# KirillHit/snn_for_object_detection

Hardware: AMD Instinct MI355X
Metric: event-frames/sec (BxT) SODa-3M GEN1 304x240 fwd+bwd (higher is better)
Workload: dtype f32 (16-bit split products)

## Files before the change

include/snn_hip.h:

```cpp
#ifndef SNN_HIP_H
#define SNN_HIP_H

#include <stddef.h>
#include <stdint.h>

#ifdef __cplusplus
extern "C" {
#endif

#define SNN_ABI_VERSION 20

enum {
    SNN_NEURON_NONE = 0,
    SNN_NEURON_LIF = 1,
    SNN_NEURON_LI = 2,
    SNN_NEURON_LI_TANH = 3,
    SNN_NEURON_SLI = 4,
    SNN_NEURON_SYNAPSE = 5
};

enum { SNN_PREC_FP32 = 0, SNN_PREC_BF16X3 = 1, SNN_PREC_BF16X6 = 3, SNN_PREC_FP16X3 = 4, SNN_PREC_BF16X1 = 5,
       SNN_PREC_BF16S = 6 };

enum { SNN_SCAN_WIDE_ADDRESSING = 1,
       SNN_SCAN_LAST_STEP_ONLY = 2,
       SNN_SCAN_BF16_STORAGE = 4,
       SNN_SCAN_SPIKES_FROM_VDEC = 8,
       SNN_SCAN_SUMS_FROM_STATE = 16,
       SNN_SCAN_STATE_LOOKBACK = 32   };

enum { SNN_POOL_AVG = 0, SNN_POOL_MAX = 1, SNN_POOL_SUM = 2 };

enum { SNN_ACT_RELU = 0, SNN_ACT_SILU = 1, SNN_ACT_TANH = 2 };

enum { SNN_SURR_SUPER = 0, SNN_SURR_TRIANGLE = 1, SNN_SURR_SIGMOID = 2, SNN_SURR_ATAN = 3 };

typedef struct snn_neuron_params {
    float c_mem;
    float c_syn;
    float v_leak;
    float v_th;
    float v_reset;
    float alpha;
    float v_st;
    float tau_sec;
    float tau_dis;
    float dt;
    float sigma;
    int surrogate;
    int reset_detached;
} snn_neuron_params;

int snn_abi_version(void);
const char* snn_last_error(void);

int snn_nchw_to_nhwc(const float* src, float* dst, int64_t N, int C, int H, int W, void* stream);
int snn_nhwc_to_nchw(const float* src, float* dst, int64_t N, int C, int H, int W, void* stream);
int snn_weight_transpose(const float* w, float* wt, int Cout, int KH, int KW, int Cin, void* stream);
int snn_weight_transpose_batched(const float* flat_w, float* flat_wt, const int64_t* table, int n_layers, void* stream);
int snn_weight_presplit(const float* w, void* out, int64_t n, int precision, void* stream);

int snn_conv2d_wgrad_bn_supported(int64_t N, int H, int W, int Cin, int Ho, int Wo, int Cout, int KH, int KW, int stride,
// ... 30 lines not shown
                     const float* addend2, int64_t ld_addend2, int precision, void* stream);
int snn_conv2d_wgrad(const float* x, int64_t ldx, const float* dy, int64_t lddy, float* dw,
                     int64_t N, int H, int W, int Cin, int Ho, int Wo, int Cout,
                     int KH, int KW, int stride, int pad, int accumulate,
                     float* workspace, int splitk, int precision, void* stream);
int snn_conv2d_wgrad_splitk(int64_t N, int H, int W, int Cin, int Ho, int Wo, int Cout, int KH, int KW,
                            int stride, int pad, int precision);
int snn_conv2d_wgrad_kernel(int64_t N, int H, int W, int Cin, int Ho, int Wo, int Cout, int KH, int KW, int stride, int pad,
                            int precision);
int snn_conv2d_gather_plan(int mode, int64_t N, int H, int W, int Cin, int Ho, int Wo, int Cout, int KH, int KW, int stride,
                           int pad, int64_t ld_in, int64_t ld_out, int align_bits, int has_split_image, int has_addend,
                           int has_addend2, int frames_per_step, int precision, int phase, int* out);
int snn_conv2d_wgrad_plan(int64_t N, int H, int W, int Cin, int Ho, int Wo, int Cout, int KH, int KW, int stride, int pad,
                          int64_t ldx, int64_t lddy, int align_bits, int precision, int spikes, int num_cu, int* out);
int snn_conv1x1_spikes_supported(int64_t N, int H, int W, int Cin, int Cout, int64_t ld, int fwd_precision,
                                 int bwd_precision);
int snn_conv1x1_spikes_fwd(const float* vdec, int64_t ld, float v_th, const float* w, float* y, int64_t ldy, int64_t N, int H,
                           int W, int Cin, int Cout, void* stream);
int snn_conv1x1_spikes_wgrad(const float* vdec, int64_t ld, float v_th, const float* dy, int64_t lddy, float* dw, int64_t N,
                             int H, int W, int Cin, int Cout, int accumulate, float* workspace, int splitk, void* stream);

int snn_conv2d_spikes_supported(int64_t N, int H, int W, int Cin, int Ho, int Wo, int Cout, int KH, int KW, int stride,
                                int pad, int64_t ld, int fwd_precision, int bwd_precision);
int snn_conv2d_spikes_fwd(const float* vdec, int64_t ld, float v_th, const float* w, float* y, int64_t ldy, int64_t N, int H,
                          int W, int Cin, int Ho, int Wo, int Cout, int KH, int KW, int stride, int pad, double* bn_partial,
                          int frames_per_step, int* bn_layout, void* stream);
int snn_conv2d_spikes_wgrad(const float* vdec, int64_t ld, float v_th, const float* dy, int64_t lddy, float* dw, int64_t N,
                            int H, int W, int Cin, int Ho, int Wo, int Cout, int KH, int KW, int stride, int pad,
                            int accumulate, float* workspace, int splitk, void* stream);
int snn_conv3x3_halo_spikes(const float* vdec, int64_t ld, float v_th, const void* w_image, float* y, int64_t ldy, int64_t N,
                            int H, int W, int Cin, int Cout, double* bn_partial, int frames_per_step, int* bn_layout,
                            void* stream);

size_t snn_bn_stats_partial_size(int T, int64_t M, int C);
int snn_bn_stats(const float* y, int64_t ldy, int T, int64_t M, int C, double* partial, void* stream);
int snn_bn_stats_finalize(const double* partial, int chunks, int rows_per_chunk, int T, int64_t M, int C,
                          const float* gamma, const float* bias, float eps, float momentum,
                          float* running_mean, float* running_var, int use_running,
                          float* mean, float* invstd, float* alpha, float* beta, void* stream);

int snn_bn_stats_reduce(const double* partial, int chunks, int rows_per_chunk, int T, int64_t M, int C, double* sums,
                        void* stream);
int snn_bn_stats_from_sums(const double* sums, int T, int64_t M_total, int C,
                           const float* gamma, const float* bias, float eps, float momentum,
                           float* running_mean, float* running_var,
                           float* mean, float* invstd, float* alpha, float* beta,
                           double* var_scratch, void* stream);

int snn_affine_neuron_fwd(int neuron, const float* y, int64_t ldy,
                          const float* alpha, const float* beta,
                          const float* v0, const float* i0,
                          float* out, int64_t ldo, const float* addend, int64_t ld_addend,
                          float* vT, float* iT, float* vdec,
                          int T, int64_t M, int C, const snn_neuron_params* p, int flags, void* stream);

size_t snn_affine_neuron_bwd_sums_size(int T, int64_t M, int C);
int snn_affine_neuron_bwd_sums_from_state(int neuron, int T, int64_t M, int C, int64_t ldg, const snn_neuron_params* p,
                                          int flags);
int snn_affine_neuron_bwd_plan(int neuron, int T, int64_t M, int C, int64_t ldg, int64_t ldy, int with_sums,
                               const snn_neuron_params* p, int flags, int64_t* out);
int snn_affine_neuron_bwd(int neuron, const float* g_out, int64_t ldg, const float* state,
                          const float* y, int64_t ldy, const float* g_vT, const float* g_iT,
                          const float* alpha, const float* beta, int apply_scale,
                          float* gx, float* g_v0, float* g_i0, double* sums,
                          int T, int64_t M, int C, const snn_neuron_params* p, int flags, void* stream);

int snn_lif_tau_param(const float* w_mem, const float* w_syn, int n, int C, float* c_mem, float* c_syn, void* stream);
int snn_lif_tau_fwd(int neuron, const float* y, int64_t ldy, const float* alpha, const float* beta,
                    const float* v0, const float* i0, float* out, int64_t ldo,
                    const float* addend, int64_t ld_addend, float* vT, float* iT, float* vdec,
                    int T, int64_t M, int C, const snn_neuron_params* p,
                    const float* c_mem, const float* c_syn, int flags, void* stream);
size_t snn_lif_tau_bwd_partial_size(int T, int64_t M, int C, int with_sums);
int snn_lif_tau_bwd_plan(int neuron, int T, int64_t M, int C, int64_t ldg, int64_t ldy, int with_sums, int with_tau_sums,
                         const snn_neuron_params* p, int flags, int64_t* out);
int snn_lif_tau_bwd(int neuron, const float* g_out, int64_t ldg, const float* state, const float* y, int64_t ldy,
                    const float* g_vT, const float* g_iT, const float* alpha, const float* beta, int apply_scale,
                    float* gx, float* g_v0, float* g_i0, double* sums,
                    int T, int64_t M, int C, const snn_neuron_params* p,
                    const float* c_mem, const float* c_syn, const float* v0, double* tau_partial, int flags, void* stream);
int snn_lif_tau_finalize(const double* tau_partial, int T, int64_t M, int C, int with_sums,
                         const float* c_mem, const float* c_syn, int per_layer,
                         float* d_wmem, float* d_wsyn, int accumulate, void* stream);

int snn_lif_ckpt_interval(void);
int snn_lif_fwd_ckpt(const float* y, int64_t ldy, const float* alpha, const float* beta,
                     const float* v0, const float* i0, float* out, int64_t ldo,
// ... 144 lines not shown
```

snn_for_object_detection_amd/_hip.py:

```python

import ctypes
import os
from ctypes import POINTER, Structure, c_char_p, c_double, c_float, c_int, c_int32, c_int64, c_size_t, c_void_p

_HERE = os.path.dirname(os.path.abspath(__file__))
LIB_PATH = os.environ.get("SNN_HIP_LIB") or os.path.join(_HERE, "libsnn_hip.so")

NEURON_NONE, NEURON_LIF, NEURON_LI, NEURON_LI_TANH, NEURON_SLI, NEURON_SYNAPSE = 0, 1, 2, 3, 4, 5
POOL_AVG, POOL_MAX, POOL_SUM = 0, 1, 2
ACT_RELU, ACT_SILU, ACT_TANH = 0, 1, 2
ABI_VERSION = 20
PREC_FP32, PREC_BF16X3, PREC_BF16X6, PREC_FP16X3, PREC_BF16X1, PREC_BF16S = 0, 1, 3, 4, 5, 6
SCAN_WIDE_ADDRESSING, SCAN_LAST_STEP_ONLY, SCAN_BF16_STORAGE, SCAN_SPIKES_FROM_VDEC, SCAN_SUMS_FROM_STATE = 1, 2, 4, 8, 16
SCAN_STATE_LOOKBACK = 32
SURR_SUPER, SURR_TRIANGLE, SURR_SIGMOID, SURR_ATAN = 0, 1, 2, 3


class NeuronParams(Structure):
    _fields_ = [("c_mem", c_float), ("c_syn", c_float), ("v_leak", c_float), ("v_th", c_float),
                ("v_reset", c_float), ("alpha", c_float), ("v_st", c_float), ("tau_sec", c_float),
                ("tau_dis", c_float), ("dt", c_float), ("sigma", c_float),
                ("surrogate", c_int), ("reset_detached", c_int)]


_P, _I, _L, _F = c_void_p, c_int, c_int64, c_float

SIGNATURES = {
    "snn_abi_version": (c_int, []),
    "snn_last_error": (c_char_p, []),
    "snn_nchw_to_nhwc": (c_int, [_P, _P, _L, _I, _I, _I, _P]),
    "snn_nhwc_to_nchw": (c_int, [_P, _P, _L, _I, _I, _I, _P]),
    "snn_weight_transpose": (c_int, [_P, _P, _I, _I, _I, _I, _P]),
    "snn_weight_transpose_batched": (c_int, [_P, _P, _P, _I, _P]),
    "snn_detect_decode": (c_int, [_P, _P, _P, _I, _I, _P, _P, _P, _P]),
    "snn_nms_sorted": (c_int, [_P, _P, _P, _I, _F, _P, _P, _P, _P, _P]),
    "snn_detect_decode_batched": (c_int, [_P, _P, _P, _I, _I, _I, _P, _P, _P, _P]),
    "snn_nms_sorted_batched": (c_int, [_P, _P, _P, _I, _I, _I, _F, _P, _P, _P, _P, _P]),
    "snn_detect_assemble": (c_int, [_P, _P, _P, _P, _P, _P, _I, _I, _I, _F, _P, _P]),
    "snn_conv2d_fwd": (c_int, [_P, _L, _P, _P, _P, _L, _L, _I, _I, _I, _I, _I, _I, _I, _I, _I, _I, _P, _L, _P, _I, _P, _I,
                               _P]),
    "snn_weight_presplit": (c_int, [_P, _P, _L, _I, _P]),
    "snn_conv2d_fwd_bn_partial_size": (c_size_t, [_L, _I, _I, _I, _I]),
    "snn_conv2d_wgrad_bn_supported": (c_int, [_L, _I, _I, _I, _I, _I, _I, _I, _I, _I, _I]),
    "snn_conv2d_wgrad_bn": (c_int, [_P, _L, _P, _L, _P, _L, _P, _I, _I, _P, _L, _I, _I, _I, _I, _I, _I, _I, _I, _I, _I, _I,
                                    _P, _I, _P]),
    "snn_conv3x3_s2_dgrad_supported": (c_int, [_L, _I, _I, _I, _I, _I, _I]),
    "snn_conv3x3_s2_dgrad_plan": (c_int, [_L, _I, _I, _I, _I, _I, _I, _P]),
    "snn_conv3x3_halo_plan": (c_int, [_L, _I, _I, _I, _I, _I, _P]),
    "snn_conv2d_wgrad_halo_plan": (c_int, [_L, _I, _I, _I, _I, _I, _I, _I, _I, _P]),
    "snn_conv_first_plan": (c_int, [_L, _I, _I, _I, _I, _I, _I, _I, _I, _I, _I, _P]),
    "snn_conv3x3_s2_dgrad": (c_int, [_P, _L, _P, _P, _L, _L, _I, _I, _I, _I, _I, _I, _P, _L, _P, _L, _I, _P]),
    "snn_conv3x3_halo_supported": (c_int, [_L, _I, _I, _I, _I]),
    "snn_conv3x3_halo_bn_chunks": (c_int64, [_I, _I, _I]),
    "snn_weight_frag_image_bytes": (c_size_t, [_I, _I]),
    "snn_weight_frag_image_batched": (c_int, [_P, _P, _P, _I, _I, _I, _I, _P]),
    "snn_conv3x3_halo": (c_int, [_P, _L, _P, _P, _L, _L, _I, _I, _I, _I, _P, _L, _P, _L, _P, _I, _P, _I, _P]),
    "snn_conv2d_dgrad": (c_int, [_P, _L, _P, _P, _P, _L, _L, _I, _I, _I, _I, _I, _I, _I, _I, _I, _I, _P, _L, _P, _L,
                                 _I, _P]),
    "snn_conv2d_wgrad": (c_int, [_P, _L, _P, _L, _P, _L, _I, _I, _I, _I, _I, _I, _I, _I, _I, _I, _I, _P, _I, _I,
                                 _P]),
    "snn_conv2d_wgrad_splitk": (c_int, [_L, _I, _I, _I, _I, _I, _I, _I, _I, _I, _I, _I]),
    "snn_conv2d_wgrad_kernel": (c_int, [_L, _I, _I, _I, _I, _I, _I, _I, _I, _I, _I, _I]),
    "snn_conv2d_gather_plan": (c_int, [_I, _L, _I, _I, _I, _I, _I, _I, _I, _I, _I, _I, _L, _L, _I, _I, _I, _I, _I, _I, _I, _P]),
    "snn_conv2d_wgrad_plan": (c_int, [_L, _I, _I, _I, _I, _I, _I, _I, _I, _I, _I, _L, _L, _I, _I, _I, _I, _P]),
    "snn_conv1x1_spikes_supported": (c_int, [_L, _I, _I, _I, _I, _L, _I, _I]),
    "snn_conv1x1_spikes_fwd": (c_int, [_P, _L, _F, _P, _P, _L, _L, _I, _I, _I, _I, _P]),
    "snn_conv1x1_spikes_wgrad": (c_int, [_P, _L, _F, _P, _L, _P, _L, _I, _I, _I, _I, _I, _P, _I, _P]),
    "snn_conv2d_spikes_supported": (c_int, [_L, _I, _I, _I, _I, _I, _I, _I, _I, _I, _I, _L, _I, _I]),
    "snn_conv2d_spikes_fwd": (c_int, [_P, _L, _F, _P, _P, _L, _L, _I, _I, _I, _I, _I, _I, _I, _I, _I, _I, _P, _I, _P, _P]),
    "snn_conv2d_spikes_wgrad": (c_int, [_P, _L, _F, _P, _L, _P, _L, _I, _I, _I, _I, _I, _I, _I, _I, _I, _I, _I, _P, _I, _P]),
    "snn_conv3x3_halo_spikes": (c_int, [_P, _L, _F, _P, _P, _L, _L, _I, _I, _I, _I, _P, _I, _P, _P]),
    "snn_bn_stats_partial_size": (c_size_t, [_I, _L, _I]),
    "snn_bn_stats": (c_int, [_P, _L, _I, _L, _I, _P, _P]),
    "snn_bn_stats_finalize": (c_int, [_P, _I, _I, _I, _L, _I, _P, _P, _F, _F, _P, _P, _I, _P, _P, _P, _P, _P]),
    "snn_bn_stats_reduce": (c_int, [_P, _I, _I, _I, _L, _I, _P, _P]),
    "snn_bn_stats_from_sums": (c_int, [_P, _I, _L, _I, _P, _P, _F, _F, _P, _P, _P, _P, _P, _P, _P, _P]),
    "snn_bn_bwd_reduce": (c_int, [_P, _I, _L, _I, _P, _P]),
    "snn_bn_bwd_coef": (c_int, [_P, _P, _P, _I, _L, _I, _P, _P, _P, _P, _P, _P, _P, _P, _I, _P]),
    "snn_affine_neuron_fwd": (c_int, [_I, _P, _L, _P, _P, _P, _P, _P, _L, _P, _L, _P, _P, _P, _I, _L, _I,
                                      POINTER(NeuronParams), _I, _P]),
    "snn_lif_ckpt_interval": (c_int, []),
    "snn_lif_fwd_ckpt": (c_int, [_P, _L, _P, _P, _P, _P, _P, _L, _P, _L, _P, _P, _P, _I, _L, _I,
                                 POINTER(NeuronParams), _P]),
    "snn_lif_bwd_ckpt": (c_int, [_P, _L, _P, _P, _L, _P, _P, _P, _P, _I, _P, _P, _P, _P, _I, _L, _I,
                                 POINTER(NeuronParams), _P]),
    "snn_affine_neuron_bwd_sums_size": (c_size_t, [_I, _L, _I]),
    "snn_affine_neuron_bwd": (c_int, [_I, _P, _L, _P, _P, _L, _P, _P, _P, _P, _I, _P, _P, _P, _P, _I, _L, _I,
                                      POINTER(NeuronParams), _I, _P]),
    "snn_bn_bwd_finalize": (c_int, [_P, _I, _L, _I, _P, _P, _P, _P, _P, _P, _P, _P, _I, _P]),
    "snn_bn_bwd_finalize_from_state": (c_int, [_P, _I, _L, _I, _P, _P, _P, _P, _P, _P, _L, _P, _P, _P, _P, _P, _I, _P]),
    "snn_bn_bwd_reduce_from_state": (c_int, [_P, _I, _L, _I, _P, _P, _P, _P, _P, _P, _L, _P, _P]),
    "snn_affine_neuron_bwd_sums_from_state": (c_int, [_I, _I, _L, _I, _L, POINTER(NeuronParams), _I]),
    "snn_affine_neuron_bwd_plan": (c_int, [_I, _I, _L, _I, _L, _L, _I, POINTER(NeuronParams), _I, _P]),
    "snn_lif_tau_param": (c_int, [_P, _P, _I, _I, _P, _P, _P]),
    "snn_lif_tau_fwd": (c_int, [_I, _P, _L, _P, _P, _P, _P, _P, _L, _P, _L, _P, _P, _P, _I, _L, _I,
                                POINTER(NeuronParams), _P, _P, _I, _P]),
    "snn_lif_tau_bwd_partial_size": (c_size_t, [_I, _L, _I, _I]),
    "snn_lif_tau_bwd_plan": (c_int, [_I, _I, _L, _I, _L, _L, _I, _I, POINTER(NeuronParams), _I, _P]),
    "snn_lif_tau_bwd": (c_int, [_I, _P, _L, _P, _P, _L, _P, _P, _P, _P, _I, _P, _P, _P, _P, _I, _L, _I,
                                POINTER(NeuronParams), _P, _P, _P, _P, _I, _P]),
    "snn_lif_tau_finalize": (c_int, [_P, _I, _L, _I, _I, _P, _P, _I, _P, _P, _I, _P]),
    "snn_bn_bwd_apply": (c_int, [_P, _P, _L, _P, _P, _P, _P, _L, _I, _L, _I, _I, _P]),
    "snn_bn_bwd_apply_bf16": (c_int, [_P, _P, _L, _P, _P, _P, _P, _L, _I, _L, _I, _I, _P]),
    "snn_bn_stats_bf16": (c_int, [_P, _L, _I, _L, _I, _P, _P]),
    "snn_copy_channels": (c_int, [_P, _L, _P, _L, _L, _I, _P]),
    "snn_add_channels": (c_int, [_P, _L, _P, _L, _L, _I, _P]),
    "snn_add": (c_int, [_P, _L, _P, _L, _P, _L, _L, _I, _P]),
    "snn_roi_workspace_size": (c_size_t, [_I, _I, _I]),
    "snn_roi_assign": (c_int, [_P, _P, _I, _I, _I, _F, _P, _P, _P, _P, _P]),
    "snn_det_loss_workspace_size": (c_size_t, [_L]),
    "snn_det_loss_fwd": (c_int, [_P, _P, _P, _P, _P, _L, _I, _F, _P, _P, _P, _P]),
    "snn_det_loss_bwd": (c_int, [_P, _P, _P, _P, _P, _L, _I, _F, _P, _P, _P, _P, _P]),
    "snn_label_steps": (c_int, [_P, _I, _I, _I, _I, _I, _P, _P]),
# ... 80 lines not shown
```

snn_for_object_detection_amd/csrc/conv_common.h:

```cpp
#pragma once
#include "snn_common.h"

namespace {

constexpr int kThreads = 256;
#define SNN_CONV_MIN_WAVES 3

typedef __bf16 bf16x8 __attribute__((ext_vector_type(8)));
typedef __bf16 bf16x4 __attribute__((ext_vector_type(4)));
typedef __bf16 bf16x2 __attribute__((ext_vector_type(2)));
typedef float f32x2 __attribute__((ext_vector_type(2)));
typedef unsigned u32x4 __attribute__((ext_vector_type(4)));
typedef unsigned u32x2 __attribute__((ext_vector_type(2)));
typedef _Float16 f16x8 __attribute__((ext_vector_type(8)));
typedef _Float16 f16x2 __attribute__((ext_vector_type(2)));
constexpr float kF16WeightScale = 256.0f;
constexpr float kF16ActScale = 16.0f;
constexpr float kF16Unscale = 1.0f / (kF16WeightScale * kF16ActScale);

__device__ __forceinline__ int div_magic(int n, int d, unsigned magic) { return d == 1 ? n : (int)__umulhi((unsigned)n, magic); }

enum : unsigned {
    kAlignIn16 = 1u, kAlignIn8 = 2u, kAlignW16 = 4u, kAlignOut16 = 8u, kAlignOut8 = 16u, kAlignAdd16 = 32u, kAlignAdd8 = 64u,
    kAlignAdd2_16 = 128u, kAlignAdd2_8 = 256u, kAlignSplit16 = 512u, kAlignAll = 1023u
// ... 17 lines not shown
           N * (int64_t)Ho * Wo < 0x7fffffffLL && (int64_t)H * W * ld * 16 < 0x7fffffffLL;
}

}

struct FirstGeom {
    int64_t ldx, ldy;
    int rows;
    int H, W, Ho, Wo, Cout, stride, pad;
    int group_rows, group_blocks;
    double* bn_partial;
    const float* bn_y;
    int64_t bn_ldy;
    const float* bn_coef;
    int bn_tc;
    int bn_fps;
    int rs;
};

struct FirstPlan {
    int ok;
    int rs, LW, cgs, PP;
    int blocks;
    int group_rows, group_blocks;
    int max_rows, last_stage_rows;
    size_t lds;
};
FirstPlan snn_first_layer_plan(int64_t N, int H, int W, int Ho, int Wo, int Cout, int stride, int pad,
                               int frames_per_step, bool wgrad, int num_cu);
bool snn_first_layer_shape(int Cin, int Cout, int KH, int KW);
int snn_first_layer_blocks(int64_t rows, int num_cu);
int snn_launch_first(bool wgrad, bool bnapply, bool sb, int blocks, size_t lds, const float* x, const float* w,
                     const float* dy, float* out, const FirstGeom& fg, void* stream, const char* name);
```

snn_for_object_detection_amd/csrc/conv_gather.hip:

```cpp
#include <stdlib.h>
#include <type_traits>
#include "conv_common.h"

#if defined(SNN_STAMP) || defined(SNN_CLOCK)
__device__ unsigned long long g_stamps[2048 * 8];
__device__ unsigned long long g_stamps2[2048 * 4];
extern "C" int snn_debug_stamps(unsigned long long* out, int n) {
    return (int)hipMemcpyFromSymbol(out, HIP_SYMBOL(g_stamps), sizeof(unsigned long long) * n);
}
extern "C" int snn_debug_stamps2(unsigned long long* out, int n) {
    return (int)hipMemcpyFromSymbol(out, HIP_SYMBOL(g_stamps2), sizeof(unsigned long long) * n);
}
#endif
#ifdef SNN_STAMP
#define STAMP(i) do { unsigned long long t_ = __builtin_readcyclecounter(); st_acc[i] += t_ - st_last; st_last = t_; } while (0)
#else
#define STAMP(i) do {} while (0)
#endif

namespace {

constexpr int BM = 128;
constexpr int BK = 32;
constexpr int LDK = BK + 4;
// ... 24 lines not shown
template <int WM, int WN, int TN>
__device__ __forceinline__ void stat_flush(double (&s)[TN], double (&q)[TN], double* red, double* __restrict__ partial,
                                           int64_t step, int64_t chunk, int64_t chunks, int n0, int OC, int tid) {
    const int lane = tid & 63, wave = tid >> 6;
#pragma unroll
    for (int j = 0; j < TN; ++j) {
        s[j] += __shfl_xor(s[j], 32, 64);
        q[j] += __shfl_xor(q[j], 32, 64);
        if (lane < 32) {
            red[((wave * TN + j) * 32 + lane) * 2 + 0] = s[j];
            red[((wave * TN + j) * 32 + lane) * 2 + 1] = q[j];
        }
    }
    __syncthreads();
    if (tid < WN * TN * 32) {
        const int wn = tid / (TN * 32), jr = tid % (TN * 32);
        double ss = 0.0, qq = 0.0;
#pragma unroll
        for (int wm = 0; wm < WM; ++wm) {
            const double* src = red + (((wm * WN + wn) * TN) * 32 + jr) * 2;
            ss += src[0];
            qq += src[1];
        }
        if (n0 + tid < OC) {
            double* dst = partial + snn_bn_partial_index(step, chunk, n0 + tid, chunks, OC);
            dst[0] = ss;
            dst[1] = qq;
        }
    }
    __syncthreads();
}

template <int BN, int WM, int WN, bool DGRAD, bool VEC, int SPLIT, bool FAST, bool PRESPLIT = false, bool SB = false,
          bool XSP = false>
__global__ __launch_bounds__(kThreads, (FAST && SPLIT) ? (PRESPLIT ? 3 : (SB ? (DGRAD ? 4 : SNN_GATHER_SB_WAVES) : 2)) : SNN_CONV_MIN_WAVES) void k_conv_gather(const float* __restrict__ in, const float* __restrict__ wk,
                                                          float* __restrict__ out, ConvGeom g,
                                                          const float* __restrict__ addend, int64_t ld_add,
                                                          const float* __restrict__ addend2, int64_t ld_add2) {
    constexpr int TM = BM / WM / 32;
    constexpr int TN = BN / WN / 32;
    constexpr int BROWS = BN / 32;
    static_assert(WM * WN == 4, "4 waves");
    static_assert(!SB || (FAST && SPLIT == 5 && !PRESPLIT), "bf16 storage: the pipelined one-product kernel");
    static_assert(!XSP || (FAST && SPLIT == 4 && !DGRAD && !PRESPLIT && !SB), "spikes from potentials: fp16 x 3 forward");
    constexpr int ES = SB ? 2 : 4;
    constexpr int NPIECE = SPLIT == 3 ? 3 : (SPLIT == 5 ? 1 : 2);
    constexpr int A_BYTES = SPLIT ? NPIECE * BM * LDB * 2 : BM * LDK * 4;
    constexpr int B_BYTES = SPLIT ? NPIECE * BN * LDB * 2 : BN * LDK * 4;
    constexpr int STAGE_BYTES = 4 * 32 * (TN * 32 + 4) * 4;
    constexpr int SMEM_BYTES = A_BYTES + B_BYTES > STAGE_BYTES ? A_BYTES + B_BYTES : STAGE_BYTES;
    __shared__ __attribute__((aligned(16))) unsigned char smem[SMEM_BYTES];
    float* As = reinterpret_cast<float*>(smem);
    float* Bs = reinterpret_cast<float*>(smem + A_BYTES);
    __bf16* Ah = reinterpret_cast<__bf16*>(smem);
    __bf16* Al = Ah + BM * LDB;
    __bf16* Am = Al + BM * LDB;
    __bf16* Bh = reinterpret_cast<__bf16*>(smem + A_BYTES);
    __bf16* Bl = Bh + BN * LDB;
    __bf16* Bm = Bl + BN * LDB;

    const int tid = threadIdx.x;
#if defined(SNN_STAMP) || defined(SNN_CLOCK)
    const unsigned long long st_kernel_begin = __builtin_amdgcn_s_memtime();
    const unsigned long long st_real_begin = __builtin_amdgcn_s_memrealtime();
#endif
    const int lane_id = tid & 63, wave = tid >> 6;
    const int wm = wave / WN, wn = wave % WN;
    const int r = lane_id & 31, h = lane_id >> 5;

    const int bid_xcd = blockIdx.x & 7, bid_q = blockIdx.x >> 3;
    const int bid_n = bid_q % g.ntiles;
    const int64_t bid_m = (int64_t)bid_xcd * g.mtiles_per_xcd + bid_q / g.ntiles;
    if (bid_m >= g.mtiles) return;
    const int64_t m0 = bid_m * BM;
    const int n0 = bid_n * BN;

    const int lrr = tid >> 3;
// ... 10 lines not shown
        const unsigned t = mm / ow_;
        const int ox = (int)(mm - t * ow_);
        const unsigned img = t / oh_;
        const int oy = (int)(t - img * oh_);
        a_base[j] = (int)(img * (unsigned)(g.IH * g.IW));
        if (!DGRAD) {
            a_y0[j] = oy * g.stride - g.pad;
            a_x0[j] = ox * g.stride - g.pad;
        } else if (g.stride == 1) {
            a_y0[j] = oy + g.pad;
            a_x0[j] = ox + g.pad;
        } else {
            a_y0[j] = (int)((unsigned)(oy * g.stride + g.ph + g.pad - g.kh0) / (unsigned)g.stride);
            a_x0[j] = (int)((unsigned)(ox * g.stride + g.pw + g.pad - g.kw0) / (unsigned)g.stride);
        }
    }

    auto decode_k = [&](int kk, int& dy, int& dx, int& c, int& wcol) {
        int tap = div_magic(kk, g.IC, g.magic_ic);
        c = kk - tap * g.IC;
        if (!DGRAD) {
            int kh = div_magic(tap, g.KW, g.magic_kw), kw = tap - kh * g.KW;
            dy = kh;
            dx = kw;
            wcol = kk;
        } else {
            int jh = div_magic(tap, g.nkw, g.magic_kw), jw = tap - jh * g.nkw;
            dy = -jh;
            dx = -jw;
            wcol = ((g.kh0 + g.stride * jh) * g.KW + (g.kw0 + g.stride * jw)) * g.IC + c;
        }
    };

    using AReg = typename std::conditional<SB, u32x2, f32x4>::type;
    AReg ra[4];
    f32x4 rb[BROWS];

    __amdgpu_buffer_rsrc_t rs_a, rs_b;
    int a_rel[4];
    unsigned a_mask[4];
    unsigned b_rel[BROWS];
    if (FAST) {
        const int ow_ = DGRAD ? g.OWc : g.OW, oh_ = DGRAD ? g.OHc : g.OH;
        const int64_t img0 = (unsigned)m0 / (unsigned)(oh_ * ow_);
        const int64_t ipix = (int64_t)g.IH * g.IW;
        const int64_t bytes = ((((int64_t)g.nimg - img0) * ipix - 1) * g.ldi + g.IC) * ES;
        rs_a = __builtin_amdgcn_make_buffer_rsrc(const_cast<char*>(reinterpret_cast<const char*>(in) + img0 * ipix * g.ldi * ES), 0,
                                                 bytes > 0xffffffffLL ? (int)0xffffffffu : (int)(unsigned)bytes,
                                                 0x00020000);
        rs_b = __builtin_amdgcn_make_buffer_rsrc(const_cast<float*>(wk), 0, g.OC * g.KtotFull * 4, 0x00020000);
        const int tw_n = DGRAD ? g.nkw : g.KW;
#pragma unroll
        for (int j = 0; j < 4; ++j) {
            const int relpix = (a_base[j] - (int)(img0 * ipix)) + a_y0[j] * g.IW + a_x0[j];
            a_rel[j] = (relpix * (int)g.ldi + kq) * ES;
            const int nth = DGRAD ? g.nkh : g.KH;
            unsigned xm = 0, mask = 0;
#pragma unroll
            for (int tw = 0; tw < 6; ++tw) {
                const int ix = DGRAD ? a_x0[j] - tw : a_x0[j] + tw;
                xm |= (tw < tw_n && (unsigned)ix < (unsigned)g.IW) ? 1u << tw : 0u;
            }
#pragma unroll
            for (int th = 0; th < 6; ++th) {
                const int iy = DGRAD ? a_y0[j] - th : a_y0[j] + th;
                mask |= (th < nth && (unsigned)iy < (unsigned)g.IH) ? xm << (th * tw_n) : 0u;
            }
            a_mask[j] = a_ok[j] ? mask : 0u;
        }
#pragma unroll
        for (int j = 0; j < BROWS; ++j) {
            const int n = n0 + lr + 32 * j;
            b_rel[j] = n < g.OC ? (unsigned)(n * g.KtotFull + kq) * 4u : 0x80000000u;
        }
    }
    const unsigned fast_tw_n = DGRAD ? g.nkw : g.KW;
    const unsigned fast_tw_one = fast_tw_n == 1 ? 1u : 0u;
    auto load_tiles_fast = [&](int k0n, AReg (&ra)[4], f32x4 (&rb)[BROWS], int which = 3) {
        const bool kin = k0n < g.Ktot;
        const int tap = (int)__umulhi((unsigned)k0n, g.magic_ic);
        const int c0 = k0n - tap * g.IC;
        const int th = (int)(__umulhi((unsigned)tap, g.magic_kw) + (unsigned)tap * fast_tw_one);
        const int tw = tap - th * (int)fast_tw_n;
        int toff, wcol0;
        if (!DGRAD) {
            toff = ((th * g.IW + tw) * (int)g.ldi + c0) * ES;
            wcol0 = k0n;
        } else {
            toff = (c0 - (th * g.IW + tw) * (int)g.ldi) * ES;
            wcol0 = ((g.kh0 + g.stride * th) * g.KW + (g.kw0 + g.stride * tw)) * g.IC + c0;
        }
        const int tbit = kin ? tap : 31;
        if (which & 1) {
#pragma unroll
            for (int j = 0; j < 4; ++j) {
                const int voff = ((a_mask[j] >> tbit) & 1u) ? a_rel[j] + toff : -1;
                if constexpr (SB) ra[j] = __builtin_bit_cast(u32x2, __builtin_amdgcn_raw_buffer_load_b64(rs_a, voff, 0, 0));
                else ra[j] = __builtin_bit_cast(f32x4, __builtin_amdgcn_raw_buffer_load_b128(rs_a, voff, 0, 0));
            }
        }
        if (which & 2) {
            const unsigned wb = (unsigned)wcol0 * 4u;
#pragma unroll
            for (int j = 0; j < BROWS; ++j)
                rb[j] = __builtin_bit_cast(f32x4, __builtin_amdgcn_raw_buffer_load_b128(rs_b, (int)(b_rel[j] + wb), 0, 0));
        }
    };

    auto load_tiles = [&](int k0) {
        if (FAST) {
            load_tiles_fast(k0, ra, rb);
            return;
        }
        if constexpr (!SB) {
        const int kk = k0 + kq;
        if (VEC) {
            const bool kin = kk < g.Ktot;
            int dy, dx, c, wcol;
            decode_k(kin ? kk : g.Ktot - 4, dy, dx, c, wcol);
            const f32x4 zero = {0.f, 0.f, 0.f, 0.f};
#pragma unroll
            for (int j = 0; j < 4; ++j) {
                const int iy = a_y0[j] + dy, ix = a_x0[j] + dx;
                const bool ok = kin & a_ok[j] & ((unsigned)iy < (unsigned)g.IH) & ((unsigned)ix < (unsigned)g.IW);
                const int iyc = min(max(iy, 0), g.IH - 1), ixc = min(max(ix, 0), g.IW - 1);
                f32x4 v = *reinterpret_cast<const f32x4*>(in + (int64_t)(a_base[j] + iyc * g.IW + ixc) * g.ldi + c);
                ra[j] = ok ? v : zero;
            }
#pragma unroll
            for (int j = 0; j < BROWS; ++j) {
                const int n = n0 + lr + 32 * j;
                const int nc = min(n, g.OC - 1);
                f32x4 v = *reinterpret_cast<const f32x4*>(wk + (int64_t)nc * g.KtotFull + wcol);
                rb[j] = (kin & (n < g.OC)) ? v : zero;
            }
        } else {
#pragma unroll
            for (int e = 0; e < 4; ++e) {
                const int ke = kk + e;
                const bool kin = ke < g.Ktot;
                int dy, dx, c, wcol;
                decode_k(kin ? ke : 0, dy, dx, c, wcol);
#pragma unroll
                for (int j = 0; j < 4; ++j) {
                    const int iy = a_y0[j] + dy, ix = a_x0[j] + dx;
                    float v = 0.f;
                    if (kin && a_ok[j] && (unsigned)iy < (unsigned)g.IH && (unsigned)ix < (unsigned)g.IW)
// ... 4 lines not shown
                for (int j = 0; j < BROWS; ++j) {
                    int n = n0 + lr + 32 * j;
                    rb[j][e] = (kin && n < g.OC) ? wk[(int64_t)n * g.KtotFull + wcol] : 0.f;
                }
            }
        }
        }
    };
    auto split_store = [&](const f32x4& v, __bf16* hi_img, __bf16* mid_img, __bf16* lo_img, int row) {
        bf16x4 hi, mid, lo;
#pragma unroll
        for (int e = 0; e < 4; e += 2) {
            f32x2 rest = {v[e], v[e + 1]};
            bf16x2 p = __builtin_convertvector(rest, bf16x2);
            unsigned bits = __builtin_bit_cast(unsigned, p);
            hi[e] = p[0]; hi[e + 1] = p[1];
            rest[0] -= __builtin_bit_cast(float, bits << 16);
            rest[1] -= __builtin_bit_cast(float, bits & 0xffff0000u);
            if (SPLIT == 3) {
                p = __builtin_convertvector(rest, bf16x2);
                bits = __builtin_bit_cast(unsigned, p);
                mid[e] = p[0]; mid[e + 1] = p[1];
                rest[0] -= __builtin_bit_cast(float, bits << 16);
                rest[1] -= __builtin_bit_cast(float, bits & 0xffff0000u);
            }
            p = __builtin_convertvector(rest, bf16x2);
            lo[e] = p[0]; lo[e + 1] = p[1];
        }
        *reinterpret_cast<bf16x4*>(&hi_img[row * LDB + kq]) = hi;
        if (SPLIT == 3) *reinterpret_cast<bf16x4*>(&mid_img[row * LDB + kq]) = mid;
        *reinterpret_cast<bf16x4*>(&lo_img[row * LDB + kq]) = lo;
    };
    auto store_tiles = [&]() {
        if constexpr (SB) return;
        else if (SPLIT) {
#pragma unroll
            for (int j = 0; j < 4; ++j) split_store(ra[j], Ah, Am, Al, lr + 32 * j);
#pragma unroll
            for (int j = 0; j < BROWS; ++j) split_store(rb[j], Bh, Bm, Bl, lr + 32 * j);
        } else {
#pragma unroll
            for (int j = 0; j < 4; ++j) *reinterpret_cast<f32x4*>(&As[(lr + 32 * j) * LDK + kq]) = ra[j];
#pragma unroll
            for (int j = 0; j < BROWS; ++j) *reinterpret_cast<f32x4*>(&Bs[(lr + 32 * j) * LDK + kq]) = rb[j];
        }
    };

    f32x16 acc[TM][TN];
#pragma unroll
    for (int i = 0; i < TM; ++i)
#pragma unroll
        for (int j = 0; j < TN; ++j)
#pragma unroll
            for (int e = 0; e < 16; ++e) acc[i][j][e] = 0.f;

    if constexpr (FAST && SPLIT != 0) {
        constexpr int NP = NPIECE;
        constexpr int NPROD = SPLIT == 3 ? 6 : (SPLIT == 5 ? 1 : 3);
        bf16x4 pa[4][NP], pb[BROWS][NP];
        auto convert = [&](const f32x4& v, bf16x4* out, float scale) {
            if constexpr (SPLIT == 5) {
#pragma unroll
                for (int e = 0; e < 4; e += 2) {
                    const bf16x2 p = __builtin_convertvector(f32x2{v[e], v[e + 1]}, bf16x2);
                    out[0][e] = p[0]; out[0][e + 1] = p[1];
                }
                return;
// ... 3 lines not shown
#pragma unroll
                for (int e = 0; e < 4; e += 2) {
                    const float a = v[e] * scale, b = v[e + 1] * scale;
                    const f16x2 ph = __builtin_convertvector(f32x2{a, b}, f16x2);
                    const f16x2 pl = __builtin_convertvector(f32x2{a - (float)ph[0], b - (float)ph[1]}, f16x2);
                    hi[e >> 1] = __builtin_bit_cast(unsigned, ph);
                    lo[e >> 1] = __builtin_bit_cast(unsigned, pl);
                }
                out[0] = __builtin_bit_cast(bf16x4, hi);
                out[1] = __builtin_bit_cast(bf16x4, lo);
                return;
            }
#pragma unroll
            for (int e = 0; e < 4; e += 2) {
                f32x2 rest = {v[e], v[e + 1]};
                bf16x2 p = __builtin_convertvector(rest, bf16x2);
                unsigned bits = __builtin_bit_cast(unsigned, p);
                out[0][e] = p[0]; out[0][e + 1] = p[1];
                rest[0] -= __builtin_bit_cast(float, bits << 16);
                rest[1] -= __builtin_bit_cast(float, bits & 0xffff0000u);
                if (SPLIT == 3) {
                    p = __builtin_convertvector(rest, bf16x2);
                    bits = __builtin_bit_cast(unsigned, p);
                    out[2][e] = p[0]; out[2][e + 1] = p[1];
                    rest[0] -= __builtin_bit_cast(float, bits << 16);
                    rest[1] -= __builtin_bit_cast(float, bits & 0xffff0000u);
                }
                p = __builtin_convertvector(rest, bf16x2);
                out[1][e] = p[0]; out[1][e + 1] = p[1];
            }
        };
        auto convert_a = [&](const AReg& v, bf16x4* out) {
            if constexpr (SB) out[0] = __builtin_bit_cast(bf16x4, v);
            else if constexpr (XSP) {
                u32x2 hi;
#pragma unroll
                for (int e = 0; e < 4; e += 2)
                    hi[e >> 1] = (v[e] > g.x_th ? 0x4C00u : 0u) | (v[e + 1] > g.x_th ? 0x4C000000u : 0u);
                out[0] = __builtin_bit_cast(bf16x4, hi);
            } else convert(v, out, kF16ActScale);
        };
        auto convert_b = [&](const f32x4& v, bf16x4* out) {
            if constexpr (PRESPLIT) {
                static_assert(!PRESPLIT || SPLIT == 2 || SPLIT == 4, "pre-split weights: two-piece modes only");
                out[0] = __builtin_bit_cast(bf16x4, f32x2{v[0], v[1]});
                out[1] = __builtin_bit_cast(bf16x4, f32x2{v[2], v[3]});
            } else {
                convert(v, out, kF16WeightScale);
            }
        };
        auto write_tiles = [&]() {
#pragma unroll
            for (int j = 0; j < 4; ++j) {
                const int o = (lr + 32 * j) * LDB + kq;
                *reinterpret_cast<bf16x4*>(&Ah[o]) = pa[j][0];
                if constexpr (NP >= 2 && !XSP) *reinterpret_cast<bf16x4*>(&Al[o]) = pa[j][1];
                if constexpr (NP >= 3) *reinterpret_cast<bf16x4*>(&Am[o]) = pa[j][2];
            }
#pragma unroll
            for (int j = 0; j < BROWS; ++j) {
                const int o = (lr + 32 * j) * LDB + kq;
                *reinterpret_cast<bf16x4*>(&Bh[o]) = pb[j][0];
                if constexpr (NP >= 2) *reinterpret_cast<bf16x4*>(&Bl[o]) = pb[j][1];
                if constexpr (NP >= 3) *reinterpret_cast<bf16x4*>(&Bm[o]) = pb[j][2];
            }
        };
        auto mfma_group = [&](int ks) {
            bf16x8 ah[TM], am[TM], al[TM], bh[TN], bm[TN], bl[TN];
#pragma unroll
            for (int i = 0; i < TM; ++i) {
                const int off = ((wm * TM + i) * 32 + r) * LDB + ks * 16 + 8 * h;
                ah[i] = *reinterpret_cast<const bf16x8*>(&Ah[off]);
                if constexpr (NP >= 2 && !XSP) al[i] = *reinterpret_cast<const bf16x8*>(&Al[off]);
                if constexpr (NP >= 3) am[i] = *reinterpret_cast<const bf16x8*>(&Am[off]);
            }
#pragma unroll
            for (int j = 0; j < TN; ++j) {
                const int off = ((wn * TN + j) * 32 + r) * LDB + ks * 16 + 8 * h;
                bh[j] = *reinterpret_cast<const bf16x8*>(&Bh[off]);
                if constexpr (NP >= 2) bl[j] = *reinterpret_cast<const bf16x8*>(&Bl[off]);
                if constexpr (NP >= 3) bm[j] = *reinterpret_cast<const bf16x8*>(&Bm[off]);
            }
#pragma unroll
            for (int i = 0; i < TM; ++i)
#pragma unroll
                for (int j = 0; j < TN; ++j) {
                    if constexpr (SPLIT == 5) {
                        acc[i][j] = __builtin_amdgcn_mfma_f32_32x32x16_bf16(ah[i], bh[j], acc[i][j], 0, 0, 0);
                        continue;
                    }
                    if constexpr (SPLIT == 4 && XSP) {
                        const f16x8 xah = __builtin_bit_cast(f16x8, ah[i]);
                        const f16x8 xbh = __builtin_bit_cast(f16x8, bh[j]), xbl = __builtin_bit_cast(f16x8, bl[j]);
                        acc[i][j] = __builtin_amdgcn_mfma_f32_32x32x16_f16(xah, xbl, acc[i][j], 0, 0, 0);
                        acc[i][j] = __builtin_amdgcn_mfma_f32_32x32x16_f16(xah, xbh, acc[i][j], 0, 0, 0);
                        continue;
                    }
                    if constexpr (SPLIT == 4) {
                        const f16x8 xah = __builtin_bit_cast(f16x8, ah[i]), xal = __builtin_bit_cast(f16x8, al[i]);
                        const f16x8 xbh = __builtin_bit_cast(f16x8, bh[j]), xbl = __builtin_bit_cast(f16x8, bl[j]);
                        acc[i][j] = __builtin_amdgcn_mfma_f32_32x32x16_f16(xal, xbh, acc[i][j], 0, 0, 0);
                        acc[i][j] = __builtin_amdgcn_mfma_f32_32x32x16_f16(xah, xbl, acc[i][j], 0, 0, 0);
                        acc[i][j] = __builtin_amdgcn_mfma_f32_32x32x16_f16(xah, xbh, acc[i][j], 0, 0, 0);
                        continue;
                    }
                    acc[i][j] = __builtin_amdgcn_mfma_f32_32x32x16_bf16(al[i], bh[j], acc[i][j], 0, 0, 0);
                    acc[i][j] = __builtin_amdgcn_mfma_f32_32x32x16_bf16(ah[i], bl[j], acc[i][j], 0, 0, 0);
                    if (SPLIT == 3) {
                        acc[i][j] = __builtin_amdgcn_mfma_f32_32x32x16_bf16(am[i], bm[j], acc[i][j], 0, 0, 0);
                        acc[i][j] = __builtin_amdgcn_mfma_f32_32x32x16_bf16(am[i], bh[j], acc[i][j], 0, 0, 0);
                        acc[i][j] = __builtin_amdgcn_mfma_f32_32x32x16_bf16(ah[i], bm[j], acc[i][j], 0, 0, 0);
                    }
                    acc[i][j] = __builtin_amdgcn_mfma_f32_32x32x16_bf16(ah[i], bh[j], acc[i][j], 0, 0, 0);
                }
        };
        constexpr int NM = TM * TN * (XSP ? 2 : NPROD);
        constexpr int NREAD = XSP ? TM + TN * NP : (TM + TN) * NP;
        constexpr int CONV_OPS = SPLIT == 3 ? 24 : (SPLIT == 5 ? 2 : 14);
        constexpr int VPG_A = ((XSP ? 4 * 8 : 4 * CONV_OPS) + NM - 1) / NM;
        constexpr int VPG_B = PRESPLIT ? 1 : (BROWS * CONV_OPS + NM - 1) / NM;
        if (g.Ktot > 0) {
            AReg ra0[4];
            f32x4 rb0[BROWS];
            load_tiles_fast(0, ra0, rb0);
            load_tiles_fast(BK, ra, rb);
#pragma unroll
            for (int j = 0; j < 4; ++j) convert_a(ra0[j], pa[j]);
#pragma unroll
            for (int j = 0; j < BROWS; ++j) convert_b(rb0[j], pb[j]);
            write_tiles();
        }
        __syncthreads();
#ifdef SNN_STAMP
        unsigned long long st_acc[8] = {0, 0, 0, 0, 0, 0, 0, 0};
        unsigned long long st_last = __builtin_readcyclecounter();
        const unsigned long long st_begin = st_last;
#endif
#pragma unroll 1
        for (int k0 = 0; k0 < g.Ktot; k0 += BK) {
            mfma_group(0);
#pragma unroll
            for (int j = 0; j < 4; ++j) convert_a(ra[j], pa[j]);
            __builtin_amdgcn_sched_group_barrier(0x100, NREAD, 0);
#pragma unroll
            for (int m = 0; m < NM; ++m) {
                __builtin_amdgcn_sched_group_barrier(0x008, 1, 0);
                __builtin_amdgcn_sched_group_barrier(0x002, VPG_A, 0);
            }
            __builtin_amdgcn_sched_barrier(0);
            STAMP(0);
            mfma_group(1);
#pragma unroll
            for (int j = 0; j < BROWS; ++j) convert_b(rb[j], pb[j]);
            __builtin_amdgcn_sched_group_barrier(0x100, NREAD, 0);
#pragma unroll
            for (int m = 0; m < NM; ++m) {
                __builtin_amdgcn_sched_group_barrier(0x008, 1, 0);
                __builtin_amdgcn_sched_group_barrier(0x002, VPG_B, 0);
            }
            __builtin_amdgcn_sched_barrier(0);
            STAMP(1);
            load_tiles_fast(k0 + 2 * BK, ra, rb);
            STAMP(2);
            __syncthreads();
            STAMP(3);
            write_tiles();
            STAMP(4);
            __syncthreads();
            STAMP(5);
        }
#ifdef SNN_STAMP
        if (tid == 0 && bid_n == 0 && blockIdx.x < 2048) {
            st_acc[6] = __builtin_readcyclecounter() - st_begin;
            st_acc[7] = st_begin;
            for (int i = 0; i < 8; ++i) g_stamps[blockIdx.x * 8 + i] = st_acc[i];
        }
#endif
    } else {
        if (g.Ktot > 0) {
            load_tiles(0);
            store_tiles();
        }
        __syncthreads();

    #pragma unroll 1
        for (int k0 = 0; k0 < g.Ktot; k0 += BK) {
            load_tiles(k0 + BK);
            __builtin_amdgcn_sched_barrier(0);
            if (SPLIT) {
    #pragma unroll
                for (int ks = 0; ks < BK / 16; ++ks) {
                    bf16x8 ah[TM], am[TM], al[TM], bh[TN], bm[TN], bl[TN];
    #pragma unroll
                    for (int i = 0; i < TM; ++i) {
// ... 137 lines not shown
                const int a = (int)(t - img * (unsigned)g.OHc);
                const int64_t pix = ((int64_t)img * g.OH + (a * g.stride + g.ph)) * g.OW + (b * g.stride + g.pw);
                dst = out_b + (pix * g.ldo + n) * ES;
                a1p = ad1_b + (pix * ld_add + n) * ES;
                a2p = ad2_b + (pix * ld_add2 + n) * ES;
            }
            if (ovec && n + 3 < g.OC) {
                if (addend) v += St::ld4_last(a1p, 0);
                if (addend2) v += St::ld4_last(a2p, 0);
                St::st4(dst, 0, v);
            } else {
#pragma unroll
                for (int q = 0; q < 4; ++q)
                    if (n + q < g.OC) {
                        float o = v[q];
                        if (addend) o += St::ld1(a1p, q);
                        if (addend2) o += St::ld1(a2p, q);
                        St::st1(dst, q, o);
                    }
            }
        }
        __syncthreads();
    }
#if defined(SNN_STAMP) || defined(SNN_CLOCK)
    if (tid == 0 && bid_n == 0 && blockIdx.x < 2048) {
        g_stamps2[blockIdx.x * 4 + 0] = st_kernel_begin;
        g_stamps2[blockIdx.x * 4 + 1] = __builtin_amdgcn_s_memtime();
        g_stamps2[blockIdx.x * 4 + 2] = st_real_begin;
        g_stamps2[blockIdx.x * 4 + 3] = __builtin_amdgcn_s_memrealtime();
    }
#endif
}

enum GatherLoader { kLoadScalar = 0, kLoadVec = 1, kLoadFast = 2, kLoadFastPresplit = 3, kLoadSB = 4, kLoadXSP = 5 };
enum GatherRefusal { kGatherOk = 0, kGatherTooManyPixels, kGatherNotFastSB, kGatherNotFastXSP, kGatherGridTooLarge };
struct GatherPlan {
    int ok, why;
    int loader;
    int bn;
    int out_vec;
    int mtiles, mtiles_per_xcd, ntiles;
    int64_t blocks;
};
static GatherPlan gather_plan(const ConvGeom& g, bool dgrad, int split, bool sb, bool xsp, unsigned align, bool has_split,
                              bool has_add, bool has_add2) {
    GatherPlan p = {};
    const bool vec = (g.IC % 4 == 0) && (g.ldi % 4 == 0) && (align & (sb ? kAlignIn8 : kAlignIn16)) && (align & kAlignW16);
    const int64_t gm = snn_ceil_div(g.Mtot, BM);
    if (!(g.Mtot < 0x7fffffffLL && (int64_t)g.IH * g.IW < 0x7fffffffLL)) {
        p.why = kGatherTooManyPixels;
        return p;
    }
    const int nth = dgrad ? g.nkh : g.KH, ntw = dgrad ? g.nkw : g.KW;
    const int ntaps = nth * ntw;
    static const bool no_fast = snn_tuning_env("SNN_CONV_NO_FAST") != nullptr;
    const bool fast = vec && !no_fast && g.IC % BK == 0 && ntaps >= 1 && ntaps <= 31 && nth <= 6 && ntw <= 6 &&
                      (int64_t)g.IH * g.IW * g.ldi * 16 < 0x7fffffffLL && (int64_t)g.OC * g.KtotFull * 4 < 0x7fffffffLL;
    p.out_vec = (g.ldo % 4 == 0) && (align & (sb ? kAlignOut8 : kAlignOut16)) &&
                (!has_add || (align & (sb ? kAlignAdd8 : kAlignAdd16))) &&
                (!has_add2 || (align & (sb ? kAlignAdd2_8 : kAlignAdd2_16)));
    if (sb && !fast) {
        p.why = kGatherNotFastSB;
        return p;
    }
    if (xsp && !fast) {
        p.why = kGatherNotFastXSP;
        return p;
    }
    const bool presplit = has_split && (split == 2 || split == 4) && (align & kAlignSplit16);
    p.loader = sb ? kLoadSB : xsp ? kLoadXSP : (fast && presplit) ? kLoadFastPresplit : fast ? kLoadFast : vec ? kLoadVec : kLoadScalar;
    p.bn = g.OC <= 32 ? 32 : (g.OC <= 64 ? 64 : 128);
    p.mtiles = (int)gm;
    p.mtiles_per_xcd = (int)snn_ceil_div(gm, 8);
    p.ntiles = (int)snn_ceil_div(g.OC, p.bn);
    p.blocks = (int64_t)p.mtiles_per_xcd * 8 * p.ntiles;
    if (p.blocks > 0x7fffffffLL) {
        p.why = kGatherGridTooLarge;
        return p;
    }
    p.ok = 1;
    return p;
}

static unsigned gather_align_bits(const void* in, const void* wk, const void* wk_split, const void* out, const void* addend,
                                  int64_t ld_add, const void* addend2, int64_t ld_add2) {
    unsigned a = 0;
    if (aligned(16, {in})) a |= kAlignIn16;
    if (aligned(8, {in})) a |= kAlignIn8;
    if (aligned(16, {wk})) a |= kAlignW16;
    if (aligned(16, {out})) a |= kAlignOut16;
    if (aligned(8, {out})) a |= kAlignOut8;
    if (addend && ld_add % 4 == 0 && aligned(16, {addend})) a |= kAlignAdd16;
    if (addend && ld_add % 4 == 0 && aligned(8, {addend})) a |= kAlignAdd8;
    if (addend2 && ld_add2 % 4 == 0 && aligned(16, {addend2})) a |= kAlignAdd2_16;
    if (addend2 && ld_add2 % 4 == 0 && aligned(8, {addend2})) a |= kAlignAdd2_8;
    if (wk_split && aligned(16, {wk_split})) a |= kAlignSplit16;
    return a;
}

constexpr int gather_wm(int bn) { return bn == 32 ? 4 : 2; }
constexpr int gather_wn(int bn) { return bn == 32 ? 1 : 2; }

static int launch_gather(bool dgrad, int split, bool sb, bool xsp, const float* in, const float* wk, const void* wk_split,
                         float* out, const ConvGeom& g, const float* addend, int64_t ld_add, const float* addend2,
                         int64_t ld_add2, hipStream_t st, const char* name) {
    const GatherPlan p = gather_plan(g, dgrad, split, sb, xsp,
                                     gather_align_bits(in, wk, wk_split, out, addend, ld_add, addend2, ld_add2),
                                     wk_split != nullptr, addend != nullptr, addend2 != nullptr);
    SNN_REQUIRE(p.why != kGatherTooManyPixels, "%s: too many pixels", name);
    SNN_REQUIRE(p.why != kGatherNotFastSB, "%s: bf16 storage covers the pipelined implicit GEMM only (channels a multiple of 32, pixel "
                "stride a multiple of 4, 8-byte aligned tensors): %d channels, stride %lld", name, g.IC, (long long)g.ldi);
    SNN_REQUIRE(p.why != kGatherNotFastXSP, "%s: covers the pipelined implicit GEMM only (input channels a multiple of 32, pixel stride a "
                "multiple of 4, 16-byte aligned tensors): %d channels, stride %lld", name, g.IC, (long long)g.ldi);
    SNN_REQUIRE(p.why != kGatherGridTooLarge, "%s: grid too large", name);
    ConvGeom gg = g;
    gg.out_vec = p.out_vec;
    gg.mtiles = p.mtiles;
    gg.mtiles_per_xcd = p.mtiles_per_xcd;
    gg.ntiles = p.ntiles;
    const dim3 grid((unsigned)p.blocks);
    const float* wsrc = p.loader == kLoadFastPresplit ? static_cast<const float*>(wk_split) : wk;
    dispatch(
        [&](auto BN, auto L, auto DGRAD, auto SPLIT) {
            constexpr int l = L(), s = SPLIT();
            constexpr bool vec = l != kLoadScalar, fast = l >= kLoadFast, pre = l == kLoadFastPresplit, sbl = l == kLoadSB,
                           xspl = l == kLoadXSP;
            constexpr int ksplit = fast ? s : (vec ? (s == 4 ? 3 : (s == 5 ? 2 : s)) : 0);
            if constexpr ((DGRAD() ? s != 3 && s != 4 : s != 2) && (!sbl || s == 5) && (!xspl || (!DGRAD() && s == 4)) &&
                          (!pre || s == 2 || s == 4)) {
                hipLaunchKernelGGL((k_conv_gather<BN(), gather_wm(BN()), gather_wn(BN()), DGRAD(), vec, ksplit, fast, pre, sbl, xspl>),
                                   grid, dim3(kThreads), 0, st, in, wsrc, out, gg, addend, ld_add, addend2, ld_add2);
                return true;
            }
            return false;
        },
        OneOf<32, 64, 128>{p.bn}, OneOf<0, 1, 2, 3, 4, 5>{p.loader}, Flag{dgrad}, OneOf<0, 2, 3, 4, 5>{split});
    SNN_CHECK_LAUNCH(name);
    return 0;
}

}

namespace {
template <bool F16>
__global__ void k_weight_presplit(const f32x4* __restrict__ w, u32x4* __restrict__ out, int64_t groups) {
    for (int64_t i = (int64_t)blockIdx.x * blockDim.x + threadIdx.x; i < groups; i += (int64_t)gridDim.x * blockDim.x) {
        const f32x4 v = w[i];
        u32x4 o;
#pragma unroll
        for (int e = 0; e < 4; e += 2) {
            if (F16) {
                const float a = v[e] * kF16WeightScale, b = v[e + 1] * kF16WeightScale;
                const f16x2 ph = __builtin_convertvector(f32x2{a, b}, f16x2);
                const f16x2 pl = __builtin_convertvector(f32x2{a - (float)ph[0], b - (float)ph[1]}, f16x2);
                o[e >> 1] = __builtin_bit_cast(unsigned, ph);
                o[2 + (e >> 1)] = __builtin_bit_cast(unsigned, pl);
            } else {
                f32x2 rest = {v[e], v[e + 1]};
                const bf16x2 ph = __builtin_convertvector(rest, bf16x2);
                const unsigned bits = __builtin_bit_cast(unsigned, ph);
                rest[0] -= __builtin_bit_cast(float, bits << 16);
                rest[1] -= __builtin_bit_cast(float, bits & 0xffff0000u);
                const bf16x2 pl = __builtin_convertvector(rest, bf16x2);
                o[e >> 1] = bits;
                o[2 + (e >> 1)] = __builtin_bit_cast(unsigned, pl);
            }
        }
        out[i] = o;
    }
// ... 227 lines not shown
                                            int bwd_precision) {
    return snn_conv2d_spikes_supported(N, H, W, Cin, H, W, Cout, 1, 1, 1, 0, ld, fwd_precision, bwd_precision);
}

extern "C" int snn_conv2d_spikes_fwd(const float* vdec, int64_t ld, float v_th, const float* w, float* y, int64_t ldy,
                                     int64_t N, int H, int W, int Cin, int Ho, int Wo, int Cout, int KH, int KW, int stride,
                                     int pad, double* bn_partial, int frames_per_step, int* bn_layout, void* stream) {
    SNN_REQUIRE(vdec && w && y, "snn_conv2d_spikes_fwd: null pointer");
    SNN_REQUIRE(v_th >= 0.0f, "snn_conv2d_spikes_fwd: a negative threshold would turn padding into spikes");
    if (check_conv_shape("snn_conv2d_spikes_fwd", N, H, W, Cin, Ho, Wo, Cout, KH, KW, stride, pad)) return 1;
    SNN_REQUIRE(spikes_shape_ok(N, H, W, Cin, Ho, Wo, Cout, KH, KW, stride, pad, ld) && ldy >= Cout,
                "snn_conv2d_spikes_fwd: shape not covered (ask snn_conv2d_spikes_supported)");
    SNN_REQUIRE(!bn_partial || (bn_layout && frames_per_step > 0 && N % frames_per_step == 0),
                "snn_conv2d_spikes_fwd: statistics need bn_layout and a frames_per_step that divides N");
    if (bn_layout) bn_layout[0] = bn_layout[1] = 0;
    ConvGeom g = gather_fwd_geom(N, H, W, Cin, Ho, Wo, Cout, KH, KW, stride, pad, ld, ldy);
    g.x_th = v_th;
    const int64_t step_rows = bn_partial ? (int64_t)frames_per_step * Ho * Wo : 0;
    if (const int chunks = gather_bn_plan(bn_partial != nullptr, step_rows)) {
        g.bn_partial = bn_partial;
        g.bn_rows = step_rows;
        g.bn_chunks = chunks;
        bn_layout[0] = g.bn_chunks;
        bn_layout[1] = BM;
    }
    return launch_gather(false, 4, false, true, vdec, w, nullptr, y, g, nullptr, 0, nullptr, 0, (hipStream_t)stream,
                         "snn_conv2d_spikes_fwd");
}

extern "C" int snn_conv1x1_spikes_fwd(const float* vdec, int64_t ld, float v_th, const float* w, float* y, int64_t ldy,
                                      int64_t N, int H, int W, int Cin, int Cout, void* stream) {
    return snn_conv2d_spikes_fwd(vdec, ld, v_th, w, y, ldy, N, H, W, Cin, H, W, Cout, 1, 1, 1, 0, nullptr, 0, nullptr, stream);
}
```

snn_for_object_detection_amd/csrc/conv_wgrad.hip:

```cpp
#include <stdlib.h>
#include <type_traits>
#include "conv_common.h"

namespace {

constexpr int WB_K = 32;

struct WgradGeom {
    int64_t Mtot;
    int H, W, Cin, Ho, Wo, Cout, KH, KW, stride, pad;
    int64_t ldx, lddy;
    int Ktot;
    int64_t pix_per_split;
    int tiles_m, tiles_n, splitk;
    int nimg;
    float x_th;
};

template <int TM, int TN, int WM, int WN, bool VEC>
__global__ __launch_bounds__(kThreads, SNN_CONV_MIN_WAVES) void k_conv_wgrad(const float* __restrict__ x, const float* __restrict__ dy,
                                                         float* __restrict__ ws, WgradGeom g) {
    static_assert(WM * WN == 4, "4 waves");
    constexpr int BMc = 32 * TM * WM, BNk = 32 * TN * WN;
    constexpr int DG = BMc / 4, XG = BNk / 4;
// ... 141 lines not shown
        for (int ks = 0; ks < WB_K / 2; ++ks) {
            float a[TM], b[TN];
#pragma unroll
            for (int i = 0; i < TM; ++i) a[i] = Ds[(ks * 2 + h) * BMc + (wm * TM + i) * 32 + r];
#pragma unroll
            for (int j = 0; j < TN; ++j) b[j] = Xs[(ks * 2 + h) * BNk + (wn * TN + j) * 32 + r];
#pragma unroll
            for (int i = 0; i < TM; ++i)
#pragma unroll
                for (int j = 0; j < TN; ++j)
                    acc[i][j] = __builtin_amdgcn_mfma_f32_32x32x2f32(a[i], b[j], acc[i][j], 0, 0, 0);
        }
        __syncthreads();
        store_tiles();
        __syncthreads();
        slot ^= 1;
    }

    float* slab = ws + (int64_t)z * g.Cout * (int64_t)g.Ktot;
#pragma unroll
    for (int i = 0; i < TM; ++i)
#pragma unroll
        for (int j = 0; j < TN; ++j) {
            const int kc = kc0 + (wn * TN + j) * 32 + r;
            if (kc >= g.Ktot) continue;
#pragma unroll
            for (int e = 0; e < 16; ++e) {
                const int co = co0 + (wm * TM + i) * 32 + (e & 3) + 8 * (e >> 2) + 4 * h;
                if (co < g.Cout) slab[(int64_t)co * g.Ktot + kc] = acc[i][j][e];
            }
        }
}

template <int TM, int TN, int WM, int WN, int WBK, bool ONE, bool SB = false, bool XSP = false>
__global__ __launch_bounds__(kThreads, 2) void k_conv_wgrad_pipe(const float* __restrict__ x,
                                                                 const float* __restrict__ dy,
                                                                 float* __restrict__ ws, WgradGeom g) {
    static_assert(WM * WN == 4, "4 waves");
    constexpr int BMc = 32 * TM * WM, BNk = 32 * TN * WN;
    constexpr int DG = BMc / 4, XG = BNk / 4;
    static_assert(WBK == 32 || WBK == 64, "stage length");
    static_assert(!SB || ONE, "bf16 storage: one product");
    static_assert(!XSP || (!ONE && !SB), "spikes from potentials: the bf16 x 3 kernel");
    constexpr int ES = SB ? 2 : 4;
    constexpr int LDW = WBK + 8;
    constexpr int NQ = WBK / 4;
    constexpr int GPP = kThreads / NQ;
    constexpr int DQ = (DG + GPP - 1) / GPP, XQ = (XG + GPP - 1) / GPP;
    __shared__ __attribute__((aligned(16))) __bf16 Dh[BMc * LDW];
    __shared__ __attribute__((aligned(16))) __bf16 Dl[ONE ? 8 : BMc * LDW];
    __shared__ __attribute__((aligned(16))) __bf16 Xh[BNk * LDW];
    __shared__ __attribute__((aligned(16))) __bf16 Xl[(ONE || XSP) ? 8 : BNk * LDW];
    __shared__ __attribute__((aligned(16))) int Pinfo[2][WBK][4];

    const int tid = threadIdx.x;
    const int lane_id = tid & 63, wave = tid >> 6;
    const int wm = wave / WN, wn = wave % WN;
    const int r = lane_id & 31, h = lane_id >> 5;

    const int tiles = g.tiles_m * g.tiles_n;
    int L = blockIdx.x, z, tile;
    if (g.splitk % 8 == 0) {
        z = (L % 8) + 8 * (L / (8 * tiles));
        tile = (L / 8) % tiles;
    } else {
        z = L / tiles;
        tile = L % tiles;
    }
    const int co0 = (tile % g.tiles_m) * BMc;
    const int kc0 = (tile / g.tiles_m) * BNk;
    const unsigned p_lo = (unsigned)((int64_t)z * g.pix_per_split);
    unsigned p_hi = p_lo + (unsigned)g.pix_per_split;
    if (p_hi > (unsigned)g.Mtot) p_hi = (unsigned)g.Mtot;
    if (p_lo >= p_hi) p_hi = p_lo;

    const unsigned opix = (unsigned)(g.Ho * g.Wo), ipix = (unsigned)(g.H * g.W);
    const unsigned img_lo = p_lo / opix;
    __amdgpu_buffer_rsrc_t rs_d, rs_x;
    {
        const int64_t dbytes = p_hi > p_lo ? (((int64_t)(p_hi - p_lo) - 1) * g.lddy + g.Cout) * ES : 0;
        rs_d = __builtin_amdgcn_make_buffer_rsrc(
            const_cast<char*>(reinterpret_cast<const char*>(dy) + (int64_t)p_lo * g.lddy * ES), 0, (int)dbytes, 0x00020000);
        const int64_t xbytes = ((((int64_t)g.nimg - img_lo) * ipix - 1) * g.ldx + g.Cin) * ES;
        rs_x = __builtin_amdgcn_make_buffer_rsrc(
            const_cast<char*>(reinterpret_cast<const char*>(x) + (int64_t)img_lo * ipix * g.ldx * ES), 0,
// ... 4 lines not shown
    int d_off[DQ];
    int x_tapoff[XQ];
    int x_kh[XQ], x_kw[XQ], x_cq[XQ], d_cq[DQ];
    bool x_ok[XQ];
#pragma unroll
    for (int q = 0; q < DQ; ++q) {
        d_cq[q] = (grp0 + GPP * q) * 4;
        const bool ok = (grp0 + GPP * q) < DG && (co0 + d_cq[q]) < g.Cout;
        d_off[q] = ok ? ((quad * 4) * (int)g.lddy + co0 + d_cq[q]) * ES : -1;
    }
#pragma unroll
    for (int q = 0; q < XQ; ++q) {
        x_cq[q] = (grp0 + GPP * q) * 4;
        const int kc = kc0 + x_cq[q];
        x_ok[q] = (grp0 + GPP * q) < XG && kc < g.Ktot;
        const int kcc = x_ok[q] ? kc : 0;
        const int tap = kcc / g.Cin, ci = kcc - tap * g.Cin;
        x_kh[q] = tap / g.KW;
        x_kw[q] = tap - x_kh[q] * g.KW;
        x_tapoff[q] = ((x_kh[q] * g.W + x_kw[q]) * (int)g.ldx + ci) * ES;
    }

    int d_img = 0, d_oy = 0, d_ox = 0;
    unsigned d_p = p_lo + tid;
    if (tid < WBK) {
        const unsigned pp = d_p < (unsigned)g.Mtot ? d_p : 0u;
        const unsigned t = pp / (unsigned)g.Wo;
        d_ox = (int)(pp - t * (unsigned)g.Wo);
        const unsigned im = t / (unsigned)g.Ho;
        d_oy = (int)(t - im * (unsigned)g.Ho);
        d_img = (int)(im - img_lo);
    }
    auto decode = [&](int slot) {
        if (tid < WBK) {
            const int y0 = d_oy * g.stride - g.pad, x0 = d_ox * g.stride - g.pad;
            int4 info;
            info.x = ((d_img * (int)ipix + y0 * g.W + x0) * (int)g.ldx) * ES;
            info.y = y0;
            info.z = x0;
            info.w = d_p < p_hi ? 1 : 0;
            *reinterpret_cast<int4*>(&Pinfo[slot][tid][0]) = info;
            d_p += WBK;
            d_ox += WBK;
            while (d_ox >= g.Wo) {
                d_ox -= g.Wo;
                if (++d_oy == g.Ho) {
                    d_oy = 0;
                    ++d_img;
                }
            }
        }
    };

    using OReg = typename std::conditional<SB, u32x2, f32x4>::type;
    OReg rd[DQ][4], rx[XQ][4];
    auto load_tiles = [&](unsigned p0, int slot) {
        const int dstage = (int)(p0 - p_lo) * (int)g.lddy * ES;
        auto fetch = [&](__amdgpu_buffer_rsrc_t rs, int voff) -> OReg {
            if constexpr (SB) return __builtin_bit_cast(u32x2, __builtin_amdgcn_raw_buffer_load_b64(rs, voff, 0, 0));
            else return __builtin_bit_cast(f32x4, __builtin_amdgcn_raw_buffer_load_b128(rs, voff, 0, 0));
        };
#pragma unroll
        for (int e = 0; e < 4; ++e) {
            const int4 info = *reinterpret_cast<const int4*>(&Pinfo[slot][quad * 4 + e][0]);
#pragma unroll
            for (int q = 0; q < DQ; ++q) {
                const int voff = d_off[q] < 0 ? -1 : d_off[q] + e * (int)g.lddy * ES + dstage;
                rd[q][e] = fetch(rs_d, voff);
            }
#pragma unroll
            for (int q = 0; q < XQ; ++q) {
                const int iy = info.y + x_kh[q], ix = info.z + x_kw[q];
                const bool ok = (info.w != 0) & x_ok[q] & ((unsigned)iy < (unsigned)g.H) & ((unsigned)ix < (unsigned)g.W);
                const int voff = ok ? info.x + x_tapoff[q] : -1;
                rx[q][e] = fetch(rs_x, voff);
            }
        }
    };
    bf16x4 pd[DQ][4][2], px[XQ][4][2];
    auto convert_quad = [&](const OReg (&v)[4], bf16x4 (&out)[4][2]) {
        if constexpr (SB) {
#pragma unroll
            for (int c = 0; c < 4; ++c) {
                const unsigned a0 = v[0][c >> 1], a1 = v[1][c >> 1], a2 = v[2][c >> 1], a3 = v[3][c >> 1];
                u32x2 o;
                if (c & 1) o = u32x2{(a0 >> 16) | (a1 & 0xffff0000u), (a2 >> 16) | (a3 & 0xffff0000u)};
                else o = u32x2{(a0 & 0xffffu) | (a1 << 16), (a2 & 0xffffu) | (a3 << 16)};
                out[c][0] = __builtin_bit_cast(bf16x4, o);
            }
        } else {
#pragma unroll
        for (int c = 0; c < 4; ++c)
#pragma unroll
            for (int e = 0; e < 4; e += 2) {
                f32x2 rest = {v[e][c], v[e + 1][c]};
                bf16x2 pp = __builtin_convertvector(rest, bf16x2);
                const unsigned bits = __builtin_bit_cast(unsigned, pp);
                out[c][0][e] = pp[0]; out[c][0][e + 1] = pp[1];
                if constexpr (!ONE) {
                    rest[0] -= __builtin_bit_cast(float, bits << 16);
                    rest[1] -= __builtin_bit_cast(float, bits & 0xffff0000u);
                    pp = __builtin_convertvector(rest, bf16x2);
                    out[c][1][e] = pp[0]; out[c][1][e + 1] = pp[1];
                }
            }
        }
    };
    auto convert_spikes = [&](const OReg (&v)[4], bf16x4 (&out)[4][2]) {
        if constexpr (XSP) {
#pragma unroll
            for (int c = 0; c < 4; ++c) {
                u32x2 o;
#pragma unroll
                for (int e = 0; e < 4; e += 2)
                    o[e >> 1] = (v[e][c] > g.x_th ? 0x3F80u : 0u) | (v[e + 1][c] > g.x_th ? 0x3F800000u : 0u);
                out[c][0] = __builtin_bit_cast(bf16x4, o);
            }
        }
    };
    auto write_tiles = [&]() {
#pragma unroll
        for (int q = 0; q < DQ; ++q)
            if (grp0 + GPP * q < DG) {
#pragma unroll
                for (int c = 0; c < 4; ++c) {
                    *reinterpret_cast<bf16x4*>(&Dh[(d_cq[q] + c) * LDW + quad * 4]) = pd[q][c][0];
                    if constexpr (!ONE) *reinterpret_cast<bf16x4*>(&Dl[(d_cq[q] + c) * LDW + quad * 4]) = pd[q][c][1];
                }
            }
#pragma unroll
        for (int q = 0; q < XQ; ++q)
            if (grp0 + GPP * q < XG) {
#pragma unroll
                for (int c = 0; c < 4; ++c) {
                    *reinterpret_cast<bf16x4*>(&Xh[(x_cq[q] + c) * LDW + quad * 4]) = px[q][c][0];
                    if constexpr (!ONE && !XSP) *reinterpret_cast<bf16x4*>(&Xl[(x_cq[q] + c) * LDW + quad * 4]) = px[q][c][1];
                }
            }
    };

    f32x16 acc[TM][TN];
#pragma unroll
    for (int i = 0; i < TM; ++i)
#pragma unroll
        for (int j = 0; j < TN; ++j)
#pragma unroll
            for (int e = 0; e < 16; ++e) acc[i][j][e] = 0.f;

    auto mfma_group = [&](int ks) {
        bf16x8 ah[TM], al[TM], bh[TN], bl[TN];
#pragma unroll
        for (int i = 0; i < TM; ++i) {
            const int off = ((wm * TM + i) * 32 + r) * LDW + ks * 16 + 8 * h;
            ah[i] = *reinterpret_cast<const bf16x8*>(&Dh[off]);
            if constexpr (!ONE) al[i] = *reinterpret_cast<const bf16x8*>(&Dl[off]);
        }
#pragma unroll
        for (int j = 0; j < TN; ++j) {
            const int off = ((wn * TN + j) * 32 + r) * LDW + ks * 16 + 8 * h;
            bh[j] = *reinterpret_cast<const bf16x8*>(&Xh[off]);
            if constexpr (!ONE && !XSP) bl[j] = *reinterpret_cast<const bf16x8*>(&Xl[off]);
        }
#pragma unroll
        for (int i = 0; i < TM; ++i)
#pragma unroll
            for (int j = 0; j < TN; ++j) {
                if constexpr (!ONE) {
                    acc[i][j] = __builtin_amdgcn_mfma_f32_32x32x16_bf16(al[i], bh[j], acc[i][j], 0, 0, 0);
                    if constexpr (!XSP) acc[i][j] = __builtin_amdgcn_mfma_f32_32x32x16_bf16(ah[i], bl[j], acc[i][j], 0, 0, 0);
                }
                acc[i][j] = __builtin_amdgcn_mfma_f32_32x32x16_bf16(ah[i], bh[j], acc[i][j], 0, 0, 0);
            }
    };
    constexpr int NM = TM * TN * (ONE ? 1 : (XSP ? 2 : 3));
    constexpr int NREAD = XSP ? 2 * TM + TN : (TM + TN) * (ONE ? 1 : 2);
    constexpr int CQ_OPS = SB ? 12 : 56;
    constexpr int VPG_D = (DQ * CQ_OPS + NM - 1) / NM, VPG_X = (XQ * (XSP ? 24 : CQ_OPS) + NM - 1) / NM;

    decode(0);
    __syncthreads();
    load_tiles(p_lo, 0);
    decode(1);
    __syncthreads();
#pragma unroll
    for (int q = 0; q < DQ; ++q) convert_quad(rd[q], pd[q]);
#pragma unroll
    for (int q = 0; q < XQ; ++q) {
        if constexpr (XSP) convert_spikes(rx[q], px[q]);
        else convert_quad(rx[q], px[q]);
    }
    write_tiles();
    load_tiles(p_lo + WBK, 1);
    decode(0);
    __syncthreads();

    int slot = 0;
#pragma unroll 1
    for (unsigned p0 = p_lo; p0 < p_hi; p0 += WBK) {
        mfma_group(0);
#pragma unroll
        for (int q = 0; q < DQ; ++q) convert_quad(rd[q], pd[q]);
        __builtin_amdgcn_sched_group_barrier(0x100, NREAD, 0);
#pragma unroll
        for (int m = 0; m < NM; ++m) {
            __builtin_amdgcn_sched_group_barrier(0x008, 1, 0);
            __builtin_amdgcn_sched_group_barrier(0x002, VPG_D, 0);
        }
        __builtin_amdgcn_sched_barrier(0);
        mfma_group(1);
#pragma unroll
        for (int q = 0; q < XQ; ++q) {
            if constexpr (XSP) convert_spikes(rx[q], px[q]);
            else convert_quad(rx[q], px[q]);
        }
        __builtin_amdgcn_sched_group_barrier(0x100, NREAD, 0);
#pragma unroll
        for (int m = 0; m < NM; ++m) {
            __builtin_amdgcn_sched_group_barrier(0x008, 1, 0);
            __builtin_amdgcn_sched_group_barrier(0x002, VPG_X, 0);
        }
        __builtin_amdgcn_sched_barrier(0);
#pragma unroll
        for (int ks = 2; ks < WBK / 16; ++ks) mfma_group(ks);
        load_tiles(p0 + 2 * WBK, slot);
        __syncthreads();
        write_tiles();
        decode(slot ^ 1);
        __syncthreads();
        slot ^= 1;
    }

    float* slab = ws + (int64_t)z * g.Cout * (int64_t)g.Ktot;
#pragma unroll
    for (int i = 0; i < TM; ++i)
#pragma unroll
        for (int j = 0; j < TN; ++j) {
            const int kcol = kc0 + (wn * TN + j) * 32 + r;
            if (kcol >= g.Ktot) continue;
#pragma unroll
            for (int e = 0; e < 16; ++e) {
                const int co = co0 + (wm * TM + i) * 32 + (e & 3) + 8 * (e >> 2) + 4 * h;
                if (co < g.Cout) slab[(int64_t)co * g.Ktot + kcol] = acc[i][j][e];
            }
        }
}
// ... 243 lines not shown
    FirstPlan p = snn_first_layer_plan(N, H, W, Ho, Wo, Cout, stride, pad, 0, true, num_cu);
    if (!(ldx % 2 == 0 && (align & kAlignIn8) && lddy % 4 == 0 && (align & (dy_bf16 ? kAlignDy8 : kAlignDy16)) &&
          (int64_t)W * ldx < 0x7fffffffLL))
        p.ok = 0;
    return p;
}
static unsigned wgrad_align_bits(const void* x, const void* dy) {
    return (aligned(16, {x}) ? kAlignIn16 : 0u) | (aligned(8, {x}) ? kAlignIn8 : 0u) | (aligned(16, {dy}) ? kAlignDy16 : 0u) |
           (aligned(8, {dy}) ? kAlignDy8 : 0u);
}
static FirstPlan first_layer_wgrad_plan(const float* x, int64_t ldx, const float* dy, int64_t lddy, int64_t N, int H, int W,
                                        int Cin, int Ho, int Wo, int Cout, int KH, int KW, int stride, int pad) {
    return first_layer_wgrad_plan(wgrad_align_bits(x, dy), ldx, lddy, N, H, W, Cin, Ho, Wo, Cout, KH, KW, stride, pad, false, 0);
}

enum WgradKernel { kWgradPipe = 0, kWgradVec = 1, kWgradScalar = 2, kWgradHalo = 3, kWgradFirst = 4 };
enum WgradRefusal { kWgradOk = 0, kWgradHaloSplitk, kWgradNotPipeSB, kWgradNotPipeXSP, kWgradGridTooLarge };
struct WgradPlan {
    int ok, why;
    int kernel;
    WgradTile t;
    int tiles_m, tiles_n, wbk;
    int splitk;
    int64_t pix_per_split;
    int64_t last_pix;
    int empty_splits;
    bool one;
    FirstPlan fp;
    SnnWgradHaloPlan hp;
    ReducePlan r;
};
static WgradPlan wgrad_plan(int64_t N, int H, int W, int Cin, int Ho, int Wo, int Cout, int KH, int KW, int stride, int pad,
                            int64_t ldx, int64_t lddy, unsigned align, int precision, bool xsp, int num_cu, int splitk,
                            bool halo = true) {
    WgradPlan p = {};
    if (num_cu <= 0) num_cu = snn_num_cu();
    const int bwd_split = precision;
    const bool sbf = precision == SNN_PREC_BF16S;
    const int64_t M = N * Ho * (int64_t)Wo;
    const int Ktot = KH * KW * Cin;
    const int64_t n = (int64_t)Cout * Ktot;
    p.splitk = splitk > 0 ? splitk : wgrad_splitk(N, H, W, Cin, Ho, Wo, Cout, KH, KW, stride, pad, precision, num_cu);
    p.r = wgrad_reduce_plan(n, p.splitk, (align & kAlignDw16) != 0, num_cu);
    p.fp = xsp ? FirstPlan{}
               : first_layer_wgrad_plan(align, ldx, lddy, N, H, W, Cin, Ho, Wo, Cout, KH, KW, stride, pad, sbf, num_cu);
    if (p.fp.ok) {
        p.kernel = kWgradFirst;
        p.ok = 1;
        return p;
    }
    if (bwd_split && halo) {
        p.hp = snn_wgrad_halo_plan(N, H, W, Cin, Ho, Wo, Cout, KH, KW, stride, pad, num_cu);
        if (p.hp.ok) {
            p.kernel = kWgradHalo;
            p.ok = p.splitk == p.hp.slabs;
            p.why = p.ok ? kWgradOk : kWgradHaloSplitk;
            return p;
        }
    }
    const bool vec = (Cin % 4 == 0) && (Cout % 4 == 0) && (ldx % 4 == 0) && (lddy % 4 == 0) &&
                     (sbf ? (align & kAlignIn8) && (align & kAlignDy8) : (align & kAlignIn16) && (align & kAlignDy16));
    p.t = wgrad_tile(Cout, Ktot, bwd_split && Cin % 4 == 0 && Cout % 4 == 0, M);
    static const int wbk_small = snn_tuning_env("SNN_WGRAD_WBK") ? atoi(snn_tuning_env("SNN_WGRAD_WBK")) : 64;
    p.wbk = (p.t.id >= 4 && wbk_small == 64) ? 64 : 32;
    p.pix_per_split = snn_ceil_div(snn_ceil_div(M, p.splitk), p.wbk) * p.wbk;
    const int64_t span_pix = p.pix_per_split * (int64_t)stride * stride + 3 * (int64_t)H * W;
    static const bool no_pipe = snn_tuning_env("SNN_WGRAD_NO_PIPE") != nullptr;
    const bool pipe = vec && bwd_split && !no_pipe && M < 0x7fffffffLL && span_pix * ldx * 4 < 0x7fffffffLL &&
                      p.pix_per_split * lddy * 4 < 0x7fffffffLL && (int64_t)H * W * ldx * 4 < 0x7fffffffLL;
    p.one = precision == SNN_PREC_BF16X1 || sbf;
    p.kernel = pipe ? kWgradPipe : (vec ? kWgradVec : kWgradScalar);
    if (sbf && !pipe) {
        p.why = kWgradNotPipeSB;
        return p;
    }
    if (xsp && !(pipe && !p.one)) {
        p.why = kWgradNotPipeXSP;
        return p;
    }
    p.tiles_m = (int)snn_ceil_div(Cout, p.t.bm);
    p.tiles_n = (int)snn_ceil_div(Ktot, p.t.bn);
    if ((int64_t)p.tiles_m * p.tiles_n * p.splitk > 0x7fffffff) {
        p.why = kWgradGridTooLarge;
        return p;
    }
    const int64_t owners = snn_ceil_div(M, p.pix_per_split);
    p.last_pix = M - (owners - 1) * p.pix_per_split;
    p.empty_splits = (int)(p.splitk - owners);
    p.ok = 1;
    return p;
}
}

static int wgrad_common(const float* x, int64_t ldx, const float* dy, int64_t lddy, float* dw, int64_t N,
                        int H, int W, int Cin, int Ho, int Wo, int Cout, int KH, int KW, int stride, int pad,
                        int accumulate, float* workspace, int splitk, int precision, void* stream, bool xsp, float x_th) {
    SNN_REQUIRE(x && dy && dw && workspace, "snn_conv2d_wgrad: null pointer");
    SNN_REQUIRE(precision == SNN_PREC_FP32 || precision == SNN_PREC_BF16X3 || precision == SNN_PREC_BF16X1 ||
                    precision == SNN_PREC_BF16S,
                "snn_conv2d_wgrad: precision must be SNN_PREC_FP32, _BF16X3, _BF16X1 or _BF16S (got %d)", precision);
    const bool sbf = precision == SNN_PREC_BF16S;
    if (check_conv_shape("snn_conv2d_wgrad", N, H, W, Cin, Ho, Wo, Cout, KH, KW, stride, pad)) return 1;
    SNN_REQUIRE(ldx >= Cin && lddy >= Cout, "snn_conv2d_wgrad: pixel stride smaller than channel count");
    SNN_REQUIRE(splitk >= 1 && splitk <= 32768, "snn_conv2d_wgrad: bad splitk %d", splitk);
    SNN_REQUIRE(N * (int64_t)H * W < 0x7fffffffLL, "snn_conv2d_wgrad: more than 2^31 input pixels");
    WgradGeom g;
    g.Mtot = N * Ho * (int64_t)Wo;
    g.H = H; g.W = W; g.Cin = Cin; g.Ho = Ho; g.Wo = Wo; g.Cout = Cout;
    g.KH = KH; g.KW = KW; g.stride = stride; g.pad = pad;
    g.ldx = ldx; g.lddy = lddy;
    g.Ktot = KH * KW * Cin;
    g.x_th = x_th;
    const unsigned align = wgrad_align_bits(x, dy) | (aligned(16, {dw, workspace}) ? kAlignDw16 : 0u);
    WgradPlan p = wgrad_plan(N, H, W, Cin, Ho, Wo, Cout, KH, KW, stride, pad, ldx, lddy, align, precision, xsp, 0, splitk);
    if (p.kernel == kWgradFirst) {
        const FirstPlan& fp = p.fp;
        FirstGeom fg = {ldx, lddy, (int)(N * Ho), H, W, Ho, Wo, Cout, stride, pad, fp.group_rows, splitk, nullptr,
                        nullptr, 0, nullptr, 0, 1, fp.rs};
        if (const int rc = snn_launch_first(true, false, sbf, splitk, fp.lds, x, nullptr, dy, workspace, fg, stream, "snn_conv2d_wgrad"))
            return rc;
        return wgrad_reduce_slabs(workspace, dw, (int64_t)Cout * g.Ktot, splitk, accumulate, (hipStream_t)stream);
    }
    if (p.kernel == kWgradHalo) {
        const SnnWgradHaloPlan& hp = p.hp;
        SNN_REQUIRE(p.why != kWgradHaloSplitk, "snn_conv2d_wgrad: splitk %d, expected %d (snn_conv2d_wgrad_splitk)", splitk,
                    hp.slabs);
        const int rc = snn_wgrad_halo_launch(hp, x, ldx, dy, lddy, workspace, N, H, W, Cin, Ho, Wo, Cout, stride,
                                             xsp ? 2 : ((precision == SNN_PREC_BF16X1 || sbf) ? 1 : 3), sbf,
                                             (hipStream_t)stream, x_th);
        if (rc == 0)
            return wgrad_reduce_slabs(workspace, dw, (int64_t)Cout * g.Ktot, hp.slabs, accumulate, (hipStream_t)stream);
        if (rc > 0) return rc;
        p = wgrad_plan(N, H, W, Cin, Ho, Wo, Cout, KH, KW, stride, pad, ldx, lddy, align, precision, xsp, 0, splitk, false);
    }
    SNN_REQUIRE(p.why != kWgradNotPipeSB, "snn_conv2d_wgrad: bf16 storage covers the event-frame layer and the pipelined kernels only "
                "(channels and strides multiples of 4, 8-byte aligned tensors, < 2 GiB per pixel split)");
    SNN_REQUIRE(p.why != kWgradNotPipeXSP, "snn_conv1x1_spikes_wgrad: covers the pipelined bf16 x 3 kernel only (channels and "
                "strides multiples of 4, 16-byte aligned tensors, < 2 GiB per pixel split)");
    SNN_REQUIRE(p.why != kWgradGridTooLarge, "snn_conv2d_wgrad: grid too large");
    g.pix_per_split = p.pix_per_split;
    g.nimg = (int)N;
    g.tiles_m = p.tiles_m;
    g.tiles_n = p.tiles_n;
    g.splitk = splitk;
    dim3 grid((unsigned)((int64_t)g.tiles_m * g.tiles_n * splitk));
    hipStream_t st = (hipStream_t)stream;
    dispatch(
        [&](auto ID, auto KERNEL, auto WBK, auto ONE, auto SB, auto XSP) {
            constexpr WgradShape t = kWgradShapes[ID()];
            if constexpr (KERNEL() != kWgradPipe) {
                hipLaunchKernelGGL((k_conv_wgrad<t.tm, t.tn, t.wm, t.wn, KERNEL() == kWgradVec>), grid, dim3(kThreads), 0, st, x, dy,
                                   workspace, g);
            } else if constexpr ((!SB() || ONE()) && (!XSP() || (!ONE() && !SB()))) {
                hipLaunchKernelGGL((k_conv_wgrad_pipe<t.tm, t.tn, t.wm, t.wn, WBK(), ONE(), SB(), XSP()>), grid, dim3(kThreads), 0,
                                   st, x, dy, workspace, g);
            }
            return true;
        },
        OneOf<0, 1, 2, 3, 4, 5>{p.t.id}, OneOf<0, 1, 2>{p.kernel}, OneOf<32, 64>{p.wbk}, Flag{p.one}, Flag{sbf}, Flag{xsp});
    SNN_CHECK_LAUNCH("snn_conv2d_wgrad");
    return wgrad_reduce_slabs(workspace, dw, (int64_t)Cout * g.Ktot, splitk, accumulate, st);
}

extern "C" int snn_conv2d_wgrad_splitk(int64_t N, int H, int W, int Cin, int Ho, int Wo, int Cout, int KH, int KW,
                                       int stride, int pad, int precision) {
    if (N <= 0 || Ho <= 0 || Wo <= 0 || Cin <= 0 || Cout <= 0 || KH <= 0 || KW <= 0) return 1;
    return wgrad_plan(N, H, W, Cin, Ho, Wo, Cout, KH, KW, stride, pad, Cin, Cout, kAlignAll, precision, false, 0, 0).splitk;
}

extern "C" int snn_conv2d_wgrad_kernel(int64_t N, int H, int W, int Cin, int Ho, int Wo, int Cout, int KH, int KW, int stride,
                                       int pad, int precision) {
    if (N <= 0 || Ho <= 0 || Wo <= 0 || Cin <= 0 || Cout <= 0 || KH <= 0 || KW <= 0) return 0;
    if (snn_first_layer_shape(Cin, Cout, KH, KW)) return 2;
    const int k = wgrad_plan(N, H, W, Cin, Ho, Wo, Cout, KH, KW, stride, pad, Cin, Cout, kAlignAll, precision, false, 0, 0).kernel;
    return k == kWgradHalo ? 1 : (k == kWgradFirst ? 2 : 0);
}

extern "C" int snn_conv2d_wgrad_bn_supported(int64_t N, int H, int W, int Cin, int Ho, int Wo, int Cout, int KH, int KW,
                                             int stride, int pad) {
    if (Cin != 2 || KH != 3 || KW != 3) return 0;
    return snn_first_layer_plan(N, H, W, Ho, Wo, Cout, stride, pad, 0, true, 0).ok;
}

extern "C" int snn_conv2d_wgrad_bn(const float* x, int64_t ldx, const float* gx, int64_t ldgx, const float* y, int64_t ldy,
                                   const float* coef, int T, int frames_per_step, float* dw, int64_t N, int H, int W,
                                   int Cin, int Ho, int Wo, int Cout, int KH, int KW, int stride, int pad, int accumulate,
                                   float* workspace, int splitk, void* stream) {
    SNN_REQUIRE(x && gx && y && coef && dw && workspace, "snn_conv2d_wgrad_bn: null pointer");
    if (check_conv_shape("snn_conv2d_wgrad_bn", N, H, W, Cin, Ho, Wo, Cout, KH, KW, stride, pad)) return 1;
    SNN_REQUIRE(frames_per_step > 0 && T > 0 && (int64_t)T * frames_per_step == N,
                "snn_conv2d_wgrad_bn: %lld frames are not %d timesteps of %d", (long long)N, T, frames_per_step);
    SNN_REQUIRE(ldx >= Cin && ldgx >= Cout && ldy >= Cout, "snn_conv2d_wgrad_bn: pixel stride smaller than channel count");
// ... 24 lines not shown
    if (check_conv_shape("snn_conv2d_wgrad_plan", N, H, W, Cin, Ho, Wo, Cout, KH, KW, stride, pad)) return 1;
    if (!(precision == SNN_PREC_FP32 || precision == SNN_PREC_BF16X3 || precision == SNN_PREC_BF16X1 ||
          precision == SNN_PREC_BF16S) || ldx < Cin || lddy < Cout || !(N * (int64_t)H * W < 0x7fffffffLL))
        return 1;
    if (spikes && (precision != SNN_PREC_BF16X3 || !spikes_shape_ok(N, H, W, Cin, Ho, Wo, Cout, KH, KW, stride, pad, ldx)))
        return 1;
    const WgradPlan p = wgrad_plan(N, H, W, Cin, Ho, Wo, Cout, KH, KW, stride, pad, ldx, lddy, (unsigned)align_bits, precision,
                                   spikes != 0, num_cu, 0);
    if (!p.ok) return 1;
    const bool gemm = p.kernel <= kWgradScalar;
    const int v[18] = {1, p.kernel, gemm ? p.t.id : 0, gemm ? p.t.bm : 0, gemm ? p.t.bn : 0, p.tiles_m, p.tiles_n, gemm ? p.wbk : 0,
                       p.splitk, (int)p.pix_per_split, (int)p.last_pix, p.empty_splits, p.r.kind, p.r.kg, p.r.groups, p.r.per,
                       (int)p.r.blocks, gemm ? (int)((int64_t)p.tiles_m * p.tiles_n * p.splitk) : 0};
    for (int i = 0; i < 18; ++i) out[i] = v[i];
    return 0;
}

extern "C" int snn_conv2d_spikes_wgrad(const float* vdec, int64_t ld, float v_th, const float* dy, int64_t lddy, float* dw,
                                       int64_t N, int H, int W, int Cin, int Ho, int Wo, int Cout, int KH, int KW, int stride,
                                       int pad, int accumulate, float* workspace, int splitk, void* stream) {
    SNN_REQUIRE(v_th >= 0.0f, "snn_conv2d_spikes_wgrad: a negative threshold would turn padding into spikes");
    SNN_REQUIRE(spikes_shape_ok(N, H, W, Cin, Ho, Wo, Cout, KH, KW, stride, pad, ld),
                "snn_conv2d_spikes_wgrad: shape not covered (ask snn_conv2d_spikes_supported)");
    return wgrad_common(vdec, ld, dy, lddy, dw, N, H, W, Cin, Ho, Wo, Cout, KH, KW, stride, pad, accumulate, workspace, splitk,
                        SNN_PREC_BF16X3, stream, true, v_th);
}

extern "C" int snn_conv1x1_spikes_wgrad(const float* vdec, int64_t ld, float v_th, const float* dy, int64_t lddy, float* dw,
                                        int64_t N, int H, int W, int Cin, int Cout, int accumulate, float* workspace,
                                        int splitk, void* stream) {
    return snn_conv2d_spikes_wgrad(vdec, ld, v_th, dy, lddy, dw, N, H, W, Cin, H, W, Cout, 1, 1, 1, 0, accumulate, workspace,
                                   splitk, stream);
}
```

snn_for_object_detection_amd/csrc/scan_fwd.hip:

```cpp
#include "scan_common.h"

namespace {

#ifndef SNN_SCAN_PREFETCH
#define SNN_SCAN_PREFETCH 2
#endif
template <int NEURON, int VEC, int SAVE, bool SB = false, bool PC = false>
__global__ __launch_bounds__(kThreads) void k_affine_neuron_fwd(
    const float* __restrict__ y, int64_t ldy, const float* __restrict__ alpha, const float* __restrict__ beta,
    const float* __restrict__ v0, const float* __restrict__ i0, float* __restrict__ out, int64_t ldo,
    const float* __restrict__ addend, int64_t ld_add, float* __restrict__ vT, float* __restrict__ iT,
    float* __restrict__ vdec, int T, int64_t M, int C, snn_neuron_params p, int last_only,
    const float* __restrict__ cmem_pc = nullptr, const float* __restrict__ csyn_pc = nullptr) {
    typedef typename Vec<VEC>::type V;
    static_assert(!SB || SAVE != 2, "the checkpointed scan keeps fp32 checkpoints: not combined with bf16 storage");
    static_assert(!PC || (NEURON == SNN_NEURON_LIF && !SB && SAVE != 2), "per-channel time constants: LIF on fp32 tensors");
    const int cv = C / VEC;
    const int64_t total = M * cv;
    for (int64_t col = (int64_t)blockIdx.x * kThreads + threadIdx.x; col < total;
         col += (int64_t)gridDim.x * kThreads) {
        const int64_t m = col / cv;
        const int c = (int)(col % cv) * VEC;
        V v, i;
        [[maybe_unused]] V cmv, csv;
        if constexpr (PC) {
            cmv = Vec<VEC>::load(cmem_pc + c);
            csv = Vec<VEC>::load(csyn_pc + c);
        }
        if (NEURON != SNN_NEURON_NONE) {
            if (v0) v = Vec<VEC>::load(v0 + m * C + c);
            else {
#pragma unroll
                for (int j = 0; j < VEC; ++j) lane<VEC>(v, j) = p.v_leak;
            }
            if (i0) i = Vec<VEC>::load(i0 + m * C + c);
            else {
#pragma unroll
                for (int j = 0; j < VEC; ++j) lane<VEC>(i, j) = 0.0f;
            }
        }
        auto time_loop = [&](auto piped_c, auto add_c, auto noout_c, auto last_c) {
        constexpr bool PIPED = decltype(piped_c)::value;
        constexpr bool LAST = decltype(last_c)::value;
        constexpr bool ADD = decltype(add_c)::value;
        constexpr bool NOOUT = decltype(noout_c)::value;
        constexpr int kPrefetch = PIPED ? SNN_SCAN_PREFETCH : 0;
        struct StepOps { V x, a, b, ad; };
        auto fetch_step = [&](int t) {
            const int tc = t < T ? t : T - 1;
            const int64_t row = (int64_t)tc * M + m;
            StepOps o;
            o.x = VecS<VEC, SB>::load_last(y, row * ldy + c);
            if (PIPED || alpha) {
                o.a = Vec<VEC>::load(alpha + (int64_t)tc * C + c);
                o.b = Vec<VEC>::load(beta + (int64_t)tc * C + c);
            }
            if (PIPED ? ADD : addend != nullptr) o.ad = VecS<VEC, SB>::load_last(addend, row * ld_add + c);
            return o;
        };
        StepOps sq[kPrefetch > 0 ? kPrefetch : 1];
        if constexpr (kPrefetch > 0) {
#pragma unroll
            for (int k = 0; k < kPrefetch; ++k) sq[k] = fetch_step(k);
        }
        [[maybe_unused]] V o_keep;
        for (int t = 0; t < T; ++t) {
            const int64_t row = (int64_t)t * M + m;
            if (SAVE == 2 && NEURON == SNN_NEURON_LIF && (t % kCkpt) == 0) {
                float* ck = vdec + ((int64_t)(t / kCkpt) * 2 * M + m) * C + c;
                Vec<VEC>::store(ck, v);
                Vec<VEC>::store(ck + M * C, i);
            }
            StepOps cur;
            if constexpr (kPrefetch > 0) {
                cur = sq[0];
#pragma unroll
                for (int k = 0; k + 1 < kPrefetch; ++k) sq[k] = sq[k + 1];
                sq[kPrefetch - 1] = fetch_step(t + kPrefetch);
// ... 34 lines not shown
                        c_mem = lane<VEC>(cmv, j);
                        c_syn = lane<VEC>(csv, j);
                    }
                    float dv = c_mem * ((p.v_leak - vj) + i_new);
                    float v_dec = vj + dv;
                    float di = c_syn * i_new;
                    lane<VEC>(i, j) = i_new + di;
                    if (NEURON == SNN_NEURON_LIF) {
                        float u = v_dec - p.v_th;
                        float z = (u > 0.0f) ? 1.0f : 0.0f;
                        lane<VEC>(v, j) = (1.0f - z) * v_dec + z * p.v_reset;
                        lane<VEC>(o, j) = z;
                        lane<VEC>(vd, j) = v_dec;
                    } else {
                        lane<VEC>(v, j) = v_dec;
                        lane<VEC>(o, j) = (NEURON == SNN_NEURON_LI_TANH) ? tanhf(v_dec) : v_dec;
                    }
                }
            }
            if (PIPED ? ADD : addend != nullptr) {
#pragma unroll
                for (int j = 0; j < VEC; ++j) lane<VEC>(o, j) += lane<VEC>(cur.ad, j);
            }
            if constexpr (LAST) {
                o_keep = o;
            } else if constexpr (!NOOUT) {
                if (PIPED || !last_only) VecS<VEC, SB>::store(out, row * ldo + c, o);
                else if (t == T - 1) VecS<VEC, SB>::store(out, m * ldo + c, o);
            }
            if (SAVE == 1 && (NEURON == SNN_NEURON_LIF || NEURON == SNN_NEURON_SLI || NEURON == SNN_NEURON_SYNAPSE)) {
                if constexpr (VEC == 4 && !SB && SNN_SCAN_NT_AUX != 0) __builtin_nontemporal_store(vd, reinterpret_cast<f32x4*>(vdec + row * C + c));
                else VecS<VEC, SB>::store(vdec, row * C + c, vd);
            }
        }
        if constexpr (LAST) VecS<VEC, SB>::store(out, m * ldo + c, o_keep);
        };
        if constexpr (VEC > 1 && SAVE != 2) {
            if (alpha && !last_only) {
                if (addend) time_loop(std::true_type{}, std::true_type{}, std::false_type{}, std::false_type{});
                else if (SAVE == 1 && NEURON == SNN_NEURON_LIF && !SB && out == nullptr)
                    time_loop(std::true_type{}, std::false_type{}, std::true_type{}, std::false_type{});
                else time_loop(std::true_type{}, std::false_type{}, std::false_type{}, std::false_type{});
            } else if (alpha && last_only && !addend) {
                time_loop(std::true_type{}, std::false_type{}, std::false_type{}, std::true_type{});
            } else {
                time_loop(std::false_type{}, std::false_type{}, std::false_type{}, std::false_type{});
            }
        } else {
            time_loop(std::false_type{}, std::false_type{}, std::false_type{}, std::false_type{});
        }
        if (NEURON != SNN_NEURON_NONE) {
            if (vT) Vec<VEC>::store(vT + m * C + c, v);
            if (iT) Vec<VEC>::store(iT + m * C + c, i);
        }
    }
}

struct FwdPlan {
    int vec, save;
    unsigned blocks;
};
static FwdPlan fwd_plan(int neuron, int64_t M, int C, int lanes, bool saves, bool ckpt) {
    FwdPlan fp;
    static const bool no_v8 = snn_tuning_env("SNN_SCAN_NO_VEC8") != nullptr;
    fp.vec = (lanes == 8 && no_v8) ? 4 : lanes;
    const bool step_state = neuron == SNN_NEURON_LIF || rebuilds_x(neuron);
    fp.save = (saves && step_state) ? (ckpt ? 2 : 1) : 0;
    const int64_t total = M * (C / fp.vec);
    const int64_t per_thread = snn_ceil_div(total, (int64_t)snn_max_blocks() * kThreads);
    fp.blocks = (unsigned)snn_ceil_div(total, kThreads * per_thread);
    return fp;
}
constexpr bool fwd_instance(int neuron, int vec, int save, bool sb, bool pc = false) {
    if (pc && (neuron != SNN_NEURON_LIF || sb || save == 2)) return false;
    return (sb ? (vec != 1 && bf16_neuron(neuron) && save != 2) : vec != 8) &&
           (save == 0 || neuron == SNN_NEURON_LIF || (save == 1 && rebuilds_x(neuron)));
}

}

static int neuron_fwd(int neuron, const float* y, int64_t ldy, const float* alpha, const float* beta, const float* v0,
                      const float* i0, float* out, int64_t ldo, const float* addend, int64_t ld_addend, float* vT,
                      float* iT, float* vdec, bool ckpt, int T, int64_t M, int C, const snn_neuron_params* p,
                      int flags, void* stream, const float* cmem_pc = nullptr, const float* csyn_pc = nullptr) {
    const bool pc = cmem_pc != nullptr;
    const char* const fn = pc ? "snn_lif_tau_fwd" : "snn_affine_neuron_fwd";
    SNN_REQUIRE((flags & ~(SNN_SCAN_LAST_STEP_ONLY | SNN_SCAN_BF16_STORAGE | SNN_SCAN_SPIKES_FROM_VDEC)) == 0,
                "%s: unknown flags 0x%x", fn, flags);
    const int last_only = (flags & SNN_SCAN_LAST_STEP_ONLY) != 0;
    const bool sb = (flags & SNN_SCAN_BF16_STORAGE) != 0;
    const bool no_out = (flags & SNN_SCAN_SPIKES_FROM_VDEC) != 0;
    SNN_REQUIRE(y && p && (out || no_out), "%s: null pointer", fn);
    if (no_out) {
        SNN_REQUIRE(neuron == SNN_NEURON_LIF && vdec && !ckpt && !addend && !last_only && !sb && alpha && !out &&
                        multiples(4, {C, ldy}) && aligned(16, {y, vdec}),
                    "%s: SNN_SCAN_SPIKES_FROM_VDEC is for Norm -> LIF with saved potentials, no shortcut, "
                    "all T steps, fp32 tensors, 4-channel groups; out must be NULL", fn);
        ldo = C;
    }
    SNN_REQUIRE(!last_only || (last_step_neuron(neuron) && !addend),
                "%s: SNN_SCAN_LAST_STEP_ONLY is for LIF / LI / LI+Tanh without a shortcut", fn);
    SNN_REQUIRE(!addend || (ld_addend >= C && neuron != SNN_NEURON_LI_TANH),
                "%s: addend needs ld_addend >= C and is not allowed with LI_TANH", fn);
    SNN_REQUIRE(T > 0 && M > 0 && C > 0 && ldy >= C && ldo >= C, "%s: bad shape", fn);
    SNN_REQUIRE((alpha == nullptr) == (beta == nullptr), "%s: alpha/beta must come together", fn);
    SNN_REQUIRE(neuron >= SNN_NEURON_NONE && neuron <= SNN_NEURON_SYNAPSE, "%s: bad neuron %d", fn,
                neuron);
    auto lanes_ok = [&](int n, size_t act_bytes) {
        return multiples(n, {C, ldy, ldo, addend ? ld_addend : 0}) && aligned(act_bytes, {y, out, vdec, addend}) &&
               aligned(16, {alpha, beta, v0, i0, vT, iT, cmem_pc, csyn_pc});
    };
    SNN_REQUIRE(!sb || (lanes_ok(4, 8) && !ckpt && bf16_neuron(neuron)), "%s: %s, without checkpointing", fn, kBf16Covers);
    const int lanes = sb ? (lanes_ok(8, 16) ? 8 : 4) : (lanes_ok(4, 16) ? 4 : 1);
    const FwdPlan fp = fwd_plan(neuron, M, C, lanes, vdec != nullptr, ckpt);
    const bool launched = dispatch(
        [&](auto NEURON, auto VEC, auto SAVE, auto SB, auto PC) {
            if constexpr (fwd_instance(NEURON(), VEC(), SAVE(), SB(), PC())) {
                hipLaunchKernelGGL((k_affine_neuron_fwd<NEURON(), VEC(), SAVE(), SB(), PC()>), dim3(fp.blocks), dim3(kThreads), 0,
                                   (hipStream_t)stream, y, ldy, alpha, beta, v0, i0, out, ldo, addend, ld_addend, vT, iT,
                                   vdec, T, M, C, *p, last_only, cmem_pc, csyn_pc);
                return true;
            } else {
                return false;
            }
        },
        AnyNeuron{neuron}, OneOf<1, 4, 8>{fp.vec}, OneOf<0, 1, 2>{fp.save}, Flag{sb}, Flag{pc});
    SNN_REQUIRE(launched, "%s: no kernel instance (neuron %d, vec %d, save %d)", fn, neuron, fp.vec, fp.save);
    SNN_CHECK_LAUNCH(fn);
    return 0;
}

extern "C" int snn_affine_neuron_fwd(int neuron, const float* y, int64_t ldy, const float* alpha, const float* beta,
                                     const float* v0, const float* i0, float* out, int64_t ldo, const float* addend,
                                     int64_t ld_addend, float* vT, float* iT, float* vdec, int T, int64_t M, int C,
                                     const snn_neuron_params* p, int flags, void* stream) {
    return neuron_fwd(neuron, y, ldy, alpha, beta, v0, i0, out, ldo, addend, ld_addend, vT, iT, vdec, false, T, M, C, p,
                      flags, stream);
}

extern "C" int snn_lif_ckpt_interval(void) { return kCkpt; }

extern "C" int snn_lif_fwd_ckpt(const float* y, int64_t ldy, const float* alpha, const float* beta, const float* v0,
                                const float* i0, float* out, int64_t ldo, const float* addend, int64_t ld_addend,
                                float* vT, float* iT, float* ckpt, int T, int64_t M, int C, const snn_neuron_params* p,
                                void* stream) {
    SNN_REQUIRE(ckpt, "snn_lif_fwd_ckpt: null checkpoint buffer");
    return neuron_fwd(SNN_NEURON_LIF, y, ldy, alpha, beta, v0, i0, out, ldo, addend, ld_addend, vT, iT, ckpt, true, T, M,
                      C, p, 0, stream);
}

extern "C" int snn_lif_tau_fwd(int neuron, const float* y, int64_t ldy, const float* alpha, const float* beta,
                               const float* v0, const float* i0, float* out, int64_t ldo, const float* addend,
                               int64_t ld_addend, float* vT, float* iT, float* vdec, int T, int64_t M, int C,
                               const snn_neuron_params* p, const float* c_mem, const float* c_syn, int flags, void* stream) {
    SNN_REQUIRE(neuron == SNN_NEURON_LIF && !(flags & SNN_SCAN_BF16_STORAGE), "snn_lif_tau_fwd: %s (neuron %d, flags 0x%x)",
                kTauCovers, neuron, flags);
    SNN_REQUIRE(c_mem && c_syn, "snn_lif_tau_fwd: null time constants");
    return neuron_fwd(neuron, y, ldy, alpha, beta, v0, i0, out, ldo, addend, ld_addend, vT, iT, vdec, false, T, M, C, p,
                      flags & ~SNN_SCAN_WIDE_ADDRESSING, stream, c_mem, c_syn);
}
```

snn_for_object_detection_amd/functional.py:

```python

import collections
import ctypes
import os
from typing import List, NamedTuple, Optional, Sequence, Tuple

import torch
from torch.autograd import Function

from . import _hip
from ._hip import NeuronParams

_F32 = torch.float32
DEFAULT_DT = 0.001


SURROGATES = {"super": _hip.SURR_SUPER, "triangle": _hip.SURR_TRIANGLE, "sigmoid": _hip.SURR_SIGMOID,
              "atan": _hip.SURR_ATAN}


def _surrogate_code(surrogate: str) -> int:
    if surrogate not in SURROGATES:
        raise ValueError(f"unknown surrogate {surrogate!r}: one of {sorted(SURROGATES)}")
    return SURROGATES[surrogate]

# ... 453 lines not shown

    def __init__(self, buf: torch.Tensor):
        self.buf = buf
        self.written = False

    def claim(self) -> int:
        acc = 1 if self.written else 0
        self.written = True
        return acc


_NBT_BATCH = None


def begin_counter_batch() -> None:
    global _NBT_BATCH
    _NBT_BATCH = []


def flush_counter_batch() -> None:
    global _NBT_BATCH
    pending, _NBT_BATCH = _NBT_BATCH, None
    if pending:
        by_inc = {}
        for t, inc in pending:
            by_inc.setdefault(inc, []).append(t)
        for inc, tensors in by_inc.items():
            torch._foreach_add_(tensors, inc)


FUSE_OUTER_ADDEND = not os.environ.get("SNN_NO_OUTER_ADDEND")
USE_SIBLING_FUSION = not os.environ.get("SNN_NO_SIBLING_FUSION")
USE_SPIKES_FROM_VDEC = not os.environ.get("SNN_NO_SPIKES_FROM_VDEC")


class GradAccumulator:

    __slots__ = ("deposits", "result", "fused", "outer", "exclusive", "grad_in_slot")

    def __init__(self):
        self.deposits = {}
        self.result = None
        self.fused = {}
        self.outer = None
        self.exclusive = set()
        self.grad_in_slot = False

    def deposit(self, key, g: torch.Tensor, exclusive: bool = False) -> None:
        if self.result is None and g is not None:
            self.deposits[key] = g
            if exclusive:
                self.exclusive.add(key)

    def set_result(self, dx: torch.Tensor) -> None:
        self.result = dx


def _acc_of(x):
    return getattr(x, "_snn_acc", None)


def _same_tensor(a: torch.Tensor, b: torch.Tensor) -> bool:
    return (a.data_ptr() == b.data_ptr() and tuple(a.shape) == tuple(b.shape) and a.stride() == b.stride())


def _slot_of(param) -> Optional[GradSlot]:
# ... 317 lines not shown
            else:
                _copy_cl(g, dst)
            off += c
        return out, None


def split_channels(x: torch.Tensor, widths: Sequence[int]) -> List[torch.Tensor]:
    return list(_SplitChannels.apply(x, tuple(int(c) for c in widths)))


def _group_key(w1: torch.Tensor, w2s: Sequence[torch.Tensor]) -> Tuple[int, ...]:
    return (id(w1),) + tuple(id(w) for w in w2s)


def _group_versions(w1: torch.Tensor, w2s: Sequence[torch.Tensor]) -> Tuple[int, ...]:
    return tuple(w._version for w in w2s) + (w1._version,)


def _kept_product(w1: torch.Tensor, w2s: Sequence[torch.Tensor], shape: Tuple[int, int]):
    kept = getattr(w2s[0], "_snn_sibling_weight", None)
    entry = kept.get(_group_key(w1, w2s)) if kept is not None else None
    if entry is None:
        return None
    k1, k2s, versions, wc, wct = entry
    if (k1 is w1 and all(a is b for a, b in zip(k2s, w2s)) and versions == _group_versions(w1, w2s)
            and tuple(wc.shape) == shape):
        return wc, wct
    return None


class _SiblingConv1x1(Function):

    @staticmethod
    def forward(ctx, x, w1, dest, acc, prec, slot1, slots2, x_th, *w2s):
        _require_device(x, "conv2d input", bf16_ok=True)
        fwd_prec, bwd_prec = _conv_precs(prec, x.dtype == _BF16)
        T, B, Cin, H, W = _dims5(x)
        C1 = w1.shape[0] if w1 is not None else Cin
        widths = [int(w.shape[0]) for w in w2s]
        Ct = sum(widths)
        for w in w2s:
            if w.shape[1] != C1 or tuple(w.shape[2:]) != (1, 1):
                raise RuntimeError("sibling 1x1 convolutions: weight shapes do not match the input")
        if w1 is not None and (w1.shape[1] != Cin or tuple(w1.shape[2:]) != (1, 1)):
            raise RuntimeError("sibling 1x1 convolutions: the composed weight does not chain")
        x = _raw_to_cl(x)
        w1m = None if w1 is None else w1.detach().reshape(C1, Cin).contiguous()
        w2ms = [w.detach().reshape(c, C1).contiguous() for w, c in zip(w2s, widths)]
        need_t = ctx.needs_input_grad[0]
        kept = _kept_product(w1, w2s, (Ct, Cin)) if w1 is not None else None
        if kept is not None:
            wc, wct = kept
        else:
            if w1 is not None and all(getattr(w, "_snn_wt", None) is not None for w in (w1, *w2s)):
                if getattr(w2s[0], "_snn_sibling_group", None) is None:
                    w2s[0]._snn_sibling_group = {}
                w2s[0]._snn_sibling_group[_group_key(w1, w2s)] = (w1, tuple(w2s))
            wc = torch.empty((Ct, Cin), device=x.device, dtype=_F32)
            wct = torch.empty((Cin, Ct), device=x.device, dtype=_F32) if need_t else None
            row = 0
            for w2m, c in zip(w2ms, widths):
                if w1m is not None:
                    _small_gemm(w2m, False, w1m, False, wc[row:row + c], 0, ct=wct, ct_col=row)
                else:
                    wc[row:row + c].copy_(w2m)
                row += c
            if w1m is None and need_t:
                wct.copy_(wc.t())
        y = _out_tensor(dest, T, B, Ct, H, W, x)
        x, x_th = _spikes_fwd_operand(x, x_th, lambda: _spikes_fwd_ok(
            _hip.query("snn_conv1x1_spikes_supported", T * B, H, W, Cin, Ct, cl_stride(x), fwd_prec, bwd_prec), False,
            x.data_ptr(), wc.data_ptr()))
        if x_th is not None:
            _hip.call("snn_conv1x1_spikes_fwd", x.data_ptr(), cl_stride(x), x_th, wc.data_ptr(), y.data_ptr(), cl_stride(y),
                      T * B, H, W, Cin, Ct, _stream())
        else:
            _hip.call("snn_conv2d_fwd", x.data_ptr(), cl_stride(x), wc.data_ptr(), None, y.data_ptr(), cl_stride(y), T * B,
                      H, W, Cin, H, W, Ct, 1, 1, 1, 0, None, 0, None, 0, None, fwd_prec, _stream())
        ctx.prec = bwd_prec
        ctx.x_th = x_th
        ctx.save_for_backward(x, w1m, *w2ms)
        ctx.wct = wct
        ctx.geom = (T, B, Cin, H, W, Ct, 1, 1, H, W, 1, 0)
        ctx.widths, ctx.c1 = widths, C1
        ctx.slot1, ctx.slots2 = slot1, slots2
        ctx.acc = acc
        return y

    @staticmethod
    def backward(ctx, gy):
        x, w1m, *w2ms = ctx.saved_tensors
        T, B, Cin, H, W, Ct = ctx.geom[:6]
        C1, widths = ctx.c1, ctx.widths
        composed = w1m is not None
        gy = _raw_to_cl(gy)
        ldg, ldx = cl_stride(gy), cl_stride(x)
        dx = dw1 = None
        dw2s = [None] * len(widths)
        if ctx.needs_input_grad[0]:
            dx = _dgrad_accumulate(ctx.acc, gy, ldg, ctx.wct, x, ctx.geom, _stream(), ctx.prec)
        if any(ctx.needs_input_grad[8:]) or (composed and ctx.needs_input_grad[1]):
            slot1, slots2 = ctx.slot1, ctx.slots2
            slotted = all(s_ is not None for s_ in slots2) and (slot1 is not None or not composed)
            splitk = _hip.query("snn_conv2d_wgrad_splitk", T * B, H, W, Cin, H, W, Ct, 1, 1, 1, 0, ctx.prec)
            xw, ldxw, x_th = _spikes_wgrad_operand(x, ldx, ctx.x_th, gy, ldg)
            with _WgradLaunch(x.device, slotted, splitk, Ct, Cin, hold=(x, xw, gy), with_g=True) as (stream, ws, G):
                if x_th is not None:
                    _hip.call("snn_conv1x1_spikes_wgrad", xw.data_ptr(), ldxw, x_th, gy.data_ptr(), ldg, G.data_ptr(),
                              T * B, H, W, Cin, Ct, 0, ws.data_ptr(), splitk, stream)
                else:
                    _hip.call("snn_conv2d_wgrad", xw.data_ptr(), ldxw, gy.data_ptr(), ldg, G.data_ptr(), T * B, H, W,
                              Cin, H, W, Ct, 1, 1, 1, 0, 0, ws.data_ptr(), splitk, ctx.prec, stream)
                g1 = None
                if composed:
                    g1 = slot1.buf.view(C1, Cin) if slotted else torch.empty((C1, Cin), device=x.device, dtype=_F32)
                    acc1 = slot1.claim() if slotted else 0
                row = 0
                for b, (w2m, c) in enumerate(zip(w2ms, widths)):
                    Gb = G[row:row + c]
                    row += c
                    if slotted:
                        g2, acc2 = slots2[b].buf.view(c, C1), slots2[b].claim()
                    else:
                        g2, acc2 = torch.empty((c, C1), device=x.device, dtype=_F32), 0
                    if composed:
                        _small_gemm(Gb, False, w1m, True, g2, acc2)
                        _small_gemm(w2m, True, Gb, False, g1, acc1)
                        acc1 = 1
                    elif acc2:
                        g2.add_(Gb)
                    else:
                        g2.copy_(Gb)
                    if not slotted:
                        dw2s[b] = g2.view(c, C1, 1, 1)
                if composed and not slotted:
                    dw1 = g1.view(C1, Cin, 1, 1)
        return (dx, dw1, None, None, None, None, None, None, *dw2s)


def sibling_conv1x1(x: torch.Tensor, w1: Optional[torch.Tensor], w2s: Sequence[torch.Tensor], dest: Optional[Dest] = None,
                    forward_precision: Optional[str] = None, backward_precision: Optional[str] = None) -> torch.Tensor:
    return _SiblingConv1x1.apply(x, w1, dest, _acc_of(x), _prec_codes(forward_precision, backward_precision),
                                 _slot_of(w1), tuple(_slot_of(w) for w in w2s), getattr(x, "_snn_spike_threshold", None),
                                 *w2s)


def composed_conv1x1(x: torch.Tensor, w1: torch.Tensor, w2: torch.Tensor, dest: Optional[Dest] = None,
                     forward_precision: Optional[str] = None, backward_precision: Optional[str] = None) -> torch.Tensor:
    if x.dtype == _BF16 and (w1.shape[1] % 32 or w2.shape[0] % 32):
        y = to_bfloat16(composed_conv1x1(to_float32(x), w1, w2, None, forward_precision, backward_precision))
        return place(y, dest) if dest is not None else y
    seq, single = as_sequence(x)
    y = _SiblingConv1x1.apply(seq, w1, dest, _acc_of(seq), _prec_codes(forward_precision, backward_precision),
                              _slot_of(w1), (_slot_of(w2),), None, w2)
    return y[0] if single else y


class BnPartial(NamedTuple):
    partial: torch.Tensor
    chunks: int
    rows_per_chunk: int
    data_ptr: int
    dims: Tuple[int, int, int]


def conv2d(x: torch.Tensor, weight: torch.Tensor, stride: int = 1, padding: int = 0, dest: Optional[Dest] = None,
           forward_precision: Optional[str] = None, backward_precision: Optional[str] = None,
           bn_stats: bool = False) -> torch.Tensor:
    if x.dtype == _BF16 and (weight.shape[1] % 32 or weight.shape[0] % 32):
        y = to_bfloat16(conv2d(to_float32(x), weight, stride, padding, None, forward_precision, backward_precision, False))
        return place(y, dest) if dest is not None else y
    x_th = getattr(x, "_snn_spike_threshold", None)
    seq, single = as_sequence(x)
    bn_out = [] if bn_stats else None
    y = _Conv2d.apply(seq, weight, int(stride), int(padding), _slot_of(weight), dest, _acc_of(seq),
                      _prec_codes(forward_precision, backward_precision), bn_out, x_th)
    y = y[0] if single else y
    if bn_out:
        y._snn_bn_partial = bn_out[0]
    if bn_stats and not single and _slot_of(weight) is not None and _wgrad_bn_ok(seq, weight, int(stride), int(padding)):
        y._snn_defer_apply = True
    return y


class NeuronState(NamedTuple):
    v: torch.Tensor
    i: torch.Tensor
# ... 64 lines not shown
                  mean.data_ptr(), invstd.data_ptr(), gx.data_ptr(), y.data_ptr(), ldy, raw_local.data_ptr(), st)
    else:
        _hip.call("snn_bn_bwd_reduce", sums.data_ptr(), T, M, C, raw_local.data_ptr(), st)
    raw = raw_local.clone()
    dist.all_reduce(raw, op=dist.ReduceOp.SUM, group=sync_group[0])
    param_sums = torch.empty((T, C, 2), device=y.device, dtype=torch.float64)
    _hip.call("snn_bn_bwd_coef", raw.data_ptr(), raw_local.data_ptr(), param_sums.data_ptr(), T, M * world,
              C, _ptr(gamma), mean.data_ptr(), invstd.data_ptr(), coef[0].data_ptr(), coef[1].data_ptr(),
              coef[2].data_ptr(), dg_ptr, db_ptr, acc_flag, st)


def _ptr_at(t: Optional[torch.Tensor], offset: int) -> Optional[int]:
    return None if t is None else t.data_ptr() + offset


class _NeuronCfg(NamedTuple):
    neuron: int
    has_bn: bool
    training: bool
    eps: float
    momentum: float
    running_mean: Optional[torch.Tensor]
    running_var: Optional[torch.Tensor]
    params: NeuronParams
    g_slot: Optional[GradSlot]
    b_slot: Optional[GradSlot]
    dest: Optional[Dest]
    sync_group: object
    bn_hint: object
    last_only: bool
    defer_apply: bool
    spikes_out: Optional[list]
    tau_slots: Tuple[Optional[GradSlot], Optional[GradSlot]]


def _bf16_scan_covers(neuron: int, channels: int) -> bool:
    return neuron in (_hip.NEURON_NONE, _hip.NEURON_LIF, _hip.NEURON_LI, _hip.NEURON_LI_TANH) and channels % 4 == 0


def _takes_checkpointed_pair(neuron: int, nbytes: int, params: NeuronParams, last_only: bool, sb: bool, tau: bool) -> bool:
    return (neuron == _hip.NEURON_LIF and LIF_CHECKPOINT_BYTES is not None and not last_only and not sb
            and nbytes >= LIF_CHECKPOINT_BYTES and default_gradient_rule(params) and not tau)


def _grad_pair(slots, needed, n: int, dev):
    if not any(needed):
        return None, None, 0, None, None
    if all(s_ is not None or not need for s_, need in zip(slots, needed)):
        acc = 1 if (slots[0] or slots[1]).written else 0
        for s_ in slots:
            if s_ is not None:
                s_.claim()
        pa, pb = (s_.buf.data_ptr() if (s_ is not None and need) else None for s_, need in zip(slots, needed))
        return pa, pb, acc, None, None
    fa, fb = (torch.empty((n,), device=dev, dtype=_F32) if need else None for need in needed)
    return _ptr(fa), _ptr(fb), 0, fa, fb


class _AffineNeuron(Function):

    @staticmethod
    def forward(ctx, y, gamma, bias, v0, i0, addend, cfg, w_mem=None, w_syn=None):
        neuron, has_bn, params, dest, sync_group, last_only = (cfg.neuron, cfg.has_bn, cfg.params, cfg.dest, cfg.sync_group,
                                                               cfg.last_only)
        _require_device(y, "norm/neuron input", bf16_ok=True)
        sb = y.dtype == _BF16
# ... 63 lines not shown
        if neuron in _SAVES_STEP and need_grad:
            ckpt = ckpt_pair
            if ckpt:
                k = _hip.query("snn_lif_ckpt_interval")
                vdec = torch.empty(((T + k - 1) // k, 2, B, H, W, C), device=dev, dtype=_F32)
            else:
                vdec = torch.empty((T, B, H, W, C), device=dev, dtype=y.dtype)
        if v0 is not None:
            v0 = _expand_state(v0, (B, C, H, W), dev)
        if i0 is not None:
            i0 = _expand_state(i0, (B, C, H, W), dev)
        ctx.addend_acc = None
        ad_ptr, ld_ad = None, 0
        if addend is not None:
            if neuron == _hip.NEURON_LI_TANH:
                raise RuntimeError("a fused shortcut is not supported after LI+Tanh (its backward reads the output)")
            ctx.addend_acc = _acc_of(addend)
            addend = _raw_to_cl(addend)
            if tuple(addend.shape) != (T, B, C, H, W):
                raise RuntimeError("Residual merge: branch outputs differ in shape")
            if addend.dtype != y.dtype:
                raise RuntimeError("Residual merge: shortcut and branch are stored in different types (fp32 / bf16)")
            ad_ptr, ld_ad = addend.data_ptr(), cl_stride(addend)
        if ckpt:
            _hip.call("snn_lif_fwd_ckpt", y.data_ptr(), ldy, _ptr(alpha), _ptr(beta), _ptr(v0), _ptr(i0),
                      out.data_ptr(), cl_stride(out), ad_ptr, ld_ad, _ptr(vT), _ptr(iT), vdec.data_ptr(), T, M, C,
                      params, st)
        else:
            head = (neuron, y.data_ptr(), ldy, _ptr(alpha), _ptr(beta), _ptr(v0), _ptr(i0),
                    _ptr(out), C if out is None else cl_stride(out), ad_ptr, ld_ad, _ptr(vT) if has_state else None,
                    _ptr(iT) if has_state else None, _ptr(vdec), T, M, C, params)
            fwd_flags = ((_hip.SCAN_LAST_STEP_ONLY if last_only else 0) | sb_flag
                         | (_hip.SCAN_SPIKES_FROM_VDEC if no_out else 0))
            if tau:
                _hip.call("snn_lif_tau_fwd", *head, c_mem.data_ptr(), c_syn.data_ptr(), fwd_flags, st)
            else:
                _hip.call("snn_affine_neuron_fwd", *head, fwd_flags, st)
            if no_out:
                out = _alias(vdec, vdec.storage_offset(), T, B, C, H, W, C)
                spikes_out.append(float(params.v_th))
        ctx.ckpt = ckpt
        ctx.sb = sb
        ctx.defer_apply = cfg.defer_apply
        ctx.last_only = last_only
        ctx.cfg = (neuron, has_bn, use_running, NeuronParams.from_buffer_copy(params), (T, B, C, H, W))
        ctx.slots = (cfg.g_slot, cfg.b_slot)
        ctx.tau = tau
        ctx.tau_slots = cfg.tau_slots
        ctx.tau_n = w_mem.numel() if tau else 0
        ctx.sync_group = sync_group if (has_bn and not use_running) else None
        ctx.has_v0 = v0 is not None
        ctx.has_i0 = i0 is not None
        if neuron == _hip.NEURON_LI_TANH and need_grad and not is_channels_last(out):
            raise RuntimeError("LI+Tanh output placed in a concat slice is not supported for training")
        state = vdec if neuron in _SAVES_STEP else (out if neuron == _hip.NEURON_LI_TANH else None)
        ctx.save_for_backward(y, gamma, mean, invstd, alpha, beta, state, bias if has_bn else None, c_mem, c_syn,
                              v0 if (tau and need_grad) else None)
        if not has_state:
            ctx.mark_non_differentiable(vT, iT)
        if sb and last_only:
            out = _raw_convert(out, _F32)
        return out, vT, iT

    @staticmethod
    def backward(ctx, g_out, g_vT, g_iT):
        y, gamma, mean, invstd, alpha, beta, state, bn_bias, c_mem, c_syn, v0_saved = ctx.saved_tensors
        neuron, has_bn, use_running, params, (T, B, C, H, W) = ctx.cfg
        M = B * H * W
        st = _stream()
        dev = y.device
        has_state = neuron != _hip.NEURON_NONE
        g_addend = None
        if g_out is not None and ctx.needs_input_grad[5]:
# ... 127 lines not shown

def affine_neuron_bwd_plan(neuron: int, T: int, M: int, C: int, ldg: int, ldy: int, with_sums: bool, flags: int = 0,
                           params: Optional[NeuronParams] = None) -> BwdPlan:
    out = (ctypes.c_int64 * 10)()
    _hip.call("snn_affine_neuron_bwd_plan", neuron, T, M, C, ldg, ldy, int(bool(with_sums)), params or neuron_params(),
              flags, ctypes.addressof(out))
    return BwdPlan(*out)


class TauBwdPlan(NamedTuple):
    scan: BwdPlan
    ordered: int
    lds_bytes: int


def lif_tau_bwd_plan(T: int, M: int, C: int, ldg: int, ldy: int, with_sums: bool, with_tau_sums: bool = True, flags: int = 0,
                     params: Optional[NeuronParams] = None, neuron: int = _hip.NEURON_LIF) -> TauBwdPlan:
    out = (ctypes.c_int64 * 12)()
    _hip.call("snn_lif_tau_bwd_plan", neuron, T, M, C, ldg, ldy, int(bool(with_sums)), int(bool(with_tau_sums)),
              params or neuron_params(), flags, ctypes.addressof(out))
    return TauBwdPlan(BwdPlan(*out[:10]), int(out[10]), int(out[11]))


def _expand_state(s: torch.Tensor, shape, dev) -> torch.Tensor:
    s = s.detach()
    if s.dim() == 0 or tuple(s.shape) != tuple(shape):
        s = s.to(device=dev, dtype=_F32).expand(shape)
    return _raw_dense_cl(s)


def affine_neuron(y: torch.Tensor, neuron: int, state: Optional[NeuronState] = None, bn=None,
                  params: Optional[NeuronParams] = None, dest: Optional[Dest] = None,
                  addend: Optional[torch.Tensor] = None, last_only: bool = False, spikes_ok: bool = False,
                  tau: Optional[Tuple[torch.Tensor, torch.Tensor]] = None):
    if y.dtype == _BF16 and not _bf16_scan_covers(neuron, y.shape[-3]):
        if tau is not None:
            _tau_refusal(neuron, True)
        out, new_state = affine_neuron(to_float32(y), neuron, state, bn, params, None,
                                       None if addend is None else to_float32(addend), last_only, False)
        out = out if (last_only and y.dim() == 5) else to_bfloat16(out)
        return (place(out, dest) if dest is not None else out), new_state
    bn_hint = getattr(y, "_snn_bn_partial", None)
    defer_apply = bool(getattr(y, "_snn_defer_apply", False))
    seq, single = as_sequence(y)
    if addend is not None:
        acc = _acc_of(addend)
        addend, _ = as_sequence(addend)
        if acc is not None:
            addend._snn_acc = acc
    params = params or neuron_params()
    has_bn = bn is not None
    gamma = bias = rm = rv = None
    training, eps, momentum = False, 1e-5, 0.1
    if has_bn:
        gamma, bias = bn.weight, bn.bias
        training = bn.training or (bn.running_mean is None and bn.running_var is None)
        rm, rv = bn.running_mean, bn.running_var
        eps = bn.eps
        if bn.momentum is None:
            raise RuntimeError("cumulative-average BatchNorm (momentum=None) is not supported")
        momentum = bn.momentum
        if training and seq.shape[1] * seq.shape[3] * seq.shape[4] <= 1:
            raise ValueError("Expected more than 1 value per channel when training, got input size "
                             f"{torch.Size((seq.shape[1], seq.shape[2], seq.shape[3], seq.shape[4]))}")
        if training and bn.num_batches_tracked is not None:
            if _NBT_BATCH is not None:
                _NBT_BATCH.append((bn.num_batches_tracked, int(seq.shape[0])))
            else:
                bn.num_batches_tracked.add_(seq.shape[0])
    v0 = i0 = None
    if state is not None:
        if neuron == _hip.NEURON_SYNAPSE:
            (v0,) = state
        else:
            v0, i0 = state
    sync_group = getattr(bn, "_snn_sync_group", None) if has_bn else None
    spikes_out = [] if (spikes_ok and not single and dest is None and addend is None) else None
    w_mem, w_syn = tau if tau is not None else (None, None)
    cfg = _NeuronCfg(neuron=neuron, has_bn=has_bn, training=training, eps=float(eps), momentum=float(momentum),
                     running_mean=rm, running_var=rv, params=params, g_slot=_slot_of(gamma), b_slot=_slot_of(bias), dest=dest,
                     sync_group=sync_group, bn_hint=bn_hint, last_only=bool(last_only) and not single,
                     defer_apply=defer_apply, spikes_out=spikes_out, tau_slots=(_slot_of(w_mem), _slot_of(w_syn)))
    out, vT, iT = _AffineNeuron.apply(seq, gamma, bias, v0, i0, addend, cfg, w_mem, w_syn)
    if spikes_out:
        out._snn_spike_threshold = spikes_out[0]
    if neuron == _hip.NEURON_NONE:
        new_state = None
    elif neuron == _hip.NEURON_SYNAPSE:
        new_state = SynapseState(vT)
    else:
        new_state = NeuronState(vT, iT)
    if last_only and not single:
        return out, new_state
    return (out[0] if single else out), new_state


def _copy_cl(src: torch.Tensor, dst: torch.Tensor) -> None:
    if src.dtype != dst.dtype:
        raise RuntimeError("merge: operands are stored in different types (fp32 / bf16 storage mixed)")
    T, B, C, H, W = _dims5(src)
    _hip.call("snn_copy_channels_bf16" if src.dtype == _BF16 else "snn_copy_channels", src.data_ptr(), cl_stride(src),
              dst.data_ptr(), cl_stride(dst), T * B * H * W, C, _stream())


def _add_cl(a: torch.Tensor, b: torch.Tensor, dst: torch.Tensor) -> None:
    if not (a.dtype == b.dtype == dst.dtype):
        raise RuntimeError("merge: operands are stored in different types (fp32 / bf16 storage mixed)")
    T, B, C, H, W = _dims5(a)
    _hip.call("snn_add_bf16" if a.dtype == _BF16 else "snn_add", a.data_ptr(), cl_stride(a), b.data_ptr(), cl_stride(b),
              dst.data_ptr(), cl_stride(dst), T * B * H * W, C, _stream())


class _Concat(Function):

    @staticmethod
    def forward(ctx, dest, *xs):
        xs = [_raw_to_cl(x) for x in xs]
        T, B, _, H, W = _dims5(xs[0])
# ... 651 lines not shown
```

snn_for_object_detection_amd/generator.py:

```python

import inspect
import os
from typing import Any, List, Optional, Tuple, Union

import torch
from torch import nn

from . import _hip
from . import functional as HF
from .anchors import AnchorGenerator
from .layer_gen import *
from .layer_gen import (ConvLSTM, Dense, HipBatchNorm2d, HipConv2d, HipReLU, HipSiLU, HipTanh, LayerGen,
                        LICell, LIFCell, Residual, Return, SLICell, StateStorage, Storage, SumPool2d, SynapseCell)

ListGen = List[Union[LayerGen, "ListGen"]]
ListState = List[Union[torch.Tensor, None, "ListState"]]


def _is_module_stateful(m: nn.Module) -> bool:
    return "state" in inspect.signature(m.forward).parameters


def _neuron_cell(layer: nn.Module) -> Optional[nn.Module]:
    cell = layer.module if isinstance(layer, StateStorage) else layer
# ... 200 lines not shown
                pending = siblings[b]
            for k, (kind, idx, span) in enumerate(plan):
                if siblings is not None and k == 0:
                    continue
                last = k == len(plan) - 1
                step_dest = branch_dest if last else None
                step_promise, pending = pending, None
                if zero_copy and not last:
                    nkind, nidx, _ = plan[k + 1]
                    nxt = branch[nidx]
                    if nkind == "layer" and isinstance(nxt, BlockGen) and nxt._pass_offset is not None:
                        parent = branch_dest if (k + 1 == len(plan) - 1) else None
                        pending = HF.ConcatPromise(nxt.out_channels, parent=parent)
                        step_dest = HF.Dest(pending, nxt._pass_offset, nxt.in_channels)
                layer = branch[idx]
                if kind == "norm_neuron":
                    holder = branch[idx + 1]
                    cell = _neuron_cell(holder)
                    neuron = cell.kind
                    if span == 3:
                        neuron = _hip.NEURON_LI_TANH
                    old = branch_state[idx + 1]
                    direct = step_dest if neuron != _hip.NEURON_LI_TANH else None
                    shortcut = None
                    if fuse_here and last:
                        direct, shortcut = dest, inputs[self._fused_shortcut[1]]
                    only_last = (last_only and last and zero_copy and len(self.net) == 1 and direct is None
                                 and shortcut is None
                                 and neuron in (_hip.NEURON_LIF, _hip.NEURON_LI, _hip.NEURON_LI_TANH)
                                 and not (getattr(cell, "tau", None) is not None and torch.is_grad_enabled()
                                          and any(w.requires_grad for w in cell.tau))
                                 and not (isinstance(holder, StateStorage) and not self.training))
                    nxt_l = branch[plan[k + 1][1]] if (not last and plan[k + 1][0] == "layer") else None
                    spikes_ok = (zero_copy and not last and self.training and neuron == _hip.NEURON_LIF
                                 and direct is None and shortcut is None and not isinstance(holder, StateStorage)
                                 and HF.USE_SPIKES_FROM_VDEC
                                 and ((plan[k + 1][0] == "conv_block" and branch[plan[k + 1][1] + 1]._siblings is not None
                                       and HF.USE_SIBLING_FUSION)
                                      or (isinstance(nxt_l, HipConv2d) and nxt_l.in_channels % 32 == 0
                                          and nxt_l.out_channels % 4 == 0 and nxt_l.kernel_size[0] <= 5
                                          and nxt_l.forward_precision is None and nxt_l.backward_precision is None)))
                    Y, new = HF.affine_neuron(Y, neuron, old, bn=layer, params=cell.params, dest=direct,
                                              addend=shortcut, last_only=only_last, spikes_ok=spikes_ok,
                                              tau=getattr(cell, "tau", None))
                    if isinstance(holder, StateStorage):
                        holder.record(old, Y, new)
                    branch_state[idx + 1] = new
                elif kind == "conv_block":
                    blk = branch[idx + 1]
                    Y, branch_state[idx + 1] = blk(Y, branch_state[idx + 1], dest=step_dest, promise=step_promise,
                                                   pre_conv=layer)
                elif isinstance(layer, BlockGen):
                    Y, branch_state[idx] = layer(Y, branch_state[idx], dest=step_dest, promise=step_promise,
                                                 last_only=last_only and last and len(self.net) == 1)
                elif isinstance(layer, HipConv2d) and pre_conv is not None and k == 0:
                    Y = HF.composed_conv1x1(Y, pre_conv.weight, layer.weight, dest=step_dest,
                                            forward_precision=pre_conv.forward_precision or layer.forward_precision,
                                            backward_precision=(pre_conv.backward_precision
                                                                or layer.backward_precision))
                elif isinstance(layer, HipConv2d):
                    feeds_bn = False
                    if not last and plan[k + 1][0] == "norm_neuron" and Y.is_cuda:
                        bn = branch[plan[k + 1][1]]
                        feeds_bn = bn.training or (bn.running_mean is None and bn.running_var is None)
                    Y = layer(Y, dest=step_dest, bn_stats=feeds_bn)
                elif isinstance(layer, (LIFCell, LICell, SLICell, SynapseCell)):
                    Y, branch_state[idx] = layer(Y, branch_state[idx], dest=step_dest)
                elif flags[idx]:
                    Y, branch_state[idx] = layer(Y, branch_state[idx])
                else:
                    Y = layer(Y)
                if step_dest is not None:
                    Y = HF.place(Y, step_dest)
            if branch_dest is not None and not plan:
                Y = HF.place(Y, branch_dest)
            out.append(Y)
            out_state.append(branch_state)
# ... 186 lines not shown
```

snn_for_object_detection_amd/profiler.py:

```python

from collections import defaultdict
from typing import Dict

import torch


WGRAD_LABELS = ("k_conv_wgrad_pipe", "k_conv_wgrad_halo", "k_conv_first<wgrad>")


def _wgrad_label(n, h, w, cin, ho, wo, cout, kh, kw, stride, pad, prec) -> str:
    from . import _hip
    return WGRAD_LABELS[int(_hip.query("snn_conv2d_wgrad_kernel", n, h, w, cin, ho, wo, cout, kh, kw, stride, pad, prec))]


def _conv_label(name: str, a) -> str:
    if name == "snn_conv2d_wgrad":
        return _wgrad_label(a[5], a[6], a[7], a[8], a[9], a[10], a[11], a[12], a[13], a[14], a[15], a[19])
    dgrad = name == "snn_conv2d_dgrad"
    cin, cout = a[8], a[11]
    oc, ic = (cin, cout) if dgrad else (cout, cin)
    if not dgrad and cin == 2 and a[12] == 3 and a[13] == 3 and cout % 4 == 0 and (cout // 4) & (cout // 4 - 1) == 0 \
            and cout <= 256 and a[16] is None:
        return "k_conv_first<2, 3, false>"
    if oc <= 32:
# ... 4 lines not shown
        tile = "128, 2, 2"
    return f"k_conv_gather<{tile}, {'true' if dgrad else 'false'}, {'true' if ic % 4 == 0 else 'false'}>"


PREC_BF16S, SCAN_BF16_STORAGE = 6, 4


def work_of(name: str, a):
    if name in ("snn_conv2d_fwd", "snn_conv2d_dgrad"):
        a = tuple(a[:3]) + tuple(a[4:])
        n, h, w, cin, ho, wo, cout, kh, kw = a[5], a[6], a[7], a[8], a[9], a[10], a[11], a[12], a[13]
        sb = a[21 if name == "snn_conv2d_fwd" else 20] == PREC_BF16S
        es = 2.0 if sb else 4.0
        es_in = 4.0 if (cin == 2 and name == "snn_conv2d_fwd") else es
        flops = 2.0 * n * ho * wo * cout * kh * kw * cin
        byts = es_in * n * h * w * cin + es * n * ho * wo * cout + 4.0 * cout * kh * kw * cin
        return _conv_label(name, a) + (", bf16s" if sb else ""), flops, byts
    if name == "snn_conv2d_wgrad":
        n, h, w, cin, ho, wo, cout, kh, kw = a[5], a[6], a[7], a[8], a[9], a[10], a[11], a[12], a[13]
        sb = a[19] == PREC_BF16S
        es = 2.0 if sb else 4.0
        flops = 2.0 * n * ho * wo * cout * kh * kw * cin
        byts = (4.0 if cin == 2 else es) * n * h * w * cin + es * n * ho * wo * cout + 4.0 * cout * kh * kw * cin
        return _conv_label(name, a) + (", bf16s" if sb else ""), flops, byts
    if name in ("snn_conv1x1_spikes_fwd", "snn_conv1x1_spikes_wgrad"):
        fwd = name.endswith("_fwd")
        n, h, w, cin, cout = (a[6], a[7], a[8], a[9], a[10])
        flops = 2.0 * n * h * w * cout * cin
        byts = 4.0 * (n * h * w * cin + n * h * w * cout + cout * cin)
        if not fwd:
            return WGRAD_LABELS[0], flops, byts
        tile = "32, 4, 1" if cout <= 32 else ("64, 2, 2" if cout <= 64 else "128, 2, 2")
        return f"k_conv_gather<{tile}, false, true>", flops, byts
    if name in ("snn_conv2d_spikes_fwd", "snn_conv2d_spikes_wgrad"):
        fwd = name.endswith("_fwd")
        n, h, w, cin, ho, wo, cout, kh, kw, stride, pad = a[6:17]
        flops = 2.0 * n * ho * wo * cout * kh * kw * cin
        byts = 4.0 * (n * h * w * cin + n * ho * wo * cout + cout * kh * kw * cin)
        if not fwd:
            return _wgrad_label(n, h, w, cin, ho, wo, cout, kh, kw, stride, pad, 1) + ", spikes", flops, byts
        tile = "32, 4, 1" if cout <= 32 else ("64, 2, 2" if cout <= 64 else "128, 2, 2")
        return f"k_conv_gather<{tile}, false, true>", flops, byts
    if name == "snn_conv3x3_halo_spikes":
        n, h, w, cin, cout = a[6], a[7], a[8], a[9], a[10]
        flops = 2.0 * n * h * w * cout * 9 * cin
        byts = 4.0 * (n * h * w * cin + n * h * w * cout) + 4.0 * cout * 9 * cin
        return f"k_conv_halo3<{128 if cout % 128 == 0 else (64 if cout % 64 == 0 else 32)}, fwd, spikes>", flops, byts
    if name == "snn_conv3x3_halo":
        n, h, w, cin, cout, prec = a[5], a[6], a[7], a[8], a[9], a[17]
        es = 2.0 if prec == PREC_BF16S else 4.0
        flops = 2.0 * n * h * w * cout * 9 * cin
        byts = es * (n * h * w * cin + n * h * w * cout) + 4.0 * cout * 9 * cin
        kind = "fwd" if prec == 4 else ("dgrad" if prec == 1 else "bf16s")
        return f"k_conv_halo3<{128 if cout % 128 == 0 else (64 if cout % 64 == 0 else 32)}, {kind}>", flops, byts
    if name == "snn_conv3x3_s2_dgrad":
        n, h, w, cin, ho, wo, cout = a[5], a[6], a[7], a[8], a[9], a[10], a[11]
        sb = a[16] == PREC_BF16S
        flops = 2.0 * n * ho * wo * cout * 9 * cin
        byts = (2.0 if sb else 4.0) * (n * h * w * cin + n * ho * wo * cout) + 4.0 * cout * 9 * cin
        return "k_conv_s2dgrad3<dgrad>" + (", bf16s" if sb else ""), flops, byts
    if name == "snn_conv2d_wgrad_bn":
        n, h, w, cin, ho, wo, cout, kh, kw = a[10], a[11], a[12], a[13], a[14], a[15], a[16], a[17], a[18]
        flops = 2.0 * n * ho * wo * cout * kh * kw * cin
        byts = 4.0 * (n * h * w * cin + 2 * n * ho * wo * cout + cout * kh * kw * cin)
        return WGRAD_LABELS[2], flops, byts
    if name == "snn_affine_neuron_fwd":
        neuron, T, M, C = a[0], a[14], a[15], a[16]
        last_only = bool(a[18] & 2)
        elems = float(T) * M * C
        wrote_out = 0 if a[7] is None else (1.0 / T if last_only else 1)
        tensors = 1 + wrote_out + (1 if a[13] is not None else 0) + (1 if a[9] is not None else 0)
        sb = bool(a[18] & SCAN_BF16_STORAGE)
        return f"k_affine_neuron_fwd<{neuron}>" + (", bf16s" if sb else ""), 12.0 * elems, (2.0 if sb else 4.0) * elems * tensors
    if name == "snn_affine_neuron_bwd":
        neuron, T, M, C = a[0], a[15], a[16], a[17]
        last_only = bool(a[19] & 2)
        elems = float(T) * M * C
        one = 1.0 / T if last_only else 1
        saved = 0 if a[3] is None else (one if neuron == 3 else 1)
        from_state = bool(a[19] & 16)
        tensors = one + 1 + saved + (1 if (a[14] is not None and not from_state) else 0)
        sb = bool(a[19] & SCAN_BF16_STORAGE)
        return f"k_affine_neuron_bwd<{neuron}>" + (", bf16s" if sb else ""), 16.0 * elems, (2.0 if sb else 4.0) * elems * tensors
    if name == "snn_lif_fwd_ckpt":
        T, M, C = a[13], a[14], a[15]
        elems = float(T) * M * C
        return "k_affine_neuron_fwd<1,ckpt>", 12.0 * elems, 4.0 * elems * (2.5 + (1 if a[8] is not None else 0))
    if name == "snn_lif_bwd_ckpt":
        T, M, C = a[14], a[15], a[16]
        elems = float(T) * M * C
        return "k_lif_bwd_ckpt", 28.0 * elems, 4.0 * elems * 3.5
    if name == "snn_convlstm_seq_fwd":
        T, M, Cin, Ch = a[9], a[10], a[11], a[12]
        px = float(T) * M
        saved = 5 * Ch if a[7] is not None else 0
        return "k_lstm_seq_fwd", 2.0 * px * 4 * Ch * (Cin + Ch), 4.0 * (px * (Cin + Ch + saved) + 4 * Ch * (Cin + Ch))
    if name == "snn_convlstm_seq_bwd":
        T, M, Cin, Ch = a[12], a[13], a[14], a[15]
        px = float(T) * M
        moved = 5 * Ch + 4 * Ch + (Ch if a[4] is not None else 0) + (Cin if a[8] is not None else 0)
        return "k_lstm_seq_bwd", 2.0 * px * 4 * Ch * (Cin + Ch), 4.0 * (px * moved + 4 * Ch * (Cin + Ch))
    if name in ("snn_bn_stats", "snn_bn_stats_bf16"):
        T, M, C = a[2], a[3], a[4]
        sb = name.endswith("_bf16")
        return "k_bn_stats" + (", bf16s" if sb else ""), 3.0 * T * M * C, (2.0 if sb else 4.0) * T * M * C
    if name in ("snn_bn_bwd_apply", "snn_bn_bwd_apply_bf16"):
        T, M, C = a[8], a[9], a[10]
        sb = name.endswith("_bf16")
        return "k_bn_bwd_apply" + (", bf16s" if sb else ""), 4.0 * T * M * C, (6.0 if sb else 12.0) * T * M * C
    if name in ("snn_copy_channels", "snn_add_channels"):
        M, C = a[4], a[5]
        return "k_channels", 0.0, (8.0 if name == "snn_copy_channels" else 12.0) * M * C
    if name == "snn_add":
        return "k_add", float(a[6]) * a[7], 12.0 * a[6] * a[7]
    if name in ("snn_nchw_to_nhwc", "snn_nhwc_to_nchw"):
        n = float(a[2]) * a[3] * a[4] * a[5]
        return "k_layout", 0.0, 8.0 * n
    if name == "snn_adamax_step":
        return "k_adamax", 8.0 * a[4], 28.0 * a[4]
    if name == "snn_adamax_step_ctl":
        return "k_adamax_ctl", 12.0 * a[4], 28.0 * a[4]
    if name == "snn_grad_norm":
        return "k_grad_norm", 2.0 * a[1], 4.0 * a[1]
    return name, 0.0, 0.0


class KernelProfiler:

    def __init__(self):
        self.records = []
        self.neuron_steps = 0.0

    def before(self, name, args):
        label, flops, byts = work_of(name, args)
        if name in ("snn_affine_neuron_fwd", "snn_lif_fwd_ckpt"):
            self.neuron_steps += flops / 12.0
        start = torch.cuda.Event(enable_timing=True)
        end = torch.cuda.Event(enable_timing=True)
        start.record()
        return (label, flops, byts, start, end)

    def after(self, token):
        token[4].record()
        self.records.append(token)

    def summary(self) -> Dict[str, dict]:
        torch.cuda.synchronize()
        agg = defaultdict(lambda: {"calls": 0, "ms": 0.0, "flops": 0.0, "bytes": 0.0})
        for label, flops, byts, start, end in self.records:
            row = agg[label]
            row["calls"] += 1
            row["ms"] += start.elapsed_time(end)
            row["flops"] += flops
            row["bytes"] += byts
        for row in agg.values():
            sec = max(row["ms"], 1e-9) * 1e-3
            row["avg_us"] = 1e3 * row["ms"] / row["calls"]
            row["tflops"] = row["flops"] / sec / 1e12
            row["gbs"] = row["bytes"] / sec / 1e9
        return dict(agg)
```

Before: 7225.

## Emit packed spike bit masks from LIF forward for sibling 1x1 convs

The LIF forward scan can now also write a packed one-bit-per-channel spike mask. Sibling 1x1 convolutions consume that mask directly, expanding the bits to fp16 operands in registers instead of loading fp32 potentials and thresholding them. The aim is to cut the activation bytes the 1x1 GEMM forward and wgrad read by a large factor. The cost is an extra mask write in the scan plus new kernel variants. SCAN_SPIKE_MASK reuses the value 32 already taken by SCAN_STATE_LOOKBACK, so the two flags could collide.

```diff
diff --git a/include/snn_hip.h b/include/snn_hip.h
--- a/include/snn_hip.h
+++ b/include/snn_hip.h
@@ -27,7 +27,8 @@
        SNN_SCAN_BF16_STORAGE = 4,
        SNN_SCAN_SPIKES_FROM_VDEC = 8,
        SNN_SCAN_SUMS_FROM_STATE = 16,
-       SNN_SCAN_STATE_LOOKBACK = 32   };
+       SNN_SCAN_STATE_LOOKBACK = 32,
+       SNN_SCAN_SPIKE_MASK = 32       };
 
 enum { SNN_POOL_AVG = 0, SNN_POOL_MAX = 1, SNN_POOL_SUM = 2 };
 
@@ -124,6 +125,14 @@
                             int H, int W, int Cin, int Cout, double* bn_partial, int frames_per_step, int* bn_layout,
                             void* stream);
 
+int snn_conv1x1_mask_supported(int64_t N, int H, int W, int Cin, int Cout, const uint32_t* mask, int64_t ld_mask,
+                               const float* w, const float* y, int64_t ldy, const float* dy, int64_t lddy, const float* dw,
+                               int fwd_precision, int bwd_precision);
+int snn_conv1x1_mask_fwd(const uint32_t* mask, int64_t ld_mask, const float* w, float* y, int64_t ldy, int64_t N, int H, int W,
+                         int Cin, int Cout, void* stream);
+int snn_conv1x1_mask_wgrad(const uint32_t* mask, int64_t ld_mask, const float* dy, int64_t lddy, float* dw, int64_t N, int H,
+                           int W, int Cin, int Cout, int accumulate, float* workspace, int splitk, void* stream);
+
 size_t snn_bn_stats_partial_size(int T, int64_t M, int C);
 int snn_bn_stats(const float* y, int64_t ldy, int T, int64_t M, int C, double* partial, void* stream);
 int snn_bn_stats_finalize(const double* partial, int chunks, int rows_per_chunk, int T, int64_t M, int C,
@@ -145,6 +154,10 @@
                           float* out, int64_t ldo, const float* addend, int64_t ld_addend,
                           float* vT, float* iT, float* vdec,
                           int T, int64_t M, int C, const snn_neuron_params* p, int flags, void* stream);
+int snn_affine_neuron_fwd_mask(int neuron, const float* y, int64_t ldy, const float* alpha, const float* beta,
+                               const float* v0, const float* i0, float* out, int64_t ldo, const float* addend,
+                               int64_t ld_addend, float* vT, float* iT, float* vdec, int T, int64_t M, int C,
+                               const snn_neuron_params* p, int flags, void* stream, uint32_t* mask, int64_t ld_mask);
 
 size_t snn_affine_neuron_bwd_sums_size(int T, int64_t M, int C);
 int snn_affine_neuron_bwd_sums_from_state(int neuron, int T, int64_t M, int C, int64_t ldg, const snn_neuron_params* p,
diff --git a/snn_for_object_detection_amd/_hip.py b/snn_for_object_detection_amd/_hip.py
--- a/snn_for_object_detection_amd/_hip.py
+++ b/snn_for_object_detection_amd/_hip.py
@@ -13,6 +13,7 @@
 PREC_FP32, PREC_BF16X3, PREC_BF16X6, PREC_FP16X3, PREC_BF16X1, PREC_BF16S = 0, 1, 3, 4, 5, 6
 SCAN_WIDE_ADDRESSING, SCAN_LAST_STEP_ONLY, SCAN_BF16_STORAGE, SCAN_SPIKES_FROM_VDEC, SCAN_SUMS_FROM_STATE = 1, 2, 4, 8, 16
 SCAN_STATE_LOOKBACK = 32
+SCAN_SPIKE_MASK = 32
 SURR_SUPER, SURR_TRIANGLE, SURR_SIGMOID, SURR_ATAN = 0, 1, 2, 3
 
 
@@ -66,6 +67,9 @@
     "snn_conv1x1_spikes_supported": (c_int, [_L, _I, _I, _I, _I, _L, _I, _I]),
     "snn_conv1x1_spikes_fwd": (c_int, [_P, _L, _F, _P, _P, _L, _L, _I, _I, _I, _I, _P]),
     "snn_conv1x1_spikes_wgrad": (c_int, [_P, _L, _F, _P, _L, _P, _L, _I, _I, _I, _I, _I, _P, _I, _P]),
+    "snn_conv1x1_mask_supported": (c_int, [_L, _I, _I, _I, _I, _P, _L, _P, _P, _L, _P, _L, _P, _I, _I]),
+    "snn_conv1x1_mask_fwd": (c_int, [_P, _L, _P, _P, _L, _L, _I, _I, _I, _I, _P]),
+    "snn_conv1x1_mask_wgrad": (c_int, [_P, _L, _P, _L, _P, _L, _I, _I, _I, _I, _I, _P, _I, _P]),
     "snn_conv2d_spikes_supported": (c_int, [_L, _I, _I, _I, _I, _I, _I, _I, _I, _I, _I, _L, _I, _I]),
     "snn_conv2d_spikes_fwd": (c_int, [_P, _L, _F, _P, _P, _L, _L, _I, _I, _I, _I, _I, _I, _I, _I, _I, _I, _P, _I, _P, _P]),
     "snn_conv2d_spikes_wgrad": (c_int, [_P, _L, _F, _P, _L, _P, _L, _I, _I, _I, _I, _I, _I, _I, _I, _I, _I, _I, _P, _I, _P]),
@@ -79,6 +83,8 @@
     "snn_bn_bwd_coef": (c_int, [_P, _P, _P, _I, _L, _I, _P, _P, _P, _P, _P, _P, _P, _P, _I, _P]),
     "snn_affine_neuron_fwd": (c_int, [_I, _P, _L, _P, _P, _P, _P, _P, _L, _P, _L, _P, _P, _P, _I, _L, _I,
                                       POINTER(NeuronParams), _I, _P]),
+    "snn_affine_neuron_fwd_mask": (c_int, [_I, _P, _L, _P, _P, _P, _P, _P, _L, _P, _L, _P, _P, _P, _I, _L, _I,
+                                           POINTER(NeuronParams), _I, _P, _P, _L]),
     "snn_lif_ckpt_interval": (c_int, []),
     "snn_lif_fwd_ckpt": (c_int, [_P, _L, _P, _P, _P, _P, _P, _L, _P, _L, _P, _P, _P, _I, _L, _I,
                                  POINTER(NeuronParams), _P]),
diff --git a/snn_for_object_detection_amd/csrc/conv_common.h b/snn_for_object_detection_amd/csrc/conv_common.h
--- a/snn_for_object_detection_amd/csrc/conv_common.h
+++ b/snn_for_object_detection_amd/csrc/conv_common.h
@@ -73,3 +73,6 @@
 int snn_first_layer_blocks(int64_t rows, int num_cu);
 int snn_launch_first(bool wgrad, bool bnapply, bool sb, int blocks, size_t lds, const float* x, const float* w,
                      const float* dy, float* out, const FirstGeom& fg, void* stream, const char* name);
+
+bool snn_wgrad_mask_ok(int64_t N, int H, int W, int Cin, int Cout, const uint32_t* mask, int64_t ld_mask, const float* dy,
+                       int64_t lddy, const float* dw);
diff --git a/snn_for_object_detection_amd/csrc/conv_gather.hip b/snn_for_object_detection_amd/csrc/conv_gather.hip
--- a/snn_for_object_detection_amd/csrc/conv_gather.hip
+++ b/snn_for_object_detection_amd/csrc/conv_gather.hip
@@ -80,7 +80,7 @@
 }
 
 template <int BN, int WM, int WN, bool DGRAD, bool VEC, int SPLIT, bool FAST, bool PRESPLIT = false, bool SB = false,
-          bool XSP = false>
+          bool XSP = false, bool XM = false>
 __global__ __launch_bounds__(kThreads, (FAST && SPLIT) ? (PRESPLIT ? 3 : (SB ? (DGRAD ? 4 : SNN_GATHER_SB_WAVES) : 2)) : SNN_CONV_MIN_WAVES) void k_conv_gather(const float* __restrict__ in, const float* __restrict__ wk,
                                                           float* __restrict__ out, ConvGeom g,
                                                           const float* __restrict__ addend, int64_t ld_add,
@@ -91,6 +91,7 @@
     static_assert(WM * WN == 4, "4 waves");
     static_assert(!SB || (FAST && SPLIT == 5 && !PRESPLIT), "bf16 storage: the pipelined one-product kernel");
     static_assert(!XSP || (FAST && SPLIT == 4 && !DGRAD && !PRESPLIT && !SB), "spikes from potentials: fp16 x 3 forward");
+    static_assert(!XM || XSP, "spike bit mask: an instance of the spikes-from-potentials kernel");
     constexpr int ES = SB ? 2 : 4;
     constexpr int NPIECE = SPLIT == 3 ? 3 : (SPLIT == 5 ? 1 : 2);
     constexpr int A_BYTES = SPLIT ? NPIECE * BM * LDB * 2 : BM * LDK * 4;
@@ -167,7 +168,7 @@
         }
     };
 
-    using AReg = typename std::conditional<SB, u32x2, f32x4>::type;
+    using AReg = typename std::conditional<SB, u32x2, typename std::conditional<XM, unsigned, f32x4>::type>::type;
     AReg ra[4];
     f32x4 rb[BROWS];
 
@@ -175,7 +176,21 @@
     int a_rel[4];
     unsigned a_mask[4];
     unsigned b_rel[BROWS];
-    if (FAST) {
+    [[maybe_unused]] int xm_rel[TM];
+    if constexpr (XM) {
+        rs_a = __builtin_amdgcn_make_buffer_rsrc(const_cast<float*>(in), 0, (int)(g.Mtot * g.ldi * 4), 0x00020000);
+        rs_b = __builtin_amdgcn_make_buffer_rsrc(const_cast<float*>(wk), 0, g.OC * g.KtotFull * 4, 0x00020000);
+#pragma unroll
+        for (int i = 0; i < TM; ++i) {
+            const int64_t m = m0 + (wm * TM + i) * 32 + r;
+            xm_rel[i] = m < g.Mtot ? (int)(m * g.ldi * 4) : -1;
+        }
+#pragma unroll
+        for (int j = 0; j < BROWS; ++j) {
+            const int n = n0 + lr + 32 * j;
+            b_rel[j] = n < g.OC ? (unsigned)(n * g.KtotFull + kq) * 4u : 0x80000000u;
+        }
+    } else if (FAST) {
         const int ow_ = DGRAD ? g.OWc : g.OW, oh_ = DGRAD ? g.OHc : g.OH;
         const int64_t img0 = (unsigned)m0 / (unsigned)(oh_ * ow_);
         const int64_t ipix = (int64_t)g.IH * g.IW;
@@ -226,7 +241,13 @@
             wcol0 = ((g.kh0 + g.stride * th) * g.KW + (g.kw0 + g.stride * tw)) * g.IC + c0;
         }
         const int tbit = kin ? tap : 31;
-        if (which & 1) {
+        if constexpr (XM) {
+            if (which & 1) {
+#pragma unroll
+                for (int i = 0; i < TM; ++i)
+                    ra[i] = (unsigned)__builtin_amdgcn_raw_buffer_load_b32(rs_a, (kin && xm_rel[i] >= 0) ? xm_rel[i] + (k0n >> 5) * 4 : -1, 0, 0);
+            }
+        } else if (which & 1) {
 #pragma unroll
             for (int j = 0; j < 4; ++j) {
                 const int voff = ((a_mask[j] >> tbit) & 1u) ? a_rel[j] + toff : -1;
@@ -247,7 +268,7 @@
             load_tiles_fast(k0, ra, rb);
             return;
         }
-        if constexpr (!SB) {
+        if constexpr (!SB && !XM) {
         const int kk = k0 + kq;
         if (VEC) {
             const bool kin = kk < g.Ktot;
@@ -318,7 +339,7 @@
         *reinterpret_cast<bf16x4*>(&lo_img[row * LDB + kq]) = lo;
     };
     auto store_tiles = [&]() {
-        if constexpr (SB) return;
+        if constexpr (SB || XM) return;
         else if (SPLIT) {
 #pragma unroll
             for (int j = 0; j < 4; ++j) split_store(ra[j], Ah, Am, Al, lr + 32 * j);
@@ -388,6 +409,7 @@
         };
         auto convert_a = [&](const AReg& v, bf16x4* out) {
             if constexpr (SB) out[0] = __builtin_bit_cast(bf16x4, v);
+            else if constexpr (XM) return;
             else if constexpr (XSP) {
                 u32x2 hi;
 #pragma unroll
@@ -405,9 +427,20 @@
                 convert(v, out, kF16WeightScale);
             }
         };
+        [[maybe_unused]] unsigned xm_cur[TM];
+        auto xm_expand = [&](unsigned word, int sel) {
+            const unsigned b = (word >> (8 * sel)) & 0xffu;
+            u32x4 d;
+#pragma unroll
+            for (int q = 0; q < 4; ++q) {
+                const unsigned v = (b >> (2 * q)) & 3u;
+                d[q] = ((v | (v << 15)) & 0x00010001u) * 0x4C00u;
+            }
+            return __builtin_bit_cast(bf16x8, d);
+        };
         auto write_tiles = [&]() {
 #pragma unroll
-            for (int j = 0; j < 4; ++j) {
+            for (int j = 0; j < (XM ? 0 : 4); ++j) {
                 const int o = (lr + 32 * j) * LDB + kq;
                 *reinterpret_cast<bf16x4*>(&Ah[o]) = pa[j][0];
                 if constexpr (NP >= 2 && !XSP) *reinterpret_cast<bf16x4*>(&Al[o]) = pa[j][1];
@@ -426,6 +459,10 @@
 #pragma unroll
             for (int i = 0; i < TM; ++i) {
                 const int off = ((wm * TM + i) * 32 + r) * LDB + ks * 16 + 8 * h;
+                if constexpr (XM) {
+                    ah[i] = xm_expand(xm_cur[i], 2 * ks + h);
+                    continue;
+                }
                 ah[i] = *reinterpret_cast<const bf16x8*>(&Ah[off]);
                 if constexpr (NP >= 2 && !XSP) al[i] = *reinterpret_cast<const bf16x8*>(&Al[off]);
                 if constexpr (NP >= 3) am[i] = *reinterpret_cast<const bf16x8*>(&Am[off]);
@@ -471,15 +508,19 @@
                 }
         };
         constexpr int NM = TM * TN * (XSP ? 2 : NPROD);
-        constexpr int NREAD = XSP ? TM + TN * NP : (TM + TN) * NP;
+        constexpr int NREAD = XM ? TN * NP : (XSP ? TM + TN * NP : (TM + TN) * NP);
         constexpr int CONV_OPS = SPLIT == 3 ? 24 : (SPLIT == 5 ? 2 : 14);
-        constexpr int VPG_A = ((XSP ? 4 * 8 : 4 * CONV_OPS) + NM - 1) / NM;
+        constexpr int VPG_A = ((XM ? TM * 18 : (XSP ? 4 * 8 : 4 * CONV_OPS)) + NM - 1) / NM;
         constexpr int VPG_B = PRESPLIT ? 1 : (BROWS * CONV_OPS + NM - 1) / NM;
         if (g.Ktot > 0) {
             AReg ra0[4];
             f32x4 rb0[BROWS];
             load_tiles_fast(0, ra0, rb0);
             load_tiles_fast(BK, ra, rb);
+            if constexpr (XM) {
+#pragma unroll
+                for (int i = 0; i < TM; ++i) xm_cur[i] = ra0[i];
+            }
 #pragma unroll
             for (int j = 0; j < 4; ++j) convert_a(ra0[j], pa[j]);
 #pragma unroll
@@ -516,6 +557,10 @@
             }
             __builtin_amdgcn_sched_barrier(0);
             STAMP(1);
+            if constexpr (XM) {
+#pragma unroll
+                for (int i = 0; i < TM; ++i) xm_cur[i] = ra[i];
+            }
             load_tiles_fast(k0 + 2 * BK, ra, rb);
             STAMP(2);
             __syncthreads();
@@ -719,7 +764,7 @@
 #endif
 }
 
-enum GatherLoader { kLoadScalar = 0, kLoadVec = 1, kLoadFast = 2, kLoadFastPresplit = 3, kLoadSB = 4, kLoadXSP = 5 };
+enum GatherLoader { kLoadScalar = 0, kLoadVec = 1, kLoadFast = 2, kLoadFastPresplit = 3, kLoadSB = 4, kLoadXSP = 5, kLoadXM = 6 };
 enum GatherRefusal { kGatherOk = 0, kGatherTooManyPixels, kGatherNotFastSB, kGatherNotFastXSP, kGatherGridTooLarge };
 struct GatherPlan {
     int ok, why;
@@ -730,9 +775,9 @@
     int64_t blocks;
 };
 static GatherPlan gather_plan(const ConvGeom& g, bool dgrad, int split, bool sb, bool xsp, unsigned align, bool has_split,
-                              bool has_add, bool has_add2) {
+                              bool has_add, bool has_add2, bool xm = false) {
     GatherPlan p = {};
-    const bool vec = (g.IC % 4 == 0) && (g.ldi % 4 == 0) && (align & (sb ? kAlignIn8 : kAlignIn16)) && (align & kAlignW16);
+    const bool vec = (g.IC % 4 == 0) && (xm || g.ldi % 4 == 0) && (align & (sb ? kAlignIn8 : kAlignIn16)) && (align & kAlignW16);
     const int64_t gm = snn_ceil_div(g.Mtot, BM);
     if (!(g.Mtot < 0x7fffffffLL && (int64_t)g.IH * g.IW < 0x7fffffffLL)) {
         p.why = kGatherTooManyPixels;
@@ -742,7 +787,8 @@
     const int ntaps = nth * ntw;
     static const bool no_fast = snn_tuning_env("SNN_CONV_NO_FAST") != nullptr;
     const bool fast = vec && !no_fast && g.IC % BK == 0 && ntaps >= 1 && ntaps <= 31 && nth <= 6 && ntw <= 6 &&
-                      (int64_t)g.IH * g.IW * g.ldi * 16 < 0x7fffffffLL && (int64_t)g.OC * g.KtotFull * 4 < 0x7fffffffLL;
+                      (int64_t)g.IH * g.IW * g.ldi * 16 < 0x7fffffffLL && (int64_t)g.OC * g.KtotFull * 4 < 0x7fffffffLL &&
+                      (!xm || (ntaps == 1 && g.stride == 1 && g.pad == 0 && g.ldi * 32 >= g.IC && g.Mtot * g.ldi * 4 < 0x7fffffffLL));
     p.out_vec = (g.ldo % 4 == 0) && (align & (sb ? kAlignOut8 : kAlignOut16)) &&
                 (!has_add || (align & (sb ? kAlignAdd8 : kAlignAdd16))) &&
                 (!has_add2 || (align & (sb ? kAlignAdd2_8 : kAlignAdd2_16)));
@@ -755,7 +801,7 @@
         return p;
     }
     const bool presplit = has_split && (split == 2 || split == 4) && (align & kAlignSplit16);
-    p.loader = sb ? kLoadSB : xsp ? kLoadXSP : (fast && presplit) ? kLoadFastPresplit : fast ? kLoadFast : vec ? kLoadVec : kLoadScalar;
+    p.loader = sb ? kLoadSB : xm ? kLoadXM : xsp ? kLoadXSP : (fast && presplit) ? kLoadFastPresplit : fast ? kLoadFast : vec ? kLoadVec : kLoadScalar;
     p.bn = g.OC <= 32 ? 32 : (g.OC <= 64 ? 64 : 128);
     p.mtiles = (int)gm;
     p.mtiles_per_xcd = (int)snn_ceil_div(gm, 8);
@@ -790,10 +836,11 @@
 
 static int launch_gather(bool dgrad, int split, bool sb, bool xsp, const float* in, const float* wk, const void* wk_split,
                          float* out, const ConvGeom& g, const float* addend, int64_t ld_add, const float* addend2,
-                         int64_t ld_add2, hipStream_t st, const char* name) {
-    const GatherPlan p = gather_plan(g, dgrad, split, sb, xsp,
-                                     gather_align_bits(in, wk, wk_split, out, addend, ld_add, addend2, ld_add2),
-                                     wk_split != nullptr, addend != nullptr, addend2 != nullptr);
+                         int64_t ld_add2, hipStream_t st, const char* name, bool xm = false) {
+    unsigned align = gather_align_bits(in, wk, wk_split, out, addend, ld_add, addend2, ld_add2);
+    if (xm) align = (align & ~(kAlignIn16 | kAlignIn8)) | (aligned(4, {in}) ? kAlignIn16 : 0u);
+    const GatherPlan p = gather_plan(g, dgrad, split, sb, xsp, align, wk_split != nullptr, addend != nullptr,
+                                     addend2 != nullptr, xm);
     SNN_REQUIRE(p.why != kGatherTooManyPixels, "%s: too many pixels", name);
     SNN_REQUIRE(p.why != kGatherNotFastSB, "%s: bf16 storage covers the pipelined implicit GEMM only (channels a multiple of 32, pixel "
                 "stride a multiple of 4, 8-byte aligned tensors): %d channels, stride %lld", name, g.IC, (long long)g.ldi);
@@ -811,17 +858,17 @@
         [&](auto BN, auto L, auto DGRAD, auto SPLIT) {
             constexpr int l = L(), s = SPLIT();
             constexpr bool vec = l != kLoadScalar, fast = l >= kLoadFast, pre = l == kLoadFastPresplit, sbl = l == kLoadSB,
-                           xspl = l == kLoadXSP;
+                           xml = l == kLoadXM, xspl = l == kLoadXSP || xml;
             constexpr int ksplit = fast ? s : (vec ? (s == 4 ? 3 : (s == 5 ? 2 : s)) : 0);
             if constexpr ((DGRAD() ? s != 3 && s != 4 : s != 2) && (!sbl || s == 5) && (!xspl || (!DGRAD() && s == 4)) &&
                           (!pre || s == 2 || s == 4)) {
-                hipLaunchKernelGGL((k_conv_gather<BN(), gather_wm(BN()), gather_wn(BN()), DGRAD(), vec, ksplit, fast, pre, sbl, xspl>),
+                hipLaunchKernelGGL((k_conv_gather<BN(), gather_wm(BN()), gather_wn(BN()), DGRAD(), vec, ksplit, fast, pre, sbl, xspl, xml>),
                                    grid, dim3(kThreads), 0, st, in, wsrc, out, gg, addend, ld_add, addend2, ld_add2);
                 return true;
             }
             return false;
         },
-        OneOf<32, 64, 128>{p.bn}, OneOf<0, 1, 2, 3, 4, 5>{p.loader}, Flag{dgrad}, OneOf<0, 2, 3, 4, 5>{split});
+        OneOf<32, 64, 128>{p.bn}, OneOf<0, 1, 2, 3, 4, 5, 6>{p.loader}, Flag{dgrad}, OneOf<0, 2, 3, 4, 5>{split});
     SNN_CHECK_LAUNCH(name);
     return 0;
 }
@@ -1115,3 +1162,40 @@
                                       int64_t N, int H, int W, int Cin, int Cout, void* stream) {
     return snn_conv2d_spikes_fwd(vdec, ld, v_th, w, y, ldy, N, H, W, Cin, H, W, Cout, 1, 1, 1, 0, nullptr, 0, nullptr, stream);
 }
+
+namespace {
+static bool mask_fwd_ok(int64_t N, int H, int W, int Cin, int Cout, const uint32_t* mask, int64_t ld_mask, const float* w,
+                        const float* y, int64_t ldy) {
+    if (!(N > 0 && H > 0 && W > 0 && Cin > 0 && Cout > 0 && Cin % 32 == 0 && ld_mask >= Cin / 32 && ldy >= Cout &&
+          N * (int64_t)H * W < 0x7fffffffLL && (int64_t)Cin * Cin < 0xffffffffLL && mask && w && y))
+        return false;
+    const ConvGeom g = gather_fwd_geom(N, H, W, Cin, H, W, Cout, 1, 1, 1, 0, ld_mask, ldy);
+    unsigned align = gather_align_bits(mask, w, nullptr, y, nullptr, 0, nullptr, 0) & ~(kAlignIn16 | kAlignIn8);
+    if (aligned(4, {mask})) align |= kAlignIn16;
+    const GatherPlan p = gather_plan(g, false, 4, false, true, align, false, false, false, true);
+    return p.ok && p.loader == kLoadXM;
+}
+}
+
+extern "C" int snn_conv1x1_mask_supported(int64_t N, int H, int W, int Cin, int Cout, const uint32_t* mask, int64_t ld_mask,
+                                          const float* w, const float* y, int64_t ldy, const float* dy, int64_t lddy,
+                                          const float* dw, int fwd_precision, int bwd_precision) {
+    if (fwd_precision != SNN_PREC_FP16X3 || bwd_precision != SNN_PREC_BF16X3 || !mask) return 0;
+    if (!(N > 0 && H > 0 && W > 0 && Cin > 0 && Cout > 0 && Cin % 32 == 0 && ld_mask >= Cin / 32 && aligned(4, {mask}) &&
+          N * (int64_t)H * W * ld_mask * 4 < 0x7fffffffLL))
+        return 0;
+    if ((w || y) && !mask_fwd_ok(N, H, W, Cin, Cout, mask, ld_mask, w, y, ldy)) return 0;
+    if ((dy || dw) && !snn_wgrad_mask_ok(N, H, W, Cin, Cout, mask, ld_mask, dy, lddy, dw)) return 0;
+    return 1;
+}
+
+extern "C" int snn_conv1x1_mask_fwd(const uint32_t* mask, int64_t ld_mask, const float* w, float* y, int64_t ldy, int64_t N,
+                                    int H, int W, int Cin, int Cout, void* stream) {
+    SNN_REQUIRE(mask && w && y, "snn_conv1x1_mask_fwd: null pointer");
+    if (check_conv_shape("snn_conv1x1_mask_fwd", N, H, W, Cin, H, W, Cout, 1, 1, 1, 0)) return 1;
+    SNN_REQUIRE(mask_fwd_ok(N, H, W, Cin, Cout, mask, ld_mask, w, y, ldy),
+                "snn_conv1x1_mask_fwd: call not covered (ask snn_conv1x1_mask_supported)");
+    const ConvGeom g = gather_fwd_geom(N, H, W, Cin, H, W, Cout, 1, 1, 1, 0, ld_mask, ldy);
+    return launch_gather(false, 4, false, true, reinterpret_cast<const float*>(mask), w, nullptr, y, g, nullptr, 0, nullptr, 0,
+                         (hipStream_t)stream, "snn_conv1x1_mask_fwd", true);
+}
diff --git a/snn_for_object_detection_amd/csrc/conv_wgrad.hip b/snn_for_object_detection_amd/csrc/conv_wgrad.hip
--- a/snn_for_object_detection_amd/csrc/conv_wgrad.hip
+++ b/snn_for_object_detection_amd/csrc/conv_wgrad.hip
@@ -197,7 +197,7 @@
         }
 }
 
-template <int TM, int TN, int WM, int WN, int WBK, bool ONE, bool SB = false, bool XSP = false>
+template <int TM, int TN, int WM, int WN, int WBK, bool ONE, bool SB = false, bool XSP = false, bool XM = false>
 __global__ __launch_bounds__(kThreads, 2) void k_conv_wgrad_pipe(const float* __restrict__ x,
                                                                  const float* __restrict__ dy,
                                                                  float* __restrict__ ws, WgradGeom g) {
@@ -207,6 +207,8 @@
     static_assert(WBK == 32 || WBK == 64, "stage length");
     static_assert(!SB || ONE, "bf16 storage: one product");
     static_assert(!XSP || (!ONE && !SB), "spikes from potentials: the bf16 x 3 kernel");
+    static_assert(!XM || XSP, "spike bit mask: an instance of the spikes-from-potentials kernel");
+    constexpr int XW = ((BNk / 32) * WBK + kThreads - 1) / kThreads;
     constexpr int ES = SB ? 2 : 4;
     constexpr int LDW = WBK + 8;
     constexpr int NQ = WBK / 4;
@@ -214,8 +216,9 @@
     constexpr int DQ = (DG + GPP - 1) / GPP, XQ = (XG + GPP - 1) / GPP;
     __shared__ __attribute__((aligned(16))) __bf16 Dh[BMc * LDW];
     __shared__ __attribute__((aligned(16))) __bf16 Dl[ONE ? 8 : BMc * LDW];
-    __shared__ __attribute__((aligned(16))) __bf16 Xh[BNk * LDW];
+    __shared__ __attribute__((aligned(16))) __bf16 Xh[XM ? 8 : BNk * LDW];
     __shared__ __attribute__((aligned(16))) __bf16 Xl[(ONE || XSP) ? 8 : BNk * LDW];
+    __shared__ __attribute__((aligned(16))) unsigned Xw[XM ? XW * kThreads : 4];
     __shared__ __attribute__((aligned(16))) int Pinfo[2][WBK][4];
 
     const int tid = threadIdx.x;
@@ -286,6 +289,7 @@
         d_img = (int)(im - img_lo);
     }
     auto decode = [&](int slot) {
+        if constexpr (XM) return;
         if (tid < WBK) {
             const int y0 = d_oy * g.stride - g.pad, x0 = d_ox * g.stride - g.pad;
             int4 info;
@@ -308,22 +312,38 @@
 
     using OReg = typename std::conditional<SB, u32x2, f32x4>::type;
     OReg rd[DQ][4], rx[XQ][4];
+    [[maybe_unused]] unsigned rxw[XW] = {}, pxw[XW] = {};
+    [[maybe_unused]] const int xm_pl = tid % WBK;
+    [[maybe_unused]] const int xm_word = kc0 / 32 + tid / WBK;
+    [[maybe_unused]] bool xm_ok[XW];
+#pragma unroll
+    for (int k = 0; k < XW; ++k)
+        xm_ok[k] = tid / WBK + k * (kThreads / WBK) < BNk / 32 && (xm_word + k * (kThreads / WBK)) * 32 < g.Cin;
+    if constexpr (XM)
+        rs_x = __builtin_amdgcn_make_buffer_rsrc(const_cast<float*>(x), 0, (int)(g.Mtot * g.ldx * 4), 0x00020000);
     auto load_tiles = [&](unsigned p0, int slot) {
         const int dstage = (int)(p0 - p_lo) * (int)g.lddy * ES;
         auto fetch = [&](__amdgpu_buffer_rsrc_t rs, int voff) -> OReg {
             if constexpr (SB) return __builtin_bit_cast(u32x2, __builtin_amdgcn_raw_buffer_load_b64(rs, voff, 0, 0));
             else return __builtin_bit_cast(f32x4, __builtin_amdgcn_raw_buffer_load_b128(rs, voff, 0, 0));
         };
+        if constexpr (XM) {
+            const unsigned p = p0 + (unsigned)xm_pl;
+#pragma unroll
+            for (int k = 0; k < XW; ++k)
+                rxw[k] = (unsigned)__builtin_amdgcn_raw_buffer_load_b32(
+                    rs_x, (xm_ok[k] && p < p_hi) ? (int)((p * (unsigned)g.ldx + (unsigned)(xm_word + k * (kThreads / WBK))) * 4u) : -1, 0, 0);
+        }
 #pragma unroll
         for (int e = 0; e < 4; ++e) {
-            const int4 info = *reinterpret_cast<const int4*>(&Pinfo[slot][quad * 4 + e][0]);
+            const int4 info = XM ? int4{0, 0, 0, 0} : *reinterpret_cast<const int4*>(&Pinfo[slot][quad * 4 + e][0]);
 #pragma unroll
             for (int q = 0; q < DQ; ++q) {
                 const int voff = d_off[q] < 0 ? -1 : d_off[q] + e * (int)g.lddy * ES + dstage;
                 rd[q][e] = fetch(rs_d, voff);
             }
 #pragma unroll
-            for (int q = 0; q < XQ; ++q) {
+            for (int q = 0; q < (XM ? 0 : XQ); ++q) {
                 const int iy = info.y + x_kh[q], ix = info.z + x_kw[q];
                 const bool ok = (info.w != 0) & x_ok[q] & ((unsigned)iy < (unsigned)g.H) & ((unsigned)ix < (unsigned)g.W);
                 const int voff = ok ? info.x + x_tapoff[q] : -1;
@@ -382,8 +402,12 @@
                     if constexpr (!ONE) *reinterpret_cast<bf16x4*>(&Dl[(d_cq[q] + c) * LDW + quad * 4]) = pd[q][c][1];
                 }
             }
-#pragma unroll
-        for (int q = 0; q < XQ; ++q)
+        if constexpr (XM) {
+#pragma unroll
+            for (int k = 0; k < XW; ++k) Xw[tid + kThreads * k] = pxw[k];
+        }
+#pragma unroll
+        for (int q = 0; q < (XM ? 0 : XQ); ++q)
             if (grp0 + GPP * q < XG) {
 #pragma unroll
                 for (int c = 0; c < 4; ++c) {
@@ -411,6 +435,17 @@
         }
 #pragma unroll
         for (int j = 0; j < TN; ++j) {
+            if constexpr (XM) {
+                const u32x4 w0 = *reinterpret_cast<const u32x4*>(&Xw[(wn * TN + j) * WBK + ks * 16 + 8 * h]);
+                const u32x4 w1 = *reinterpret_cast<const u32x4*>(&Xw[(wn * TN + j) * WBK + ks * 16 + 8 * h + 4]);
+                u32x4 d;
+                d[0] = (((w0[0] >> r) & 1u) | (((w0[1] >> r) & 1u) << 16)) * 0x3F80u;
+                d[1] = (((w0[2] >> r) & 1u) | (((w0[3] >> r) & 1u) << 16)) * 0x3F80u;
+                d[2] = (((w1[0] >> r) & 1u) | (((w1[1] >> r) & 1u) << 16)) * 0x3F80u;
+                d[3] = (((w1[2] >> r) & 1u) | (((w1[3] >> r) & 1u) << 16)) * 0x3F80u;
+                bh[j] = __builtin_bit_cast(bf16x8, d);
+                continue;
+            }
             const int off = ((wn * TN + j) * 32 + r) * LDW + ks * 16 + 8 * h;
             bh[j] = *reinterpret_cast<const bf16x8*>(&Xh[off]);
             if constexpr (!ONE && !XSP) bl[j] = *reinterpret_cast<const bf16x8*>(&Xl[off]);
@@ -427,9 +462,9 @@
             }
     };
     constexpr int NM = TM * TN * (ONE ? 1 : (XSP ? 2 : 3));
-    constexpr int NREAD = XSP ? 2 * TM + TN : (TM + TN) * (ONE ? 1 : 2);
+    constexpr int NREAD = XM ? 2 * TM + 2 * TN : (XSP ? 2 * TM + TN : (TM + TN) * (ONE ? 1 : 2));
     constexpr int CQ_OPS = SB ? 12 : 56;
-    constexpr int VPG_D = (DQ * CQ_OPS + NM - 1) / NM, VPG_X = (XQ * (XSP ? 24 : CQ_OPS) + NM - 1) / NM;
+    constexpr int VPG_D = (DQ * CQ_OPS + NM - 1) / NM, VPG_X = XM ? (TN * 20 + NM - 1) / NM : (XQ * (XSP ? 24 : CQ_OPS) + NM - 1) / NM;
 
     decode(0);
     __syncthreads();
@@ -439,8 +474,11 @@
 #pragma unroll
     for (int q = 0; q < DQ; ++q) convert_quad(rd[q], pd[q]);
 #pragma unroll
+    for (int k = 0; k < XW; ++k) pxw[k] = rxw[k];
+#pragma unroll
     for (int q = 0; q < XQ; ++q) {
-        if constexpr (XSP) convert_spikes(rx[q], px[q]);
+        if constexpr (XM) continue;
+        else if constexpr (XSP) convert_spikes(rx[q], px[q]);
         else convert_quad(rx[q], px[q]);
     }
     write_tiles();
@@ -463,8 +501,11 @@
         __builtin_amdgcn_sched_barrier(0);
         mfma_group(1);
 #pragma unroll
+        for (int k = 0; k < XW; ++k) pxw[k] = rxw[k];
+#pragma unroll
         for (int q = 0; q < XQ; ++q) {
-            if constexpr (XSP) convert_spikes(rx[q], px[q]);
+            if constexpr (XM) continue;
+            else if constexpr (XSP) convert_spikes(rx[q], px[q]);
             else convert_quad(rx[q], px[q]);
         }
         __builtin_amdgcn_sched_group_barrier(0x100, NREAD, 0);
@@ -774,7 +815,7 @@
 };
 static WgradPlan wgrad_plan(int64_t N, int H, int W, int Cin, int Ho, int Wo, int Cout, int KH, int KW, int stride, int pad,
                             int64_t ldx, int64_t lddy, unsigned align, int precision, bool xsp, int num_cu, int splitk,
-                            bool halo = true) {
+                            bool halo = true, bool xm = false) {
     WgradPlan p = {};
     if (num_cu <= 0) num_cu = snn_num_cu();
     const int bwd_split = precision;
@@ -800,7 +841,7 @@
             return p;
         }
     }
-    const bool vec = (Cin % 4 == 0) && (Cout % 4 == 0) && (ldx % 4 == 0) && (lddy % 4 == 0) &&
+    const bool vec = (Cin % 4 == 0) && (Cout % 4 == 0) && (xm || ldx % 4 == 0) && (lddy % 4 == 0) &&
                      (sbf ? (align & kAlignIn8) && (align & kAlignDy8) : (align & kAlignIn16) && (align & kAlignDy16));
     p.t = wgrad_tile(Cout, Ktot, bwd_split && Cin % 4 == 0 && Cout % 4 == 0, M);
     static const int wbk_small = snn_tuning_env("SNN_WGRAD_WBK") ? atoi(snn_tuning_env("SNN_WGRAD_WBK")) : 64;
@@ -809,7 +850,8 @@
     const int64_t span_pix = p.pix_per_split * (int64_t)stride * stride + 3 * (int64_t)H * W;
     static const bool no_pipe = snn_tuning_env("SNN_WGRAD_NO_PIPE") != nullptr;
     const bool pipe = vec && bwd_split && !no_pipe && M < 0x7fffffffLL && span_pix * ldx * 4 < 0x7fffffffLL &&
-                      p.pix_per_split * lddy * 4 < 0x7fffffffLL && (int64_t)H * W * ldx * 4 < 0x7fffffffLL;
+                      p.pix_per_split * lddy * 4 < 0x7fffffffLL && (int64_t)H * W * ldx * 4 < 0x7fffffffLL &&
+                      (!xm || (Cin % 32 == 0 && ldx * 32 >= Cin && M * ldx * 4 < 0x7fffffffLL));
     p.one = precision == SNN_PREC_BF16X1 || sbf;
     p.kernel = pipe ? kWgradPipe : (vec ? kWgradVec : kWgradScalar);
     if (sbf && !pipe) {
@@ -836,14 +878,15 @@
 
 static int wgrad_common(const float* x, int64_t ldx, const float* dy, int64_t lddy, float* dw, int64_t N,
                         int H, int W, int Cin, int Ho, int Wo, int Cout, int KH, int KW, int stride, int pad,
-                        int accumulate, float* workspace, int splitk, int precision, void* stream, bool xsp, float x_th) {
+                        int accumulate, float* workspace, int splitk, int precision, void* stream, bool xsp, float x_th,
+                        bool xm = false) {
     SNN_REQUIRE(x && dy && dw && workspace, "snn_conv2d_wgrad: null pointer");
     SNN_REQUIRE(precision == SNN_PREC_FP32 || precision == SNN_PREC_BF16X3 || precision == SNN_PREC_BF16X1 ||
                     precision == SNN_PREC_BF16S,
                 "snn_conv2d_wgrad: precision must be SNN_PREC_FP32, _BF16X3, _BF16X1 or _BF16S (got %d)", precision);
     const bool sbf = precision == SNN_PREC_BF16S;
     if (check_conv_shape("snn_conv2d_wgrad", N, H, W, Cin, Ho, Wo, Cout, KH, KW, stride, pad)) return 1;
-    SNN_REQUIRE(ldx >= Cin && lddy >= Cout, "snn_conv2d_wgrad: pixel stride smaller than channel count");
+    SNN_REQUIRE((xm || ldx >= Cin) && lddy >= Cout, "snn_conv2d_wgrad: pixel stride smaller than channel count");
     SNN_REQUIRE(splitk >= 1 && splitk <= 32768, "snn_conv2d_wgrad: bad splitk %d", splitk);
     SNN_REQUIRE(N * (int64_t)H * W < 0x7fffffffLL, "snn_conv2d_wgrad: more than 2^31 input pixels");
     WgradGeom g;
@@ -853,8 +896,9 @@
     g.ldx = ldx; g.lddy = lddy;
     g.Ktot = KH * KW * Cin;
     g.x_th = x_th;
-    const unsigned align = wgrad_align_bits(x, dy) | (aligned(16, {dw, workspace}) ? kAlignDw16 : 0u);
-    WgradPlan p = wgrad_plan(N, H, W, Cin, Ho, Wo, Cout, KH, KW, stride, pad, ldx, lddy, align, precision, xsp, 0, splitk);
+    unsigned align = wgrad_align_bits(x, dy) | (aligned(16, {dw, workspace}) ? kAlignDw16 : 0u);
+    if (xm) align = (align & ~(kAlignIn16 | kAlignIn8)) | (aligned(4, {x}) ? kAlignIn16 : 0u);
+    WgradPlan p = wgrad_plan(N, H, W, Cin, Ho, Wo, Cout, KH, KW, stride, pad, ldx, lddy, align, precision, xsp, 0, splitk, !xm, xm);
     if (p.kernel == kWgradFirst) {
         const FirstPlan& fp = p.fp;
         FirstGeom fg = {ldx, lddy, (int)(N * Ho), H, W, Ho, Wo, Cout, stride, pad, fp.group_rows, splitk, nullptr,
@@ -888,18 +932,18 @@
     dim3 grid((unsigned)((int64_t)g.tiles_m * g.tiles_n * splitk));
     hipStream_t st = (hipStream_t)stream;
     dispatch(
-        [&](auto ID, auto KERNEL, auto WBK, auto ONE, auto SB, auto XSP) {
+        [&](auto ID, auto KERNEL, auto WBK, auto ONE, auto SB, auto XSP, auto XM) {
             constexpr WgradShape t = kWgradShapes[ID()];
             if constexpr (KERNEL() != kWgradPipe) {
                 hipLaunchKernelGGL((k_conv_wgrad<t.tm, t.tn, t.wm, t.wn, KERNEL() == kWgradVec>), grid, dim3(kThreads), 0, st, x, dy,
                                    workspace, g);
-            } else if constexpr ((!SB() || ONE()) && (!XSP() || (!ONE() && !SB()))) {
-                hipLaunchKernelGGL((k_conv_wgrad_pipe<t.tm, t.tn, t.wm, t.wn, WBK(), ONE(), SB(), XSP()>), grid, dim3(kThreads), 0,
+            } else if constexpr ((!SB() || ONE()) && (!XSP() || (!ONE() && !SB())) && (!XM() || XSP())) {
+                hipLaunchKernelGGL((k_conv_wgrad_pipe<t.tm, t.tn, t.wm, t.wn, WBK(), ONE(), SB(), XSP(), XM()>), grid, dim3(kThreads), 0,
                                    st, x, dy, workspace, g);
             }
             return true;
         },
-        OneOf<0, 1, 2, 3, 4, 5>{p.t.id}, OneOf<0, 1, 2>{p.kernel}, OneOf<32, 64>{p.wbk}, Flag{p.one}, Flag{sbf}, Flag{xsp});
+        OneOf<0, 1, 2, 3, 4, 5>{p.t.id}, OneOf<0, 1, 2>{p.kernel}, OneOf<32, 64>{p.wbk}, Flag{p.one}, Flag{sbf}, Flag{xsp}, Flag{xm});
     SNN_CHECK_LAUNCH("snn_conv2d_wgrad");
     return wgrad_reduce_slabs(workspace, dw, (int64_t)Cout * g.Ktot, splitk, accumulate, st);
 }
@@ -990,3 +1034,27 @@
     return snn_conv2d_spikes_wgrad(vdec, ld, v_th, dy, lddy, dw, N, H, W, Cin, H, W, Cout, 1, 1, 1, 0, accumulate, workspace,
                                    splitk, stream);
 }
+
+bool snn_wgrad_mask_ok(int64_t N, int H, int W, int Cin, int Cout, const uint32_t* mask, int64_t ld_mask, const float* dy,
+                       int64_t lddy, const float* dw) {
+    if (!(N > 0 && H > 0 && W > 0 && Cin > 0 && Cout > 0 && mask && dy && dw && Cin % 32 == 0 && Cout % 4 == 0 &&
+          ld_mask >= Cin / 32 && lddy >= Cout && lddy % 4 == 0 && aligned(4, {mask, dw}) && aligned(16, {dy}) &&
+          (int64_t)Cin * Cout < (1LL << 26)))
+        return false;
+    const int64_t M = N * H * (int64_t)W;
+    if (!(M < 0x7fffffffLL - 64 && (M + 64 + 3 * (int64_t)H * W) * ld_mask * 4 < 0x7fffffffLL && (M + 64) * lddy * 4 < 0x7fffffffLL))
+        return false;
+    const unsigned align = kAlignIn16 | kAlignDy16 | kAlignDy8 | (aligned(16, {dw}) ? kAlignDw16 : 0u);
+    const WgradPlan p = wgrad_plan(N, H, W, Cin, H, W, Cout, 1, 1, 1, 0, ld_mask, lddy, align, SNN_PREC_BF16X3, true, 0, 0, false, true);
+    return p.ok && p.kernel == kWgradPipe;
+}
+
+extern "C" int snn_conv1x1_mask_wgrad(const uint32_t* mask, int64_t ld_mask, const float* dy, int64_t lddy, float* dw, int64_t N,
+                                      int H, int W, int Cin, int Cout, int accumulate, float* workspace, int splitk,
+                                      void* stream) {
+    SNN_REQUIRE(mask && dy && dw && workspace, "snn_conv1x1_mask_wgrad: null pointer");
+    SNN_REQUIRE(snn_wgrad_mask_ok(N, H, W, Cin, Cout, mask, ld_mask, dy, lddy, dw),
+                "snn_conv1x1_mask_wgrad: call not covered (ask snn_conv1x1_mask_supported)");
+    return wgrad_common(reinterpret_cast<const float*>(mask), ld_mask, dy, lddy, dw, N, H, W, Cin, H, W, Cout, 1, 1, 1, 0,
+                        accumulate, workspace, splitk, SNN_PREC_BF16X3, stream, true, 0.0f, true);
+}
diff --git a/snn_for_object_detection_amd/csrc/scan_fwd.hip b/snn_for_object_detection_amd/csrc/scan_fwd.hip
--- a/snn_for_object_detection_amd/csrc/scan_fwd.hip
+++ b/snn_for_object_detection_amd/csrc/scan_fwd.hip
@@ -11,7 +11,8 @@
     const float* __restrict__ v0, const float* __restrict__ i0, float* __restrict__ out, int64_t ldo,
     const float* __restrict__ addend, int64_t ld_add, float* __restrict__ vT, float* __restrict__ iT,
     float* __restrict__ vdec, int T, int64_t M, int C, snn_neuron_params p, int last_only,
-    const float* __restrict__ cmem_pc = nullptr, const float* __restrict__ csyn_pc = nullptr) {
+    const float* __restrict__ cmem_pc = nullptr, const float* __restrict__ csyn_pc = nullptr,
+    uint32_t* __restrict__ mask = nullptr, int64_t ld_mask = 0) {
     typedef typename Vec<VEC>::type V;
     static_assert(!SB || SAVE != 2, "the checkpointed scan keeps fp32 checkpoints: not combined with bf16 storage");
     static_assert(!PC || (NEURON == SNN_NEURON_LIF && !SB && SAVE != 2), "per-channel time constants: LIF on fp32 tensors");
@@ -39,11 +40,12 @@
                 for (int j = 0; j < VEC; ++j) lane<VEC>(i, j) = 0.0f;
             }
         }
-        auto time_loop = [&](auto piped_c, auto add_c, auto noout_c, auto last_c) {
+        auto time_loop = [&](auto piped_c, auto add_c, auto noout_c, auto last_c, auto mask_c) {
         constexpr bool PIPED = decltype(piped_c)::value;
         constexpr bool LAST = decltype(last_c)::value;
         constexpr bool ADD = decltype(add_c)::value;
         constexpr bool NOOUT = decltype(noout_c)::value;
+        constexpr bool MASK = decltype(mask_c)::value;
         constexpr int kPrefetch = PIPED ? SNN_SCAN_PREFETCH : 0;
         struct StepOps { V x, a, b, ad; };
         auto fetch_step = [&](int t) {
@@ -144,22 +146,35 @@
                 if constexpr (VEC == 4 && !SB && SNN_SCAN_NT_AUX != 0) __builtin_nontemporal_store(vd, reinterpret_cast<f32x4*>(vdec + row * C + c));
                 else VecS<VEC, SB>::store(vdec, row * C + c, vd);
             }
+            if constexpr (MASK && VEC == 4) {
+                unsigned wd = 0;
+#pragma unroll
+                for (int j = 0; j < VEC; ++j) wd |= (lane<VEC>(vd, j) > p.v_th ? 1u : 0u) << j;
+                wd <<= (c & 31);
+                wd |= (unsigned)__builtin_amdgcn_update_dpp(0, (int)wd, 0xB1, 0xf, 0xf, true);
+                wd |= (unsigned)__builtin_amdgcn_update_dpp(0, (int)wd, 0x4E, 0xf, 0xf, true);
+                wd |= (unsigned)__builtin_amdgcn_update_dpp(0, (int)wd, 0x141, 0xf, 0xf, true);
+                mask[row * ld_mask + (c >> 5)] = wd;
+            }
         }
         if constexpr (LAST) VecS<VEC, SB>::store(out, m * ldo + c, o_keep);
         };
         if constexpr (VEC > 1 && SAVE != 2) {
             if (alpha && !last_only) {
-                if (addend) time_loop(std::true_type{}, std::true_type{}, std::false_type{}, std::false_type{});
-                else if (SAVE == 1 && NEURON == SNN_NEURON_LIF && !SB && out == nullptr)
-                    time_loop(std::true_type{}, std::false_type{}, std::true_type{}, std::false_type{});
-                else time_loop(std::true_type{}, std::false_type{}, std::false_type{}, std::false_type{});
+                constexpr std::true_type yes{};
+                constexpr std::false_type no{};
+                if (addend) time_loop(yes, yes, no, no, no);
+                else if (SAVE == 1 && NEURON == SNN_NEURON_LIF && !SB && !PC && VEC == 4 && out == nullptr && mask != nullptr)
+                    time_loop(yes, no, yes, no, yes);
+                else if (SAVE == 1 && NEURON == SNN_NEURON_LIF && !SB && out == nullptr) time_loop(yes, no, yes, no, no);
+                else time_loop(yes, no, no, no, no);
             } else if (alpha && last_only && !addend) {
-                time_loop(std::true_type{}, std::false_type{}, std::false_type{}, std::true_type{});
+                time_loop(std::true_type{}, std::false_type{}, std::false_type{}, std::true_type{}, std::false_type{});
             } else {
-                time_loop(std::false_type{}, std::false_type{}, std::false_type{}, std::false_type{});
+                time_loop(std::false_type{}, std::false_type{}, std::false_type{}, std::false_type{}, std::false_type{});
             }
         } else {
-            time_loop(std::false_type{}, std::false_type{}, std::false_type{}, std::false_type{});
+            time_loop(std::false_type{}, std::false_type{}, std::false_type{}, std::false_type{}, std::false_type{});
         }
         if (NEURON != SNN_NEURON_NONE) {
             if (vT) Vec<VEC>::store(vT + m * C + c, v);
@@ -194,11 +209,15 @@
 static int neuron_fwd(int neuron, const float* y, int64_t ldy, const float* alpha, const float* beta, const float* v0,
                       const float* i0, float* out, int64_t ldo, const float* addend, int64_t ld_addend, float* vT,
                       float* iT, float* vdec, bool ckpt, int T, int64_t M, int C, const snn_neuron_params* p,
-                      int flags, void* stream, const float* cmem_pc = nullptr, const float* csyn_pc = nullptr) {
+                      int flags, void* stream, const float* cmem_pc = nullptr, const float* csyn_pc = nullptr,
+                      uint32_t* mask = nullptr, int64_t ld_mask = 0) {
     const bool pc = cmem_pc != nullptr;
-    const char* const fn = pc ? "snn_lif_tau_fwd" : "snn_affine_neuron_fwd";
-    SNN_REQUIRE((flags & ~(SNN_SCAN_LAST_STEP_ONLY | SNN_SCAN_BF16_STORAGE | SNN_SCAN_SPIKES_FROM_VDEC)) == 0,
+    const char* const fn = pc ? "snn_lif_tau_fwd" : (mask ? "snn_affine_neuron_fwd_mask" : "snn_affine_neuron_fwd");
+    SNN_REQUIRE((flags & ~(SNN_SCAN_LAST_STEP_ONLY | SNN_SCAN_BF16_STORAGE | SNN_SCAN_SPIKES_FROM_VDEC | SNN_SCAN_SPIKE_MASK)) == 0,
                 "%s: unknown flags 0x%x", fn, flags);
+    const bool with_mask = (flags & SNN_SCAN_SPIKE_MASK) != 0;
+    SNN_REQUIRE(with_mask == (mask != nullptr) && (!with_mask || !pc),
+                "%s: SNN_SCAN_SPIKE_MASK comes with a mask buffer, through snn_affine_neuron_fwd_mask only", fn);
     const int last_only = (flags & SNN_SCAN_LAST_STEP_ONLY) != 0;
     const bool sb = (flags & SNN_SCAN_BF16_STORAGE) != 0;
     const bool no_out = (flags & SNN_SCAN_SPIKES_FROM_VDEC) != 0;
@@ -224,13 +243,16 @@
     };
     SNN_REQUIRE(!sb || (lanes_ok(4, 8) && !ckpt && bf16_neuron(neuron)), "%s: %s, without checkpointing", fn, kBf16Covers);
     const int lanes = sb ? (lanes_ok(8, 16) ? 8 : 4) : (lanes_ok(4, 16) ? 4 : 1);
+    SNN_REQUIRE(!with_mask || (no_out && C % 32 == 0 && ld_mask >= C / 32 && aligned(4, {mask}) && lanes == 4),
+                "%s: SNN_SCAN_SPIKE_MASK needs SNN_SCAN_SPIKES_FROM_VDEC, C a multiple of 32, ld_mask >= C / 32 and 16-byte "
+                "aligned operands", fn);
     const FwdPlan fp = fwd_plan(neuron, M, C, lanes, vdec != nullptr, ckpt);
     const bool launched = dispatch(
         [&](auto NEURON, auto VEC, auto SAVE, auto SB, auto PC) {
             if constexpr (fwd_instance(NEURON(), VEC(), SAVE(), SB(), PC())) {
                 hipLaunchKernelGGL((k_affine_neuron_fwd<NEURON(), VEC(), SAVE(), SB(), PC()>), dim3(fp.blocks), dim3(kThreads), 0,
                                    (hipStream_t)stream, y, ldy, alpha, beta, v0, i0, out, ldo, addend, ld_addend, vT, iT,
-                                   vdec, T, M, C, *p, last_only, cmem_pc, csyn_pc);
+                                   vdec, T, M, C, *p, last_only, cmem_pc, csyn_pc, mask, ld_mask);
                 return true;
             } else {
                 return false;
@@ -248,6 +270,17 @@
                                      const snn_neuron_params* p, int flags, void* stream) {
     return neuron_fwd(neuron, y, ldy, alpha, beta, v0, i0, out, ldo, addend, ld_addend, vT, iT, vdec, false, T, M, C, p,
                       flags, stream);
+}
+
+extern "C" int snn_affine_neuron_fwd_mask(int neuron, const float* y, int64_t ldy, const float* alpha, const float* beta,
+                                          const float* v0, const float* i0, float* out, int64_t ldo, const float* addend,
+                                          int64_t ld_addend, float* vT, float* iT, float* vdec, int T, int64_t M, int C,
+                                          const snn_neuron_params* p, int flags, void* stream, uint32_t* mask,
+                                          int64_t ld_mask) {
+    SNN_REQUIRE(((flags & SNN_SCAN_SPIKE_MASK) != 0) == (mask != nullptr),
+                "snn_affine_neuron_fwd_mask: SNN_SCAN_SPIKE_MASK and the mask buffer come together");
+    return neuron_fwd(neuron, y, ldy, alpha, beta, v0, i0, out, ldo, addend, ld_addend, vT, iT, vdec, false, T, M, C, p,
+                      flags, stream, nullptr, nullptr, mask, ld_mask);
 }
 
 extern "C" int snn_lif_ckpt_interval(void) { return kCkpt; }
diff --git a/snn_for_object_detection_amd/functional.py b/snn_for_object_detection_amd/functional.py
--- a/snn_for_object_detection_amd/functional.py
+++ b/snn_for_object_detection_amd/functional.py
@@ -509,6 +509,8 @@
 FUSE_OUTER_ADDEND = not os.environ.get("SNN_NO_OUTER_ADDEND")
 USE_SIBLING_FUSION = not os.environ.get("SNN_NO_SIBLING_FUSION")
 USE_SPIKES_FROM_VDEC = not os.environ.get("SNN_NO_SPIKES_FROM_VDEC")
+USE_SPIKE_MASK = not os.environ.get("SNN_NO_SPIKE_MASK")
+SPIKE_MASK_MIN_BYTES = 4 << 20
 
 
 class GradAccumulator:
@@ -892,7 +894,7 @@
 class _SiblingConv1x1(Function):
 
     @staticmethod
-    def forward(ctx, x, w1, dest, acc, prec, slot1, slots2, x_th, *w2s):
+    def forward(ctx, x, w1, dest, acc, prec, slot1, slots2, x_th, x_mask, *w2s):
         _require_device(x, "conv2d input", bf16_ok=True)
         fwd_prec, bwd_prec = _conv_precs(prec, x.dtype == _BF16)
         T, B, Cin, H, W = _dims5(x)
@@ -931,7 +933,14 @@
         x, x_th = _spikes_fwd_operand(x, x_th, lambda: _spikes_fwd_ok(
             _hip.query("snn_conv1x1_spikes_supported", T * B, H, W, Cin, Ct, cl_stride(x), fwd_prec, bwd_prec), False,
             x.data_ptr(), wc.data_ptr()))
-        if x_th is not None:
+        if x_th is None:
+            x_mask = None
+        if x_mask is not None and _hip.query("snn_conv1x1_mask_supported", T * B, H, W, Cin, Ct, x_mask.data_ptr(),
+                                             x_mask.shape[-1], wc.data_ptr(), y.data_ptr(), cl_stride(y), None, 0, None,
+                                             fwd_prec, bwd_prec):
+            _hip.call("snn_conv1x1_mask_fwd", x_mask.data_ptr(), x_mask.shape[-1], wc.data_ptr(), y.data_ptr(), cl_stride(y),
+                      T * B, H, W, Cin, Ct, _stream())
+        elif x_th is not None:
             _hip.call("snn_conv1x1_spikes_fwd", x.data_ptr(), cl_stride(x), x_th, wc.data_ptr(), y.data_ptr(), cl_stride(y),
                       T * B, H, W, Cin, Ct, _stream())
         else:
@@ -939,6 +948,8 @@
                       H, W, Cin, H, W, Ct, 1, 1, 1, 0, None, 0, None, 0, None, fwd_prec, _stream())
         ctx.prec = bwd_prec
         ctx.x_th = x_th
+        ctx.x_mask = x_mask
+        ctx.fwd_prec = fwd_prec
         ctx.save_for_backward(x, w1m, *w2ms)
         ctx.wct = wct
         ctx.geom = (T, B, Cin, H, W, Ct, 1, 1, H, W, 1, 0)
@@ -959,13 +970,19 @@
         dw2s = [None] * len(widths)
         if ctx.needs_input_grad[0]:
             dx = _dgrad_accumulate(ctx.acc, gy, ldg, ctx.wct, x, ctx.geom, _stream(), ctx.prec)
-        if any(ctx.needs_input_grad[8:]) or (composed and ctx.needs_input_grad[1]):
+        if any(ctx.needs_input_grad[9:]) or (composed and ctx.needs_input_grad[1]):
             slot1, slots2 = ctx.slot1, ctx.slots2
             slotted = all(s_ is not None for s_ in slots2) and (slot1 is not None or not composed)
             splitk = _hip.query("snn_conv2d_wgrad_splitk", T * B, H, W, Cin, H, W, Ct, 1, 1, 1, 0, ctx.prec)
             xw, ldxw, x_th = _spikes_wgrad_operand(x, ldx, ctx.x_th, gy, ldg)
-            with _WgradLaunch(x.device, slotted, splitk, Ct, Cin, hold=(x, xw, gy), with_g=True) as (stream, ws, G):
-                if x_th is not None:
+            x_mask = ctx.x_mask
+            with _WgradLaunch(x.device, slotted, splitk, Ct, Cin, hold=(x, xw, gy, x_mask), with_g=True) as (stream, ws, G):
+                if x_mask is not None and _hip.query("snn_conv1x1_mask_supported", T * B, H, W, Cin, Ct, x_mask.data_ptr(),
+                                                     x_mask.shape[-1], None, None, 0, gy.data_ptr(), ldg, G.data_ptr(),
+                                                     ctx.fwd_prec, ctx.prec):
+                    _hip.call("snn_conv1x1_mask_wgrad", x_mask.data_ptr(), x_mask.shape[-1], gy.data_ptr(), ldg, G.data_ptr(),
+                              T * B, H, W, Cin, Ct, 0, ws.data_ptr(), splitk, stream)
+                elif x_th is not None:
                     _hip.call("snn_conv1x1_spikes_wgrad", xw.data_ptr(), ldxw, x_th, gy.data_ptr(), ldg, G.data_ptr(),
                               T * B, H, W, Cin, Ct, 0, ws.data_ptr(), splitk, stream)
                 else:
@@ -995,14 +1012,14 @@
                         dw2s[b] = g2.view(c, C1, 1, 1)
                 if composed and not slotted:
                     dw1 = g1.view(C1, Cin, 1, 1)
-        return (dx, dw1, None, None, None, None, None, None, *dw2s)
+        return (dx, dw1, None, None, None, None, None, None, None, *dw2s)
 
 
 def sibling_conv1x1(x: torch.Tensor, w1: Optional[torch.Tensor], w2s: Sequence[torch.Tensor], dest: Optional[Dest] = None,
                     forward_precision: Optional[str] = None, backward_precision: Optional[str] = None) -> torch.Tensor:
     return _SiblingConv1x1.apply(x, w1, dest, _acc_of(x), _prec_codes(forward_precision, backward_precision),
                                  _slot_of(w1), tuple(_slot_of(w) for w in w2s), getattr(x, "_snn_spike_threshold", None),
-                                 *w2s)
+                                 getattr(x, "_snn_spike_mask", None), *w2s)
 
 
 def composed_conv1x1(x: torch.Tensor, w1: torch.Tensor, w2: torch.Tensor, dest: Optional[Dest] = None,
@@ -1012,7 +1029,7 @@
         return place(y, dest) if dest is not None else y
     seq, single = as_sequence(x)
     y = _SiblingConv1x1.apply(seq, w1, dest, _acc_of(seq), _prec_codes(forward_precision, backward_precision),
-                              _slot_of(w1), (_slot_of(w2),), None, w2)
+                              _slot_of(w1), (_slot_of(w2),), None, None, w2)
     return y[0] if single else y
 
 
@@ -1143,6 +1160,7 @@
     defer_apply: bool
     spikes_out: Optional[list]
     tau_slots: Tuple[Optional[GradSlot], Optional[GradSlot]]
+    spike_mask: bool = False
 
 
 def _bf16_scan_covers(neuron: int, channels: int) -> bool:
@@ -1272,13 +1290,21 @@
                     _ptr(iT) if has_state else None, _ptr(vdec), T, M, C, params)
             fwd_flags = ((_hip.SCAN_LAST_STEP_ONLY if last_only else 0) | sb_flag
                          | (_hip.SCAN_SPIKES_FROM_VDEC if no_out else 0))
+            mask = None
+            if no_out and cfg.spike_mask and USE_SPIKE_MASK and not tau and C % 32 == 0 and T * M * C * 4 >= SPIKE_MASK_MIN_BYTES and all(
+                    t is None or t.data_ptr() % 16 == 0 for t in (y, alpha, beta, v0, i0, vT, iT, vdec)):
+                mask = torch.empty((T, B, H, W, C // 32), device=dev, dtype=torch.int32)
             if tau:
                 _hip.call("snn_lif_tau_fwd", *head, c_mem.data_ptr(), c_syn.data_ptr(), fwd_flags, st)
+            elif mask is not None:
+                _hip.call("snn_affine_neuron_fwd_mask", *head, fwd_flags | _hip.SCAN_SPIKE_MASK, st, mask.data_ptr(), C // 32)
             else:
                 _hip.call("snn_affine_neuron_fwd", *head, fwd_flags, st)
             if no_out:
                 out = _alias(vdec, vdec.storage_offset(), T, B, C, H, W, C)
                 spikes_out.append(float(params.v_th))
+                if mask is not None:
+                    spikes_out.append(mask)
         ctx.ckpt = ckpt
         ctx.sb = sb
         ctx.defer_apply = cfg.defer_apply
@@ -1472,7 +1498,7 @@
 def affine_neuron(y: torch.Tensor, neuron: int, state: Optional[NeuronState] = None, bn=None,
                   params: Optional[NeuronParams] = None, dest: Optional[Dest] = None,
                   addend: Optional[torch.Tensor] = None, last_only: bool = False, spikes_ok: bool = False,
-                  tau: Optional[Tuple[torch.Tensor, torch.Tensor]] = None):
+                  tau: Optional[Tuple[torch.Tensor, torch.Tensor]] = None, spike_mask_ok: bool = False):
     if y.dtype == _BF16 and not _bf16_scan_covers(neuron, y.shape[-3]):
         if tau is not None:
             _tau_refusal(neuron, True)
@@ -1520,10 +1546,13 @@
     cfg = _NeuronCfg(neuron=neuron, has_bn=has_bn, training=training, eps=float(eps), momentum=float(momentum),
                      running_mean=rm, running_var=rv, params=params, g_slot=_slot_of(gamma), b_slot=_slot_of(bias), dest=dest,
                      sync_group=sync_group, bn_hint=bn_hint, last_only=bool(last_only) and not single,
-                     defer_apply=defer_apply, spikes_out=spikes_out, tau_slots=(_slot_of(w_mem), _slot_of(w_syn)))
+                     defer_apply=defer_apply, spikes_out=spikes_out, tau_slots=(_slot_of(w_mem), _slot_of(w_syn)),
+                     spike_mask=bool(spike_mask_ok))
     out, vT, iT = _AffineNeuron.apply(seq, gamma, bias, v0, i0, addend, cfg, w_mem, w_syn)
     if spikes_out:
         out._snn_spike_threshold = spikes_out[0]
+        if len(spikes_out) > 1:
+            out._snn_spike_mask = spikes_out[1]
     if neuron == _hip.NEURON_NONE:
         new_state = None
     elif neuron == _hip.NEURON_SYNAPSE:
diff --git a/snn_for_object_detection_amd/generator.py b/snn_for_object_detection_amd/generator.py
--- a/snn_for_object_detection_amd/generator.py
+++ b/snn_for_object_detection_amd/generator.py
@@ -256,17 +256,18 @@
                                           and any(w.requires_grad for w in cell.tau))
                                  and not (isinstance(holder, StateStorage) and not self.training))
                     nxt_l = branch[plan[k + 1][1]] if (not last and plan[k + 1][0] == "layer") else None
+                    to_siblings = (not last and plan[k + 1][0] == "conv_block"
+                                   and branch[plan[k + 1][1] + 1]._siblings is not None and HF.USE_SIBLING_FUSION)
                     spikes_ok = (zero_copy and not last and self.training and neuron == _hip.NEURON_LIF
                                  and direct is None and shortcut is None and not isinstance(holder, StateStorage)
                                  and HF.USE_SPIKES_FROM_VDEC
-                                 and ((plan[k + 1][0] == "conv_block" and branch[plan[k + 1][1] + 1]._siblings is not None
-                                       and HF.USE_SIBLING_FUSION)
+                                 and (to_siblings
                                       or (isinstance(nxt_l, HipConv2d) and nxt_l.in_channels % 32 == 0
                                           and nxt_l.out_channels % 4 == 0 and nxt_l.kernel_size[0] <= 5
                                           and nxt_l.forward_precision is None and nxt_l.backward_precision is None)))
                     Y, new = HF.affine_neuron(Y, neuron, old, bn=layer, params=cell.params, dest=direct,
                                               addend=shortcut, last_only=only_last, spikes_ok=spikes_ok,
-                                              tau=getattr(cell, "tau", None))
+                                              tau=getattr(cell, "tau", None), spike_mask_ok=spikes_ok and to_siblings)
                     if isinstance(holder, StateStorage):
                         holder.record(old, Y, new)
                     branch_state[idx + 1] = new
diff --git a/snn_for_object_detection_amd/profiler.py b/snn_for_object_detection_amd/profiler.py
--- a/snn_for_object_detection_amd/profiler.py
+++ b/snn_for_object_detection_amd/profiler.py
@@ -60,6 +60,15 @@
             return WGRAD_LABELS[0], flops, byts
         tile = "32, 4, 1" if cout <= 32 else ("64, 2, 2" if cout <= 64 else "128, 2, 2")
         return f"k_conv_gather<{tile}, false, true>", flops, byts
+    if name in ("snn_conv1x1_mask_fwd", "snn_conv1x1_mask_wgrad"):
+        fwd = name.endswith("_fwd")
+        n, h, w, cin, cout = (a[5], a[6], a[7], a[8], a[9])
+        flops = 2.0 * n * h * w * cout * cin
+        byts = n * h * w * cin / 8.0 + 4.0 * (n * h * w * cout + cout * cin)
+        if not fwd:
+            return WGRAD_LABELS[0] + ", mask, spikes", flops, byts
+        tile = "32, 4, 1" if cout <= 32 else ("64, 2, 2" if cout <= 64 else "128, 2, 2")
+        return f"k_conv_gather<{tile}, false, true>, mask, spikes", flops, byts
     if name in ("snn_conv2d_spikes_fwd", "snn_conv2d_spikes_wgrad"):
         fwd = name.endswith("_fwd")
         n, h, w, cin, ho, wo, cout, kh, kw, stride, pad = a[6:17]
@@ -92,14 +101,16 @@
         flops = 2.0 * n * ho * wo * cout * kh * kw * cin
         byts = 4.0 * (n * h * w * cin + 2 * n * ho * wo * cout + cout * kh * kw * cin)
         return WGRAD_LABELS[2], flops, byts
-    if name == "snn_affine_neuron_fwd":
+    if name in ("snn_affine_neuron_fwd", "snn_affine_neuron_fwd_mask"):
         neuron, T, M, C = a[0], a[14], a[15], a[16]
         last_only = bool(a[18] & 2)
         elems = float(T) * M * C
         wrote_out = 0 if a[7] is None else (1.0 / T if last_only else 1)
         tensors = 1 + wrote_out + (1 if a[13] is not None else 0) + (1 if a[9] is not None else 0)
         sb = bool(a[18] & SCAN_BF16_STORAGE)
-        return f"k_affine_neuron_fwd<{neuron}>" + (", bf16s" if sb else ""), 12.0 * elems, (2.0 if sb else 4.0) * elems * tensors
+        mask_bytes = elems / 8.0 if (name.endswith("_mask") and a[20] is not None) else 0.0
+        return (f"k_affine_neuron_fwd<{neuron}>" + (", bf16s" if sb else ""), 12.0 * elems,
+                (2.0 if sb else 4.0) * elems * tensors + mask_bytes)
     if name == "snn_affine_neuron_bwd":
         neuron, T, M, C = a[0], a[15], a[16], a[17]
         last_only = bool(a[19] & 2)
@@ -161,7 +172,7 @@
 
     def before(self, name, args):
         label, flops, byts = work_of(name, args)
-        if name in ("snn_affine_neuron_fwd", "snn_lif_fwd_ckpt"):
+        if name in ("snn_affine_neuron_fwd", "snn_affine_neuron_fwd_mask", "snn_lif_fwd_ckpt"):
             self.neuron_steps += flops / 12.0
         start = torch.cuda.Event(enable_timing=True)
         end = torch.cuda.Event(enable_timing=True)
```

New measurement: 7329, median of 6. 1.01x the previous value.
